# richarddurbin/modimizer

Hardware: AMD Instinct MI355X
Metric: Gbp/s hashed+sketched (k=21,d=64) (higher is better)
Workload: dtype u64; 1 GPU; BASELINE config 2: 10 Gbp synthetic ONT-like reads (log-normal N50 20 kb, 5% subs, 30x of a 333 Mbp genome), k=21 d=64 seed=17, seqhash scan + modset build (table bits 30); reads_per_gpu=598835, bases_per_gpu=10000000000, modimizers_per_gpu=156043826, modset_entries=102967436, k=21, d=64, table_bits=30, parallelism=reads sharded x1, modset per GPU

## Files before the change

include/modgpu.h:

```cpp
#ifndef MODGPU_H
#define MODGPU_H

#include <stdio.h>
#include <stdint.h>
#include <stdbool.h>
#include <stddef.h>

#if defined (MODGPU_WITH_REFERENCE_HEADERS) || defined (MS_MINOR)
#ifdef __cplusplus
extern "C" {
#endif
void mgSeqhashDestroy (Seqhash *sh) ;
void mgSeqhashRCiteratorDestroy (SeqhashRCiterator *si) ;
#ifdef __cplusplus
}
#endif
#else
#include "modgpu_compat.h"
#endif

#ifdef __cplusplus
extern "C" {
#endif


typedef enum {
  MG_OK = 0,
  MG_ERR_NO_DEVICE = 1,
  MG_ERR_HIP = 2,
  MG_ERR_ARG = 3,
  MG_ERR_CAPACITY = 4,
  MG_ERR_NOMEM = 5
} MgStatus ;

const char *mgLastError (void) ;
int  mgDeviceCount (void) ;
MgStatus mgSetDevice (int device) ;
const char *mgVersion (void) ;
const char *mgSourceHash (void) ;

U64 *mgIterScanHost (const Seqhash *sh, const char *s, int len) ;
void mgReloadKnobs (void) ;
int  mgIterHostBelow (int below) ;

MgStatus mgDeviceAlloc (void **dptr, size_t bytes) ;
MgStatus mgDeviceFree (void *dptr) ;
MgStatus mgMemcpyH2D (void *dst, const void *src, size_t bytes, void *stream) ;
MgStatus mgMemcpyD2H (void *dst, const void *src, size_t bytes, void *stream) ;
MgStatus mgMemsetD (void *dst, int byte, size_t bytes, void *stream) ;
MgStatus mgStreamSynchronize (void *stream) ;
MgStatus mgCopyD2HBig (void *hostDst, const void *devSrc, size_t bytes) ;
MgStatus mgCopyH2DBig (void *devDst, const void *hostSrc, size_t bytes) ;

#define MG_PACK_PAD 8
size_t   mgPackedWords (U64 nBases) ;
void     mgPackHost (const char *bases, U64 nBases, U32 *words) ;
MgStatus mgPackDevice (const U8 *dBases, U64 nBases, U32 *dWords, void *stream) ;
MgStatus mgUnpackDevice (const U32 *dWords, U64 nBases, U8 *dBases, void *stream) ;
MgStatus mgUploadPack (const char *bases, U64 nBases, U32 *dPacked, void *stream) ;

#define MG_POS_MASK 0x7fffffffu
#define MG_FWD_BIT  0x80000000u
size_t   mgScanWorkBytes (U64 totalBases, U32 nReads, U64 capacity) ;
MgStatus seqhashScanBatchDevice (const Seqhash *sh, const U32 *dPacked, U64 totalBases,
                                 const U64 *dReadOffsets, U32 nReads,
                                 U64 *dKmer, U32 *dPosF, U32 *dReadId, U64 capacity,
                                 U64 *dCount, void *dWork, void *stream) ;

int64_t seqhashScanBatch (const Seqhash *sh, const char *bases, const int64_t *readOffsets, int nReads,
                          U64 **kmer, int **pos, bool **isF, int64_t **survStart) ;

MgStatus seqhashMinimizerBatchDevice (const Seqhash *sh, const U32 *dPacked, U64 totalBases,
                                      const U64 *dReadOffsets, U32 nReads,
                                      U64 *dHash, U32 *dPosF, U64 *dReadStart, U64 capacity, U64 *n, void *stream) ;
int64_t seqhashMinimizerBatch (const Seqhash *sh, const char *bases, const int64_t *readOffsets, int nReads,
                               U64 **hash, int **pos, bool **isF, int64_t **start) ;

MgStatus modsetAddBatchDevice (Modset *ms, const U64 *dKmer, U64 n, U32 *dIndexOut, int withDepth, void *stream) ;
MgStatus modsetFindBatchDevice (Modset *ms, const U64 *dKmer, U64 n, U32 *dIndexOut, void *stream) ;

MgStatus modsetSyncToHost (Modset *ms, int wantIndex) ;
int      mgXferThreadCount (void) ;
void     mgXferDiag (U64 out8[8]) ;
MgStatus mgModsetDeviceRelease (Modset *ms) ;
void     mgModsetHostChanged (Modset *ms) ;
MgStatus mgModsetClear (Modset *ms, void *stream) ;

U64 mgModsetDeviceSlots (Modset *ms) ;

MgStatus mgTableCheckLayout (Modset *ms, U64 *out6) ;
MgStatus mgTableDiag (Modset *ms, U64 *out9) ;
MgStatus mgScanDiag (U64 *out18) ;

MgStatus modsetDepthHistogramDevice (Modset *ms, U64 *dHist65536, void *stream) ;

MgStatus mgAddReadsDevice (Modset *ms, const U32 *dPacked, U64 totalBases,
                           const U64 *dReadOffsets, U32 nReads, U64 *nHash, void *stream) ;
MgStatus mgQueryReadsDevice (Modset *ms, const U32 *dPacked, U64 totalBases,
                             const U64 *dReadOffsets, U32 nReads,
                             U32 *dSeedIndex, U32 *dSeedPosF, U32 *dSeedRead, U64 capacity,
                             U64 *nSeeds, void *stream) ;

MgStatus mgQueryReadsDeviceAsync (Modset *ms, const U32 *dPacked, U64 totalBases, const U64 *dReadOffsets, U32 nReads,
                                  U32 *dSeedIndex, U32 *dSeedPosF, U32 *dSeedRead, U64 capacity, void **ticket, void *stream) ;
MgStatus mgQueryReadsDeviceWait (void *ticket, U64 *nSeeds, void *stream) ;

MgStatus mgInsertReadsDevice (Modset *ms, const U32 *dPacked, U64 totalBases,
                              const U64 *dReadOffsets, U32 nReads,
                              U32 *dSeedIndex, U32 *dSeedPosF, U32 *dSeedRead, U64 capacity,
                              U64 *nSeeds, void *stream) ;

bool mgModsetMergeArrays (Modset *ms1, U64 *value2, U16 *depth2, U8 *info2, U32 n2) ;
bool mgModsetMergeDeviceArrays (Modset *ms1, const U64 *dValue2, const U16 *dDepth2, const U8 *dInfo2, U32 n2) ;

typedef struct MgComm MgComm ;
MgStatus mgCommInitAll (MgComm **comms , int nDev, const int *devices ) ;
MgStatus mgCommGetUniqueId (void *id128) ;
MgStatus mgCommInitRank (MgComm **comm, int nRanks, int rank, const void *id128, int device) ;
int      mgCommRank (const MgComm *c) ;
int      mgCommSize (const MgComm *c) ;
void     mgCommDestroy (MgComm *c) ;
MgStatus mgHistogramAllReduce (Modset *ms, U64 *hist65536, MgComm *c) ;
MgStatus mgDepthAllReduce (Modset *ms, MgComm *c) ;
MgStatus mgModsetMergeRankOrder (Modset *ms, MgComm *c, int root) ;

int64_t mgAddSequenceBatch (Modset *ms, const char *bases, const int64_t *readOffsets, int nReads) ;
void    mgDepthHistogram (Modset *ms, FILE *f) ;
int     mgAddSequences (Modset *ms, const char *bases, const int64_t *readOffsets, int nReads, FILE *out) ;
void    mgModsetWriteText (Modset *ms, FILE *f) ;

typedef struct {
  Modset *ms ;
  U32 size ;
  U32 max ;
  U32 *index, *offset, *id ;
  U32 *depth ;
  U32 *rev, *loc ;
  int nSeq ;
  char **names ;
  U32 *len ;
} MgReference ;
MgReference *mgReferenceCreate (Modset *ms, U32 size) ;
void mgReferenceDestroy (MgReference *ref) ;
int  mgReferenceRead (MgReference *ref, const char *bases, const int64_t *offsets, int nSeq,
                      const char **names, bool isAdd, FILE *out) ;
void mgReferenceWrite (MgReference *ref, const char *root) ;
FILE *mgGzipOpenWrite (const char *name) ;
FILE *mgGzipOpenRead (const char *name) ;
FILE *mgFzOpen (const char *name, const char *mode) ;
MgReference *mgReferenceLoad (const char *root) ;
int  mgQueryProcess (MgReference *ref, const char *bases, const int64_t *offsets, int nReads,
                     const char **names, FILE *out) ;
void mgSetVerbose (int on) ;

typedef struct {
  Modset *ms ;
  int nReads, capReads ;
  int *len, *nHit, *nMiss ;
  int (*nCopy)[4] ;
  U64 *hitStart ;
  U32 *hit ; U16 *dx ;
  U64 totHit, capHit ;
  U64 *invStart ;
  U32 *invSpace ;
  U8 *bad ; int *contained ;
} MgReadset ;
MgReadset *mgReadsetCreate (Modset *ms) ;
void mgReadsetDestroy (MgReadset *rs) ;
int  mgReadsetRead (MgReadset *rs, const char *bases, const int64_t *offsets, int nReads) ;
int  mgReadsetFileRead (MgReadset *rs, const char *filename) ;
void mgReadsetStats (MgReadset *rs, FILE *out) ;
void mgReadsetWrite (MgReadset *rs, const char *root) ;
MgReadset *mgReadsetLoad (const char *root) ;
int  mgReadsetCleanMods (MgReadset *rs, FILE *out) ;
int  mgReadsetCleanModsPath (void) ;
int  mgReadsetProperties (MgReadset *rs, FILE *out) ;
int  mgReadsetPropertiesPath (void) ;
typedef struct { U32 n ; U64 *start ;
                 U32 *iy ; U16 *nHit, *nBadOrder, *nBadFlip ; U8 *flags ; } MgOverlaps ;
int  mgReadsetFindOverlaps (MgReadset *rs, const U32 *reads, U32 n, int level, FILE *out, MgOverlaps *res ) ;
void mgOverlapsFree (MgOverlaps *res) ;
int  mgReadsetOverlapStats (MgReadset *rs, U32 d, FILE *out) ;
int  mgReadsetMarkBadReads (MgReadset *rs, FILE *out) ;
int  mgReadsetMarkContained (MgReadset *rs, FILE *out) ;
int  mgReadsetOverlapsPath (void) ;
void mgReadsetOverlapsDiag (U64 out4[4]) ;
typedef struct { U8 flags ;
                 int rDNApos, nGood, nMod2, nBadLD, nSplit, nSplitLD ; } MgModInfo ;
int  mgReadsetRefFlagFile (MgReadset *rs, const char *refFile, FILE *out) ;
int  mgReadsetRefFlagHits (MgReadset *rs, const U32 *index, const int *pos, U64 n, FILE *out) ;
int  mgReadsetResetBits (MgReadset *rs, int op, FILE *out) ;
int  mgReadsetTestMods (MgReadset *rs, int minDepth, int maxDepth, FILE *yFile, FILE *zFile, FILE *out) ;
const MgModInfo *mgReadsetModInfo (const MgReadset *rs) ;
const U8 *mgReadsetReadFlags (const MgReadset *rs) ;
int  mgReadsetTestModsRun (const MgReadset *rs) ;
int  mgReadsetRdnaPath (void) ;
void mgReadsetRdnaDiag (U64 out4[4]) ;
void mgReadsetRdnaGrid (U32 out4[4]) ;

typedef struct {
  Modset *ms ;
  int len ;
  int *pos ;
  bool *isF ;
  int ownsMs ;
} MgRepRef ;
MgRepRef *mgRepRefCreate (const char *seqFile, const char *modFile, FILE *err) ;
MgRepRef *mgRepRefFromArrays (Modset *ms, const char *bases, int64_t len, FILE *err) ;
void mgRepRefDestroy (MgRepRef *ref) ;

typedef struct MgRepRun MgRepRun ;
typedef struct {
  int nRead, nBad, nGood ;
  int *n, *seqF, *seqR ;
  bool *bad, *isF ;
  U32 max ;
  int *modN, *modNPre ;
  int *goodI, *goodLen ;
  U64 *hitStart ;
  int *hitK, *hitX ;
  int nMod, nDup, tDup, minMax ;
} MgRepResult ;
void mgRepResultFree (MgRepResult *res) ;
MgRepRun *mgRepRunBegin (MgRepRef *ref, Modset *ms) ;
int  mgRepRunAdd (MgRepRun *run, const char *bases, const int64_t *offsets, int nReads, FILE *out) ;
int  mgRepRunFinish (MgRepRun *run, FILE *err, MgRepResult *res) ;
int  mgRepAnalyze3File (MgRepRef *ref, const char *seqFile, const char *modFile, FILE *out, FILE *err, MgRepResult *res) ;
int  mgRepPath (void) ;

typedef struct {
  int nRead, nBad, nGood ;
  U32 max ;
  int nmod[5][4] ;
  int readsBefore, readsAfter ;
  int *modN, *modNPre, *modNPost ;
  U64 *preStart, *postStart ;
  int *preK, *preN, *preX, *postK, *postN, *postX ;
  int *readI ;
  U64 *hitStart ;
  int *hitK ;
} MgRep1Result ;
void mgRep1ResultFree (MgRep1Result *res) ;
int  mgRepRunFinish1 (MgRepRun *run, FILE *out, FILE *err, MgRep1Result *res) ;
int  mgRepAnalyze1File (MgRepRef *ref, const char *seqFile, const char *modFile, FILE *out, FILE *err, MgRep1Result *res) ;
int  mgRepAnalyze1Hits (U32 max, int K, int nReads, const int *readI, const U64 *hitStart, const int *hitK, const int *hitX,
// ... 98 lines not shown
```

modimizer_amd/__init__.py:

```python
import contextlib
import ctypes as C
import os
import subprocess

import numpy as np

_HERE = os.path.dirname(os.path.abspath(__file__))
LIB_PATH = os.environ.get("MODGPU_LIB") or os.path.join(_HERE, "libmodgpu.so")
CSRC = os.path.join(_HERE, "csrc")

U64P = C.POINTER(C.c_uint64)
U32P = C.POINTER(C.c_uint32)

MG_POS_MASK = 0x7FFFFFFF
MG_FWD_BIT = 0x80000000


class Seqhash(C.Structure):
    _fields_ = [("seed", C.c_int), ("k", C.c_int), ("w", C.c_int), ("mask", C.c_uint64),
                ("shift1", C.c_int), ("shift2", C.c_int), ("factor1", C.c_uint64),
                ("factor2", C.c_uint64), ("patternRC", C.c_uint64 * 4)]


class SeqhashRCiterator(C.Structure):
    _fields_ = [("sh", C.POINTER(Seqhash)), ("s", C.c_void_p), ("sEnd", C.c_void_p),
                ("h", C.c_uint64), ("hRC", C.c_uint64), ("hashBuf", C.c_void_p), ("fBuf", C.c_void_p),
                ("base", C.c_int), ("iStart", C.c_int), ("iMin", C.c_int), ("isDone", C.c_bool)]


class Modset(C.Structure):
    _fields_ = [("hasher", C.POINTER(Seqhash)), ("tableBits", C.c_int), ("size", C.c_uint32),
                ("tableSize", C.c_uint64), ("tableMask", C.c_uint64), ("index", U32P),
                ("value", U64P), ("depth", C.POINTER(C.c_uint16)), ("info", C.POINTER(C.c_uint8)),
                ("max", C.c_uint32)]


class MgReference(C.Structure):
    _fields_ = [("ms", C.POINTER(Modset)), ("size", C.c_uint32), ("max", C.c_uint32),
                ("index", U32P), ("offset", U32P), ("id", U32P), ("depth", U32P), ("rev", U32P), ("loc", U32P),
                ("nSeq", C.c_int), ("names", C.POINTER(C.c_char_p)), ("len", U32P)]


class MgReadset(C.Structure):
    _fields_ = [("ms", C.POINTER(Modset)), ("nReads", C.c_int), ("capReads", C.c_int),
                ("len", C.POINTER(C.c_int)), ("nHit", C.POINTER(C.c_int)), ("nMiss", C.POINTER(C.c_int)),
                ("nCopy", C.POINTER(C.c_int * 4)), ("hitStart", U64P), ("hit", U32P), ("dx", C.POINTER(C.c_uint16)),
                ("totHit", C.c_uint64), ("capHit", C.c_uint64), ("invStart", U64P), ("invSpace", U32P),
                ("bad", C.POINTER(C.c_uint8)), ("contained", C.POINTER(C.c_int))]


class MgOverlaps(C.Structure):
    _fields_ = [("n", C.c_uint32), ("start", U64P), ("iy", U32P), ("nHit", C.POINTER(C.c_uint16)), ("nBadOrder", C.POINTER(C.c_uint16)),
                ("nBadFlip", C.POINTER(C.c_uint16)), ("flags", C.POINTER(C.c_uint8))]


class MgModInfo(C.Structure):
    _fields_ = [("flags", C.c_uint8), ("rDNApos", C.c_int), ("nGood", C.c_int), ("nMod2", C.c_int), ("nBadLD", C.c_int), ("nSplit", C.c_int), ("nSplitLD", C.c_int)]


class MgRepRef(C.Structure):
    _fields_ = [("ms", C.POINTER(Modset)), ("len", C.c_int), ("pos", C.POINTER(C.c_int)), ("isF", C.POINTER(C.c_bool)), ("ownsMs", C.c_int)]


class MgRepResult(C.Structure):
    _fields_ = [("nRead", C.c_int), ("nBad", C.c_int), ("nGood", C.c_int),
                ("n", C.POINTER(C.c_int)), ("seqF", C.POINTER(C.c_int)), ("seqR", C.POINTER(C.c_int)),
                ("bad", C.POINTER(C.c_bool)), ("isF", C.POINTER(C.c_bool)), ("max", C.c_uint32),
                ("modN", C.POINTER(C.c_int)), ("modNPre", C.POINTER(C.c_int)),
                ("goodI", C.POINTER(C.c_int)), ("goodLen", C.POINTER(C.c_int)), ("hitStart", U64P),
                ("hitK", C.POINTER(C.c_int)), ("hitX", C.POINTER(C.c_int)),
                ("nMod", C.c_int), ("nDup", C.c_int), ("tDup", C.c_int), ("minMax", C.c_int)]


class MgRep1Result(C.Structure):
    _fields_ = [("nRead", C.c_int), ("nBad", C.c_int), ("nGood", C.c_int), ("max", C.c_uint32), ("nmod", (C.c_int * 4) * 5),
                ("readsBefore", C.c_int), ("readsAfter", C.c_int),
                ("modN", C.POINTER(C.c_int)), ("modNPre", C.POINTER(C.c_int)), ("modNPost", C.POINTER(C.c_int)),
                ("preStart", U64P), ("postStart", U64P),
                ("preK", C.POINTER(C.c_int)), ("preN", C.POINTER(C.c_int)), ("preX", C.POINTER(C.c_int)),
                ("postK", C.POINTER(C.c_int)), ("postN", C.POINTER(C.c_int)), ("postX", C.POINTER(C.c_int)),
                ("readI", C.POINTER(C.c_int)), ("hitStart", U64P), ("hitK", C.POINTER(C.c_int))]


class MgComposition(C.Structure):
    _fields_ = [("type", C.c_int), ("nSeq", C.c_uint64), ("totLen", C.c_uint64), ("lenMin", C.c_uint64), ("lenMax", C.c_uint64),
                ("base", C.c_uint64 * 256), ("qual", C.c_uint64 * 256), ("nBins", C.c_uint32), ("binCount", C.POINTER(C.c_int)), ("binSum", U64P)]


class MgSeqConvert(C.Structure):
    _fields_ = [("inType", C.c_int), ("outType", C.c_int)] + [(n, C.c_uint64) for n in (
        "nSeq", "totSeqLen", "maxSeqLen", "totIdLen", "totDescLen", "maxIdLen", "maxDescLen", "nSeqIn", "totSeqLenIn")]


class MgGzMember(C.Structure):
    _fields_ = [("cOff", C.c_uint64), ("uOff", C.c_uint64), ("cLen", C.c_uint32), ("uLen", C.c_uint32), ("crc", C.c_uint32), ("pad", C.c_uint32)]


class MgGzBlock(C.Structure):
    _fields_ = [("uOff", C.c_uint64), ("uLen", C.c_uint32), ("pad", C.c_uint32)]


class MgSeqBatch(C.Structure):
    _fields_ = [("bases", C.POINTER(C.c_int8)), ("offsets", C.POINTER(C.c_int64)), ("names", C.POINTER(C.c_char_p)),
                ("nSeq", C.c_int), ("total", C.c_int64), ("isFastq", C.c_int), ("basesCap", C.c_int64)]


EXPORTS = [
    "seqhashCreate", "seqhashWrite", "seqhashRead", "seqhashReport", "modRCiterator", "modRCnext",
    "minimizerRCiterator", "minimizerRCnext", "seqString", "mgSeqhashDestroy", "mgSeqhashRCiteratorDestroy",
    "modsetCreate", "modsetDestroy", "modsetWrite", "modsetRead", "modsetIndexFind", "modsetSummary",
    "modsetPack", "modsetDepthPrune", "modsetMerge",
    "mgLastError", "mgDeviceCount", "mgSetDevice", "mgVersion", "mgSourceHash", "mgDeviceAlloc", "mgDeviceFree",
    "mgMemcpyH2D", "mgMemcpyD2H", "mgMemsetD", "mgStreamSynchronize",
    "mgPackedWords", "mgPackHost", "mgPackDevice", "mgUnpackDevice", "mgUploadPack",
    "mgScanWorkBytes", "seqhashScanBatchDevice", "seqhashScanBatch", "seqhashMinimizerBatchDevice", "seqhashMinimizerBatch",
    "modsetAddBatchDevice", "modsetFindBatchDevice", "modsetSyncToHost", "mgXferThreadCount", "mgXferDiag", "mgCopyD2HBig", "mgCopyH2DBig", "mgModsetDeviceRelease",
    "mgModsetHostChanged", "modsetDepthHistogramDevice", "mgTableCheckLayout", "mgTableDiag", "mgScanDiag", "mgAddReadsDevice", "mgQueryReadsDevice", "mgQueryReadsDeviceAsync", "mgQueryReadsDeviceWait",
    "mgAddSequenceBatch", "mgDepthHistogram", "mgSynthGenome", "mgSynthReads",
    "mgInsertReadsDevice", "mgAddSequences", "mgModsetWriteText", "mgReferenceCreate", "mgReferenceDestroy",
    "mgReferenceRead", "mgQueryProcess", "mgReferenceWrite", "mgGzipOpenWrite", "mgFzOpen", "mgGzipOpenRead", "mgReferenceLoad",
    "mgCommInitAll", "mgCommGetUniqueId", "mgCommInitRank", "mgCommRank", "mgCommSize", "mgCommDestroy", "mgHistogramAllReduce", "mgDepthAllReduce", "mgModsetMergeRankOrder",
    "mgReadsetCreate", "mgReadsetDestroy", "mgReadsetRead", "mgReadsetFileRead", "mgReadsetStats", "mgReadsetWrite", "mgReadsetLoad",
    "mgReadsetCleanMods", "mgReadsetCleanModsPath", "mgReadsetProperties", "mgReadsetPropertiesPath",
    "mgReadsetFindOverlaps", "mgOverlapsFree", "mgReadsetOverlapStats", "mgReadsetMarkBadReads", "mgReadsetMarkContained", "mgReadsetOverlapsPath", "mgReadsetOverlapsDiag",
    "mgReadsetRefFlagFile", "mgReadsetRefFlagHits", "mgReadsetResetBits", "mgReadsetTestMods", "mgReadsetModInfo", "mgReadsetReadFlags", "mgReadsetTestModsRun", "mgReadsetRdnaPath", "mgReadsetRdnaDiag", "mgReadsetRdnaGrid",
    "mgRepRefCreate", "mgRepRefFromArrays", "mgRepRefDestroy", "mgRepRunBegin", "mgRepRunAdd", "mgRepRunFinish", "mgRepResultFree", "mgRepAnalyze3File", "mgRepPath",
    "mgRep1ResultFree", "mgRepRunFinish1", "mgRepAnalyze1File", "mgRepAnalyze1Hits", "mgRepCount2", "mgRepAnalyze2File", "mgRep1Diag",
    "mgCompositionFile", "mgCompositionText", "mgCompositionFree", "mgCompositionDiag",
    "mgSeqConvertFile", "mgSeqConvertText", "mgSeqConvertDiag",
    "mgInflateMembersDevice", "mgInflateDiag", "mgInflateMemberHost", "mgBgzfInflateFile", "mgGzipInflateFile", "mgGunzipHost", "mgGunzipDiag",
    "mgDeflateBlocksDevice", "mgDeflateBlockHost", "mgDeflateDiag", "mgBgzfDeflateFile", "mgSeqConvertFileBgzf",
    "mgSeqOpen", "mgSeqNextBatch", "mgSeqBatchFree", "mgSeqClose", "mgSeqReleaseBuffers", "mgReleaseBuffers", "mgTextParseFileDevice", "mgSeqOpenAt", "mgTextFileDiag", "mgAddSequenceFile", "mgReferenceFastaRead", "mgQueryFile",
    "mgReportDepths", "mgRefPaint", "mgRefPaintFile", "mgModsetWriteTextDevice", "mgModsetReadText", "mgModsetReadTextPath",
    "mgAddSequenceFile10x", "mgAddSequenceBatch10x", "mgTrim10xDevice", "mgAdd10xDiag",
    "mgModsetSetCopy", "mgModsetSetCopyM", "mgModsetSetCopyPath", "mgModsetSummaryDevice",
    "mgIterScanHost", "mgIterHostBelow", "mgReloadKnobs", "mgFormatF2", "mgModsetMergeArrays", "mgModsetMergeDeviceArrays", "mgModsetClear", "mgModsetDeviceSlots", "mgSetVerbose", "mgProfileEnable", "mgProfileOnly", "mgProfileReset", "mgProfileKernels", "mgProfileGet",
]


@contextlib.contextmanager
def knobs(**kv):
    old = {}
    for k, v in kv.items():
        name = "MODGPU_" + k
        old[name] = os.environ.get(name)
        if v is None:
            os.environ.pop(name, None)
        else:
            os.environ[name] = str(v)
    lib().mgReloadKnobs()
    try:
        yield
    finally:
        for name, v in old.items():
            if v is None:
                os.environ.pop(name, None)
            else:
                os.environ[name] = v
        lib().mgReloadKnobs()


def source_hash():
    import hashlib
    names = sorted(f for f in os.listdir(CSRC) if f.endswith((".hip", ".c", ".h"))) + ["Makefile", "../../include/modgpu.h", "../../include/modgpu_compat.h"]
    inc = os.path.join(_HERE, "..", "include")
    path = lambda n: os.path.join(inc, os.path.basename(n)) if n.startswith("../") else os.path.join(CSRC, n)
    listing = "".join("%s  %s\n" % (hashlib.sha256(open(path(n), "rb").read()).hexdigest(), n) for n in names)
    return hashlib.sha256(listing.encode()).hexdigest()[:16]


def binary_hash(path=None):
    import re
    try:
        m = re.search(rb"MODGPU_SRC_HASH=([0-9a-f]{16})", open(path or LIB_PATH, "rb").read())
    except OSError:
        return None
    return m.group(1).decode() if m else None


def build(force=False):
    import fcntl
    if os.environ.get("MODGPU_LIB"):
        return LIB_PATH
    def make_if_stale():
        if force or binary_hash() != source_hash():
            subprocess.check_call(["make", "-C", CSRC, "-j8", "-s"] + (["-B"] if force else []))
            if binary_hash() != source_hash():
                raise RuntimeError("libmodgpu.so does not carry the hash of its sources after make: %s != %s" % (binary_hash(), source_hash()))
    try:
        lk = open(os.path.join(CSRC, ".build.lock"), "w")
    except OSError:
        make_if_stale()
        return LIB_PATH
    with lk:
        fcntl.flock(lk, fcntl.LOCK_EX)
        make_if_stale()
    return LIB_PATH


_lib = None


def lib():
    global _lib
    if _lib is not None:
        return _lib
    if os.environ.get("MODGPU_NO_TORCH", "0") != "1":
        try:
            import torch
        except Exception:
            pass
    build()
    L = C.CDLL(LIB_PATH, mode=C.RTLD_GLOBAL)
    if not os.environ.get("MODGPU_LIB"):
        L.mgSourceHash.restype = C.c_char_p
        if L.mgSourceHash().decode() != source_hash():
            raise RuntimeError("the loaded libmodgpu.so was not built from the sources in this tree")
    vp, u64, u32, i32, i64 = C.c_void_p, C.c_uint64, C.c_uint32, C.c_int, C.c_int64
    SH, MS, IT = C.POINTER(Seqhash), C.POINTER(Modset), C.POINTER(SeqhashRCiterator)

    def sig(name, res, *args):
        if os.environ.get("MODGPU_LIB") and not hasattr(L, name):
            return
        f = getattr(L, name); f.restype = res; f.argtypes = list(args)
    sig("seqhashCreate", SH, i32, i32, i32)
    sig("seqhashWrite", None, SH, vp); sig("seqhashRead", SH, vp); sig("seqhashReport", None, SH, vp)
    sig("modRCiterator", IT, SH, vp, i32)
    sig("modRCnext", C.c_bool, IT, U64P, C.POINTER(i32), C.POINTER(C.c_bool))
    sig("minimizerRCiterator", IT, SH, vp, i32)
    sig("mgIterScanHost", vp, SH, vp, i32); sig("mgIterHostBelow", i32, i32); sig("mgReloadKnobs", None)
    sig("mgFormatF2", i32, C.c_char_p, C.c_double)
    sig("minimizerRCnext", C.c_bool, IT, U64P, C.POINTER(i32), C.POINTER(C.c_bool))
    sig("seqString", C.c_char_p, u64, i32)
    sig("mgSeqhashDestroy", None, SH); sig("mgSeqhashRCiteratorDestroy", None, IT)
    sig("modsetCreate", MS, SH, i32, u32); sig("modsetDestroy", None, MS)
    sig("modsetWrite", None, MS, vp); sig("modsetRead", MS, vp)
    sig("modsetIndexFind", u32, MS, u64, i32); sig("modsetSummary", None, MS, vp)
    sig("modsetPack", C.c_bool, MS); sig("modsetDepthPrune", None, MS, i32, i32)
    sig("modsetMerge", C.c_bool, MS, MS)
    sig("mgLastError", C.c_char_p); sig("mgDeviceCount", i32); sig("mgSetDevice", i32, i32)
    sig("mgVersion", C.c_char_p)
    sig("mgSourceHash", C.c_char_p)
    sig("mgDeviceAlloc", i32, C.POINTER(vp), C.c_size_t); sig("mgDeviceFree", i32, vp)
    sig("mgMemcpyH2D", i32, vp, vp, C.c_size_t, vp); sig("mgMemcpyD2H", i32, vp, vp, C.c_size_t, vp)
    sig("mgMemsetD", i32, vp, i32, C.c_size_t, vp); sig("mgStreamSynchronize", i32, vp)
    sig("mgPackedWords", C.c_size_t, u64); sig("mgPackHost", None, vp, u64, vp)
    sig("mgUploadPack", i32, vp, u64, vp, vp); sig("mgPackDevice", i32, vp, u64, vp, vp); sig("mgUnpackDevice", i32, vp, u64, vp, vp)
    sig("mgScanWorkBytes", C.c_size_t, u64, u32, u64)
    sig("seqhashScanBatchDevice", i32, SH, vp, u64, vp, u32, vp, vp, vp, u64, vp, vp, vp)
    sig("seqhashScanBatch", i64, SH, vp, vp, i32, C.POINTER(vp), C.POINTER(vp), C.POINTER(vp), C.POINTER(vp))
    sig("seqhashMinimizerBatchDevice", i32, SH, vp, u64, vp, u32, vp, vp, vp, u64, U64P, vp)
    sig("seqhashMinimizerBatch", i64, SH, vp, vp, i32, C.POINTER(vp), C.POINTER(vp), C.POINTER(vp), C.POINTER(vp))
    sig("modsetAddBatchDevice", i32, MS, vp, u64, vp, i32, vp)
    sig("modsetFindBatchDevice", i32, MS, vp, u64, vp, vp)
    sig("modsetSyncToHost", i32, MS, i32); sig("mgXferThreadCount", i32); sig("mgXferDiag", None, U64P); sig("mgCopyD2HBig", i32, vp, vp, C.c_size_t); sig("mgCopyH2DBig", i32, vp, vp, C.c_size_t); sig("mgModsetDeviceRelease", i32, MS)
    sig("mgModsetHostChanged", None, MS)
    sig("modsetDepthHistogramDevice", i32, MS, vp, vp); sig("mgTableCheckLayout", i32, MS, U64P); sig("mgTableDiag", i32, MS, U64P); sig("mgScanDiag", i32, U64P)
    sig("mgAddReadsDevice", i32, MS, vp, u64, vp, u32, U64P, vp)
    sig("mgQueryReadsDevice", i32, MS, vp, u64, vp, u32, vp, vp, vp, u64, U64P, vp)
    sig("mgQueryReadsDeviceAsync", i32, MS, vp, u64, vp, u32, vp, vp, vp, u64, C.POINTER(vp), vp); sig("mgQueryReadsDeviceWait", i32, vp, U64P, vp)
    sig("mgAddSequenceBatch", i64, MS, vp, vp, i32); sig("mgDepthHistogram", None, MS, vp)
    sig("mgSynthGenome", i32, vp, u64, u64, vp)
    sig("mgSynthReads", i32, vp, u64, vp, vp, vp, u32, u64, C.c_double, u64, vp, vp)
    sig("mgInsertReadsDevice", i32, MS, vp, u64, vp, u32, vp, vp, vp, u64, U64P, vp)
    sig("mgAddSequences", i32, MS, vp, vp, i32, vp); sig("mgModsetWriteText", None, MS, vp)
    sig("mgReferenceCreate", vp, MS, u32); sig("mgReferenceDestroy", None, vp)
    sig("mgReferenceRead", i32, vp, vp, vp, i32, C.POINTER(C.c_char_p), C.c_bool, vp)
    sig("mgQueryProcess", i32, vp, vp, vp, i32, C.POINTER(C.c_char_p), vp)
    RS = C.POINTER(MgReadset)
    sig("mgReadsetCreate", RS, MS); sig("mgReadsetDestroy", None, RS)
    sig("mgReadsetRead", i32, RS, vp, vp, i32); sig("mgReadsetFileRead", i32, RS, C.c_char_p)
    sig("mgReadsetStats", None, RS, vp); sig("mgReadsetWrite", None, RS, C.c_char_p); sig("mgReadsetLoad", RS, C.c_char_p)
    sig("mgReadsetCleanMods", i32, RS, vp); sig("mgReadsetCleanModsPath", i32); sig("mgReadsetProperties", i32, RS, vp); sig("mgReadsetPropertiesPath", i32)
    sig("mgReadsetFindOverlaps", i32, RS, vp, C.c_uint32, i32, vp, C.POINTER(MgOverlaps)); sig("mgOverlapsFree", None, C.POINTER(MgOverlaps))
    sig("mgReadsetOverlapStats", i32, RS, C.c_uint32, vp); sig("mgReadsetMarkBadReads", i32, RS, vp); sig("mgReadsetMarkContained", i32, RS, vp)
    sig("mgReadsetOverlapsPath", i32); sig("mgReadsetOverlapsDiag", None, vp)
    sig("mgReadsetRefFlagFile", i32, RS, C.c_char_p, vp); sig("mgReadsetRefFlagHits", i32, RS, vp, vp, u64, vp); sig("mgReadsetResetBits", i32, RS, i32, vp)
    sig("mgReadsetTestMods", i32, RS, i32, i32, vp, vp, vp); sig("mgReadsetModInfo", C.POINTER(MgModInfo), RS); sig("mgReadsetReadFlags", C.POINTER(C.c_uint8), RS)
    sig("mgReadsetTestModsRun", i32, RS); sig("mgReadsetRdnaPath", i32); sig("mgReadsetRdnaDiag", None, vp); sig("mgReadsetRdnaGrid", None, vp)
    RR, RES = C.POINTER(MgRepRef), C.POINTER(MgRepResult)
    sig("mgRepRefCreate", RR, C.c_char_p, C.c_char_p, vp); sig("mgRepRefFromArrays", RR, MS, vp, i64, vp); sig("mgRepRefDestroy", None, RR)
    sig("mgRepRunBegin", vp, RR, MS); sig("mgRepRunAdd", i32, vp, vp, vp, i32, vp); sig("mgRepRunFinish", i32, vp, vp, RES); sig("mgRepResultFree", None, RES)
    sig("mgRepAnalyze3File", i32, RR, C.c_char_p, C.c_char_p, vp, vp, RES); sig("mgRepPath", i32)
    RES1 = C.POINTER(MgRep1Result)
    sig("mgRep1ResultFree", None, RES1); sig("mgRepRunFinish1", i32, vp, vp, vp, RES1); sig("mgRepAnalyze1File", i32, RR, C.c_char_p, C.c_char_p, vp, vp, RES1)
    sig("mgRepAnalyze1Hits", i32, C.c_uint32, i32, i32, vp, vp, vp, vp, vp, vp, RES1); sig("mgRepCount2", i32, RR, vp, vp, i32, vp)
    sig("mgRepAnalyze2File", i32, RR, C.c_char_p, C.c_char_p, vp, vp); sig("mgRep1Diag", None, vp)
    COMP = C.POINTER(MgComposition)
    sig("mgCompositionFile", i32, C.c_char_p, i32, vp, vp, COMP); sig("mgCompositionText", i32, vp, u64, i32, vp, vp, COMP)
    sig("mgCompositionFree", None, COMP); sig("mgCompositionDiag", None, vp)
    CONV = C.POINTER(MgSeqConvert)
    sig("mgSeqConvertFile", i32, C.c_char_p, C.c_char_p, i32, vp, CONV); sig("mgSeqConvertText", i32, vp, u64, i32, vp, vp, CONV); sig("mgSeqConvertDiag", None, vp)
    sig("mgInflateMembersDevice", i32, vp, u64, C.POINTER(MgGzMember), u32, vp, u64, vp, C.POINTER(u32), vp); sig("mgInflateDiag", None, vp)
    sig("mgInflateMemberHost", i32, vp, u32, vp, u32, u32, C.POINTER(u32), vp); sig("mgBgzfInflateFile", i32, C.c_char_p, C.c_char_p, vp)
    sig("mgGzipInflateFile", i32, C.c_char_p, C.c_char_p, vp); sig("mgGunzipDiag", None, vp)
    sig("mgGunzipHost", i32, vp, u64, u32, u32, u32, vp, u64, C.POINTER(u64), C.POINTER(u32), vp)
    sig("mgDeflateBlocksDevice", i32, vp, u64, C.POINTER(MgGzBlock), u32, vp, u64, C.POINTER(u64), vp); sig("mgDeflateDiag", None, vp)
    sig("mgDeflateBlockHost", i32, vp, u32, vp, C.POINTER(u32), vp); sig("mgBgzfDeflateFile", i32, C.c_char_p, C.c_char_p, vp)
    sig("mgSeqConvertFileBgzf", i32, C.c_char_p, C.c_char_p, i32, vp, CONV)
    sig("mgSeqOpen", vp, C.c_char_p); sig("mgSeqNextBatch", i32, vp, C.c_int64, C.POINTER(MgSeqBatch))
    sig("mgSeqBatchFree", None, C.POINTER(MgSeqBatch)); sig("mgSeqClose", None, vp); sig("mgSeqReleaseBuffers", None); sig("mgReleaseBuffers", None)
    sig("mgTextParseFileDevice", i32, C.c_char_p, C.POINTER(vp), C.POINTER(vp), C.POINTER(i64))
    sig("mgSeqOpenAt", vp, C.c_char_p, u64, u64, u64); sig("mgTextFileDiag", None, vp)
    sig("mgAddSequenceFile", i32, MS, C.c_char_p, vp); sig("mgReferenceFastaRead", i32, vp, C.c_char_p, C.c_bool, vp)
    sig("mgQueryFile", i32, vp, C.c_char_p, vp)
    sig("mgReportDepths", i32, MS, C.POINTER(MS), i32, vp)
    sig("mgRefPaint", i32, MS, vp, vp, i32, C.POINTER(C.c_char_p), vp); sig("mgRefPaintFile", i32, MS, C.c_char_p, vp)
    sig("mgModsetWriteTextDevice", i32, MS, vp); sig("mgModsetReadText", MS, C.c_char_p); sig("mgModsetReadTextPath", i32)
    sig("mgAddSequenceFile10x", i32, MS, C.c_char_p, vp); sig("mgAddSequenceBatch10x", i64, MS, vp, vp, i32, u64)
    sig("mgTrim10xDevice", i32, vp, u64, vp, u32, u64, vp, vp, U64P, vp); sig("mgAdd10xDiag", None, U64P)
    sig("mgModsetSetCopy", i32, MS, i32, i32, i32); sig("mgModsetSetCopyM", i32, MS, i32); sig("mgModsetSetCopyPath", i32)
    sig("mgModsetSummaryDevice", i32, MS, vp)
    sig("mgReferenceWrite", None, vp, C.c_char_p); sig("mgGzipOpenWrite", vp, C.c_char_p); sig("mgGzipOpenRead", vp, C.c_char_p); sig("mgFzOpen", vp, C.c_char_p, C.c_char_p);
    sig("mgCommInitAll", i32, C.POINTER(vp), i32, C.POINTER(i32)); sig("mgCommGetUniqueId", i32, vp); sig("mgCommInitRank", i32, C.POINTER(vp), i32, i32, vp, i32)
    sig("mgCommRank", i32, vp); sig("mgCommSize", i32, vp); sig("mgCommDestroy", None, vp)
    sig("mgHistogramAllReduce", i32, MS, vp, vp); sig("mgDepthAllReduce", i32, MS, vp); sig("mgModsetMergeRankOrder", i32, MS, vp, i32)
    sig("mgReferenceLoad", C.POINTER(MgReference), C.c_char_p)
    sig("mgModsetMergeArrays", C.c_bool, MS, vp, vp, vp, u32)
    sig("mgModsetMergeDeviceArrays", C.c_bool, MS, vp, vp, vp, u32)
    sig("mgModsetClear", i32, MS, vp); sig("mgModsetDeviceSlots", u64, MS); sig("mgSetVerbose", None, i32)
    sig("mgProfileEnable", None, i32); sig("mgProfileOnly", None, i32); sig("mgProfileReset", None); sig("mgProfileKernels", i32)
    sig("mgProfileGet", i32, i32, C.POINTER(C.c_char_p), C.POINTER(C.c_double), U64P)
    _lib = L
    return L


class ModgpuError(RuntimeError):
    pass


def check(status):
    if status != 0:
        raise ModgpuError("libmodgpu status %d: %s" % (status, lib().mgLastError().decode()))


_libc = C.CDLL(None)
_libc.free.argtypes = [C.c_void_p]
_libc.fopen.restype = C.c_void_p
_libc.fopen.argtypes = [C.c_char_p, C.c_char_p]
_libc.fclose.argtypes = [C.c_void_p]


class CFile:

    def __init__(self, path, mode="w"):
        self.f = _libc.fopen(path.encode(), mode.encode())
        if not self.f:
            raise OSError("cannot open " + path)

    def __enter__(self):
        return C.c_void_p(self.f)

    def __exit__(self, *a):
        _libc.fclose(self.f)



def seqhashCreate(k, w, seed=17):
    if k < 1 or k >= 32:
        raise ValueError("seqhash k %d must be between 1 and 32" % k)
    if w < 1:
        raise ValueError("seqhash w %d must be positive" % w)
    return lib().seqhashCreate(k, w, seed)


def modsetCreate(sh, bits, size=0):
    if bits < 20 or bits > 34:
        raise ValueError("table bits %d must be between 20 and 34" % bits)
    if size >= (1 << bits) >> 2:
        raise ValueError("Modset size %u is too big for %d bits" % (size, bits))
    return lib().modsetCreate(sh, bits, size)


def iterate(sh, bases, minimizer=False):
    L = lib()
    bases = np.ascontiguousarray(bases, dtype=np.uint8)
    mk, nx = (L.minimizerRCiterator, L.minimizerRCnext) if minimizer else (L.modRCiterator, L.modRCnext)
    it = mk(sh, bases.ctypes.data, len(bases))
    u = C.c_uint64(); p = C.c_int(); f = C.c_bool()
    ks, ps, fs = [], [], []
    while nx(it, C.byref(u), C.byref(p), C.byref(f)):
        ks.append(u.value); ps.append(p.value); fs.append(int(f.value))
    L.mgSeqhashRCiteratorDestroy(it)
    return np.array(ks, np.uint64), np.array(ps, np.int32), np.array(fs, np.uint8)


def scan_batch(sh, bases, offsets):
    L = lib()
    bases = np.ascontiguousarray(bases, dtype=np.uint8)
    offsets = np.ascontiguousarray(offsets, dtype=np.int64)
    n_reads = len(offsets) - 1
    pk, pp, pf, ps = C.c_void_p(), C.c_void_p(), C.c_void_p(), C.c_void_p()
    n = L.seqhashScanBatch(sh, bases.ctypes.data, offsets.ctypes.data, n_reads,
                           C.byref(pk), C.byref(pp), C.byref(pf), C.byref(ps))
    if n < 0:
        raise ModgpuError("seqhashScanBatch failed: " + L.mgLastError().decode())

    def take(ptr, ctype, count, dtype):
        a = np.ctypeslib.as_array(C.cast(ptr, C.POINTER(ctype)), (max(count, 1),))[:count].astype(dtype, copy=True)
        _libc.free(ptr)
        return a
    kmer = take(pk, C.c_uint64, n, np.uint64)
    pos = take(pp, C.c_int, n, np.int32)
    isf = take(pf, C.c_bool, n, np.uint8)
    st = take(ps, C.c_int64, n_reads + 1, np.int64)
    return kmer, pos, isf, st


def minimizer_batch(sh, bases, offsets):
    L = lib()
# ... 691 lines not shown
```

modimizer_amd/csrc/mg_api_int.h:

```cpp
#ifndef MG_API_INT_H
#define MG_API_INT_H
#include <stdlib.h>
#include <string.h>
#include <mutex>
#include "mg_common.h"
#include "mg_internal.h"

#define MG_LOOKUP_LOAD_PCT 40

struct MgArena {
  char *base = 0; size_t bytes = 0; size_t used = 0;
  MgStatus reserve (size_t need)
  { if (need <= bytes) return MG_OK;
    if (base) MG_HIP (hipFree (base));
    base = 0; bytes = 0;
    size_t want = need + need / 8 + (1 << 20);
    MG_HIP (hipMalloc ((void **) &base, want));
    bytes = want;
    return MG_OK;
  }
  void reset () { used = 0; }
  void *take (size_t n) { size_t a = mgAl256 (used); used = a + n; return base + a; }
  void release () { if (base) (void) hipFree (base); base = 0; bytes = used = 0; }
};

struct MgDev {
  MgTable t;
  MgArena arena;
  MgArena arena2;
  hipStream_t side = 0;
  hipEvent_t scanned[2] = { 0, 0 }, inputReady = 0;
  int ticketsOut = 0, nextSlot = 0; bool slotBusy[2] = { false, false };
  U64 *hPin;
  U32 hostIndexMax;
  bool built;
  int device = -1;
};

static inline U64 mgScanRetryCap (const volatile U64 *c, U64 cap, U64 *n)
{ *n = c[0]; return (c[1] || c[0] > cap) ? c[3] : 0; }

MG_HIDDEN MgStatus mgCheckHasher (const Seqhash *sh);
MG_HIDDEN U64      mgSurvivorGuess (const Seqhash *sh, U64 totalBases);
MG_HIDDEN void     mgUploadRelease (void);
MG_HIDDEN MgDev   *mgDevLookup (const Modset *ms);
MG_HIDDEN MgStatus mgDevGet (Modset *ms, MgDev **out, hipStream_t st);
MG_HIDDEN MgStatus mgDevRefuseInFlight (const MgDev *d);
MG_HIDDEN U64      mgAddChunkSize (void);
#define MG_ADD_CHUNK (mgAddChunkSize ())
MG_HIDDEN MgStatus mgAddBatch (Modset *ms, MgDev *d, const U64 *dKmer, U64 n, U32 *dIndexOut, int withDepth,
                               bool arenaLive, hipStream_t st, const MgHistReq *counted = 0, const MgSegSrc *segSrc = 0);
extern "C" void mgHostBatchRelease (void);
#endif
```

modimizer_amd/csrc/mg_common.h:

```cpp
#ifndef MG_COMMON_H
#define MG_COMMON_H
#include "mg_knobs.h"

#include <hip/hip_runtime.h>
#include <stdint.h>
#include <time.h>
#include <algorithm>
#include <vector>
#include "modgpu.h"

#define MG_WAVE 64

#define MG_SCAN_THREADS   256
#define MG_POS_PER_THREAD 64
#define MG_TILE_BASES     (64 * MG_POS_PER_THREAD)
#define MG_TILE_WORDS     (MG_TILE_BASES / 16)

struct MgHashParams {
  U64 factor1;
  U64 mask;
  int k;
  int shift1;
  U32 d;
  int dShift;
  U64 dOddInv;
  U64 dOddLim;
  U32 c24;
  U32 inv32;
  U32 lim32;
  U32 small32;
};

void mgSetError (const char *fmt, ...);
MgStatus mgHipFail (hipError_t e, const char *what);
MgStatus mgEnsureDevice (void);
MgHashParams mgMakeParams (const Seqhash *sh);

enum MgKernelId {
  MG_K_PACK = 0, MG_K_UNPACK, MG_K_TILE_FIRST_READ, MG_K_SCAN, MG_K_TABLE_INSERT, MG_K_TABLE_ASSIGN,
  MG_K_TABLE_FLAG, MG_K_TABLE_FIND, MG_K_TABLE_LOAD, MG_K_TABLE_EXPORT, MG_K_TABLE_HIST,
  MG_K_INDEX_REPLAY, MG_K_INDEX_FINISH, MG_K_SYNTH_GENOME, MG_K_SYNTH_READS, MG_K_MEMSET,
  MG_K_SEG_SCAN, MG_K_SEG_COMPACT, MG_K_PART, MG_K_PART_HIST, MG_K_PART_SCATTER, MG_K_RANK_COUNT, MG_K_RANK_SCAN, MG_K_BUCKET_DEDUP,
  MG_K_BUCKET_MERGE, MG_K_RANK_LOOKUP, MG_K_TABLE_FIND_SEG, MG_K_HOT_REDUCE, MG_K_BUCKET_FIND, MG_K_UNPART, MG_K_CHAIN, MG_K_CHAIN_RESOLVE,
  MG_K_PAINT_ITEMS, MG_K_DEPTH_GUARD, MG_K_DEPTH_GATHER, MG_K_TEXT_LEN, MG_K_TEXT_SCAN, MG_K_TEXT_WRITE,
  MG_K_SETTEXT_LINES, MG_K_SETTEXT_SCAN, MG_K_SETTEXT_PARSE, MG_K_SETTEXT_LAST,
  MG_K_OVL_ACTIVE, MG_K_OVL_EMIT, MG_K_OVL_SORT, MG_K_OVL_RUNS, MG_K_OVL_PAIR,
  MG_K_TRIM_OFFSETS, MG_K_TRIM_GATHER, MG_K_SETCOPY, MG_K_COPY_TALLY, MG_K_COUNT
};
void mgProfBegin (int id, hipStream_t st);
void mgProfEnd (int id, hipStream_t st);
#define MG_LAUNCH(id, st, ...) do { mgProfBegin (id, st); hipLaunchKernelGGL (__VA_ARGS__); mgProfEnd (id, st); } while (0)

#define MG_HIP(call) do { hipError_t e_ = (call); if (e_ != hipSuccess) return mgHipFail (e_, #call); } while (0)

struct MgDevScratch {
  const char *what; std::vector<void *> held;
  explicit MgDevScratch (const char *what_) : what (what_) {}
  MgDevScratch (const MgDevScratch &) = delete;
  MgDevScratch &operator= (const MgDevScratch &) = delete;
  ~MgDevScratch () { for (void *p : held) (void) hipFree (p); }
  MgStatus fail () const { return mgHipFail (hipGetLastError (), what); }
  void adopt (void *p) { if (p) held.push_back (p); }
  template <class T> MgStatus get (T **p, size_t count)
  { *p = 0; const hipError_t e = hipMalloc ((void **) p, count * sizeof (T)); if (e != hipSuccess) return mgHipFail (e, what); adopt (*p); return MG_OK; }
  template <class T> T *take (T *p) { held.erase (std::remove (held.begin (), held.end (), (void *) p), held.end ()); return p; }
};
static inline bool mgDevFreeBytes (size_t *freeB)
{ size_t total = 0; if (hipMemGetInfo (freeB, &total) != hipSuccess) { (void) hipGetLastError (); return false; } return true; }
static inline int mgFailedWith (const char *sentence) { if (!mgLastError ()[0]) mgSetError ("%s", sentence); return -1; }

template <class T> struct MgDevBuf {
  T *p = 0; size_t cap = 0;
  MgStatus reserve (size_t want, size_t alloc, const char *what)
  { if (cap >= want) return MG_OK;
    drop ();
    const hipError_t e = hipMalloc ((void **) &p, alloc * sizeof (T)); if (e != hipSuccess) { p = 0; return mgHipFail (e, what); }
    cap = alloc; return MG_OK;
  }
  void drop () { if (p) (void) hipFree (p); p = 0; cap = 0; }
};

#ifdef __HIPCC__
__device__ __forceinline__ bool mgDivisible (U64 x, const MgHashParams &p)
{
  if (x & (((U64) 1 << p.dShift) - 1)) return false;
  return ((x >> p.dShift) * p.dOddInv) <= p.dOddLim;
}

__device__ __forceinline__ bool mgDivisibleOdd (U64 h, const MgHashParams &p) { return h * p.dOddInv <= p.dOddLim; }

__device__ __forceinline__ bool mgDivisibleOdd32 (U64 h, const MgHashParams &p)
{
  const U32 lo = (U32) h, hi = (U32) (h >> 32);
  const U32 a = __builtin_amdgcn_alignbit (hi, lo, 24);
  const U32 t = __umul24 (a, p.c24) + (lo & 0xffffffu);
  return t * p.inv32 <= p.lim32;
}

__device__ __forceinline__ bool mgDivisibleAny32 (U64 h, const MgHashParams &p)
{
  return !((U32) h & (((U32) 1 << p.dShift) - 1u)) && mgDivisibleOdd32 (h >> p.dShift, p);
}

__device__ __forceinline__ U32 mgRevComp16 (U32 w)
{
  const U32 x = __brev (w);
  return __builtin_amdgcn_bitop3_b32 (x << 1, x >> 1, 0x55555555u, 0x27);
}

__device__ __forceinline__ U64 mgRevComp (U64 f, int shift1)
{
  const U64 x = ((U64) mgRevComp16 ((U32) f) << 32) | mgRevComp16 ((U32) (f >> 32));
  return x >> shift1;
}
struct MgGeom { U32 R; int log2NB; int kbits; };
__device__ __forceinline__ U64 mgMixBits (U64 x, int b)
{
  if (b <= 32)
    { U32 y = (U32) x;
      const U32 m32 = b >= 32 ? ~0u : (((U32) 1 << b) - 1);
      const int h32 = (b + 1) >> 1;
      y ^= y >> h32; y = (y * 0xed558ccdu) & m32;
      y ^= y >> h32; y = (y * 0x1a85ec53u) & m32;
      y ^= y >> h32;
      return y;
    }
  const U64 mask = b >= 64 ? ~0ull : (((U64) 1 << b) - 1);
  const int h = (b + 1) >> 1;
  x ^= x >> h; x = (x * 0xff51afd7ed558ccdull) & mask;
  x ^= x >> h; x = (x * 0xc4ceb9fe1a85ec53ull) & mask;
  x ^= x >> h;
  return x;
}
#define MG_MIX_TOP 10
#define MG_MIX_MUL 0x9E3779B1u
__device__ __forceinline__ U64 mgMixK (U64 x, int b)
{
  if (b < 24) return mgMixBits (x, b);
  const int lb = b - MG_MIX_TOP;
  const U64 L = x & (((U64) 1 << lb) - 1), A = x >> lb;
  const U32 low = lb >= 32 ? (U32) L : ((U32) L & (((U32) 1 << lb) - 1));
  const U32 g = (low * MG_MIX_MUL) >> (32 - MG_MIX_TOP);
  return ((A ^ (U64) g) << lb) | mgMixBits (L, lb);
}
__device__ __forceinline__ U32 mgMixTopOfKmer (U64 x, int b, int hiB)
{
  const int lb = b - MG_MIX_TOP;
  const U32 low = lb >= 32 ? (U32) x : ((U32) x & (((U32) 1 << lb) - 1));
  return (U32) (x >> (b - hiB)) ^ ((low * MG_MIX_MUL) >> (32 - hiB));
}
__device__ __forceinline__ U32 mgBucketOfM (U64 m, const MgGeom &g)
{
  if (!g.log2NB) return 0u;
  const int s = g.kbits - g.log2NB;
  return s >= 0 ? (U32) (m >> s) : ((U32) m << (-s));
}
__device__ __forceinline__ U32 mgHomeOfM (U64 m, const MgGeom &g)
{
  U32 x = (U32) m;
  if (g.kbits >= 24) x ^= (U32) (m >> (g.kbits - MG_MIX_TOP)) * 0x9E5u;
  return __umulhi (x * 0x85EBCA6Bu, g.R);
}
__device__ __forceinline__ U32 mgNextSlot (U32 at, U32 R) { return at + 1 == R ? 0u : at + 1; }
#endif

static inline unsigned mgGrid (U64 n, unsigned per = 256, unsigned cap = 4096)
{ U64 b = (n + per - 1) / per; if (b > cap) b = cap; if (b < 1) b = 1; return (unsigned) b; }
static inline size_t mgAl256 (size_t n) { return (n + 255) & ~(size_t) 255; }
static inline double mgNowS (void) { struct timespec ts; clock_gettime (CLOCK_MONOTONIC, &ts); return ts.tv_sec + 1e-9 * ts.tv_nsec; }

static inline void mgPartSplit (int log2NB, int *hiB, int *loB)
{ if (log2NB <= 9) { *hiB = log2NB; *loB = 0; } else { *loB = log2NB / 2; *hiB = log2NB - *loB; } }

#define MG_HIST_STRIDE 16
struct MgHistReq { int log2NB; int kbits; U32 *binCount; int hiB; };

struct MgSegSrc { const U64 *segKmer; const U64 *segCount; const U64 *segStart; U64 segCap; U32 nSegs; };


MgStatus mgLaunchPack (const U8 *dBases, U64 nBases, U32 *dWords, hipStream_t st);
MgStatus mgLaunchUnpack (const U32 *dWords, U64 nBases, U8 *dBases, hipStream_t st);
MgStatus mgLaunchScan (const MgHashParams &p, const U32 *dPacked, U64 totalBases,
                       const U64 *dReadOffsets, U32 nReads,
                       U64 *dKmer, U32 *dPosF, U32 *dReadId, U64 capacity,
                       U64 *dCount, void *dWork, hipStream_t st, const MgHistReq *hist = 0, MgSegSrc *lazy = 0);

U64      mgScanTiles (U64 totalBases);
size_t   mgScanInfoBytes (U64 totalBases);
MgStatus mgScanPrepare (const U64 *dReadOffsets, U32 nReads, U64 totalBases, void *dInfo, hipStream_t st);
size_t   mgScanRangeWorkBytes (U64 nTilesRange, U64 capacity);
MgStatus mgLaunchSegCompact (const MgSegSrc &src, U64 *dKmer, U64 capacity, const U64 *dCount, hipStream_t st);
MgStatus mgLaunchScanRange (const MgHashParams &p, const U32 *dPacked, U64 totalBases,
                            const U64 *dReadOffsets, U32 nReads, const void *dInfo, U64 tile0, U64 tile1,
                            U64 *dKmer, U32 *dPosF, U32 *dReadId, U64 capacity,
                            U64 *dCount, void *dWork, hipStream_t st, const MgHistReq *hist = 0, MgSegSrc *lazy = 0);

U64      mgIterMaxBases (void);
U64      mgIterSegEntries (void);
MgStatus mgLaunchIterScan (const MgHashParams &p, const U32 *dPacked, U64 totalBases, const U64 *dReadOff,
                           U64 *dSegKmer, U32 *dSegPosF, U64 *out, U64 capEntries, U64 *flag, U64 seq, hipStream_t st);

MgStatus mgLaunchMinimizers (const MgHashParams &p, U32 w, const U32 *dPacked, const U64 *dReadOffsets, U32 nReads,
                             U64 *dHash, U32 *dPosF, U64 *dReadStart, U64 capacity, U64 *totalOut, hipStream_t st);

struct MgSlot { U64 key; U32 ord; U32 cnt; };
struct MgTable {
  MgSlot *slots; U64 nSlots;
  U64 capSlots;
  U32 capNB;
  U32 R; int log2NB;
  int kbits;
  U32 *occ;
  U64 *value;
  U16 *baseDepth;
  bool baseZero;
  U64 *liveHist;
  bool liveHistValid;
  U32 size;
  U32 max;
  U32 syncedMax;
  U64 *counters;
  bool pendingDepth;
  bool dirty;
  U64 *find8;
  U64 find8Cap;
  U64 find8Version, version;
  bool empty;
  U64 *pin;
  int newPct;
  int loadPct;
  int  maxLog2Slots;
  U32  wantR;
  U64  diag[7];
  int  tightPct;
};
MgStatus mgTableAlloc (MgTable *t, U64 slotsWanted, hipStream_t st);
MgStatus mgTableEnsure (MgTable *t, U64 nIncoming, hipStream_t st);
MgStatus mgTableRollback (MgTable *t, hipStream_t st);
MgStatus mgTableClean (MgTable *t, hipStream_t st);
void     mgTableForget (MgTable *t, hipStream_t st);
size_t   mgTableAddScratchBytes (const MgTable *t, U64 n);
bool     mgTableUseBuckets (const MgTable *t, U64 n);
MgStatus mgTableAdd (MgTable *t, const U64 *dKmer, U64 n, int withDepth, void *scratch, hipStream_t st,
                     const MgHistReq *counted = 0,
                     const MgSegSrc *segSrc = 0);
bool     mgTableAddTakesSegments (const MgTable *t, U64 n, const MgHistReq *counted);
MgStatus mgTableMarkOccupied (MgTable *t, const U64 *dKmer, U64 n, hipStream_t st);
MgStatus mgTableFind (MgTable *t, const U64 *dKmer, U64 n, U32 *dIndexOut, hipStream_t st);
MgStatus mgTableLayoutCheck (MgTable *t, U64 *dOut4, hipStream_t st);
enum { MG_DIAG_FIND_DIRECT = 0, MG_DIAG_FIND_PART1, MG_DIAG_FIND_PART2_16, MG_DIAG_FIND_PART2_8, MG_DIAG_PACK8, MG_DIAG_REHASH_BUCKET, MG_DIAG_REHASH_ATOMIC };
size_t   mgTableFindPartScratchBytes (U64 n);
int      mgTableFindDigitBits (const MgTable *t);
bool     mgTableFindTakesPartition (const MgTable *t, U64 n, const MgHistReq *counted);
size_t   mgTableFindPart2ScratchBytes (U64 n);
MgStatus mgTableFindPartitioned (MgTable *t, const MgSegSrc &segSrc, U64 n, const MgHistReq *counted, U32 *dIndexOut, U64 *el, void *scratch, hipStream_t st,
                                 void *scratch2 = 0);
MgStatus mgTableFindSegments (MgTable *t, const MgSegSrc &src, U64 n, U32 *dIndexOut, hipStream_t st);
MgStatus mgTableLoadHost (MgTable *t, const U64 *dValue, U32 first, U32 last, hipStream_t st);
MgStatus mgTableExportDepth (MgTable *t, U16 *dDelta, hipStream_t st);
MgStatus mgTableHistogram (MgTable *t, U64 *dHist, hipStream_t st);
MgStatus mgModsetTableForPass (Modset *ms, MgTable **t);
MgStatus mgTableReplayIndex (MgTable *t, const MgHashParams &p, int tableBits, U32 *dIndex, hipStream_t st);
MgStatus mgTableMergeApply (const U32 *dIdx, const U16 *dDepth2, const U8 *dInfo2, U32 n2, U16 *dBaseDepth, U8 *dInfo1, hipStream_t st);
size_t   mgTablePruneScratchBytes (U32 n);
MgStatus mgTablePrune (MgTable *t, const U8 *dInfo, int lo, int hi, U64 *dNewValue, U16 *dNewDepth, U8 *dNewInfo,
                       void *scratch, hipStream_t st);
#define MG_COUNT_WORDS 4

MgStatus mgLaunchSynthGenome (U32 *dPacked, U64 nBases, U64 seed, hipStream_t st);
MgStatus mgLaunchSynthReads (const U32 *dGenome, U64 genomeBases, const U64 *dReadStart,
                             const U64 *dReadOffsets, const U8 *dStrand, U32 nReads, U64 totalBases,
                             double errRate, U64 seed, U32 *dOut, hipStream_t st);

#endif
```

modimizer_amd/csrc/mg_knobs.c:

```c
#define _GNU_SOURCE
#include <pthread.h>
#include <sched.h>
#include <stdio.h>
#include <stdlib.h>
#include <string.h>
#include <unistd.h>
#include <sys/mman.h>
#include "mg_knobs.h"

static MgKnobs gKnobs;
static pthread_once_t gOnce = PTHREAD_ONCE_INIT;

static long num (const char *name)
{ const char *e = getenv (name); return e && *e ? atol (e) : MG_KNOB_UNSET; }

static void readAll (void)
{
  MgKnobs k;
  const char *e = getenv ("MODGPU_TABLE_PATH");
  k.tablePath = e && *e ? (long) e[0] : MG_KNOB_UNSET;
  e = getenv ("MODGPU_FIND_PATH");
  k.findPath = e && *e ? (long) e[0] : MG_KNOB_UNSET;
  k.partPacked = num ("MODGPU_PART_PACKED");       k.partBig = num ("MODGPU_PART_BIG");
  k.addChunk = num ("MODGPU_ADD_CHUNK");           k.scanGrid = num ("MODGPU_SCAN_GRID");
  k.scanGeneric = num ("MODGPU_SCAN_GENERIC");     k.scanHist = num ("MODGPU_SCAN_HIST");
  k.scanDiv64 = num ("MODGPU_SCAN_DIV64");        k.minTiled = num ("MODGPU_MIN_TILED");
  k.minTile = num ("MODGPU_MIN_TILE");
  k.noSegmentInput = num ("MODGPU_NO_SEGMENT_INPUT");
  k.rankSliceShift = num ("MODGPU_RANK_SLICE_SHIFT");
  k.flagPolarity = num ("MODGPU_FLAG_POLARITY");   k.mergeSlots = num ("MODGPU_MERGE_SLOTS");
  k.mergePlace = num ("MODGPU_MERGE_PLACE");
  k.bucketR = num ("MODGPU_BUCKET_R");             k.bucketT = num ("MODGPU_BUCKET_T");
  e = getenv ("MODGPU_HOT_SPLIT");
  k.hotSplit = e && *e ? atol (e) : MG_KNOB_UNSET;
  { const char *c = e ? strchr (e, ',') : 0; k.hotChunk = c ? atol (c + 1) : MG_KNOB_UNSET; }
  k.noAvx2 = num ("MODGPU_NO_AVX2");               k.textHost = num ("MODGPU_TEXT_HOST");
  k.textWindowKb = num ("MODGPU_TEXT_WINDOW_KB");   k.bgzfHost = num ("MODGPU_BGZF_HOST");
  k.inflateNoCrc = num ("MODGPU_INFLATE_NOCRC");   k.bgzfBlock = num ("MODGPU_BGZF_BLOCK");
  k.gzipHost = num ("MODGPU_GZIP_HOST");           k.gzipChunkKb = num ("MODGPU_GZIP_CHUNK_KB");
  k.gzipBatch = num ("MODGPU_GZIP_BATCH");         k.gzipRatio = num ("MODGPU_GZIP_RATIO");
  k.gzipMinKb = num ("MODGPU_GZIP_MIN_KB");
  k.fileBatchMbp = num ("MODGPU_FILE_BATCH_MBP");  k.fileBatchBases = num ("MODGPU_FILE_BATCH_BASES");
  k.textIdsDevice = num ("MODGPU_TEXT_IDS_DEVICE");
  k.queryHostChain = num ("MODGPU_QUERY_HOST_CHAIN");
  k.iterHostBelow = num ("MODGPU_ITER_HOST_BELOW");
  k.readsetHost = num ("MODGPU_READSET_HOST");
  k.overlapCands = num ("MODGPU_OVERLAP_CANDS");
  k.overlapLds = num ("MODGPU_OVERLAP_LDS");
  k.testModsBatch = num ("MODGPU_TESTMODS_BATCH");
  k.segSlack = num ("MODGPU_SEG_SLACK");
  k.partDigits = num ("MODGPU_PART_DIGITS");
  k.findBits = num ("MODGPU_FIND_BITS");
  k.scatterGrid = num ("MODGPU_SCATTER_GRID");     k.tableLoad = num ("MODGPU_TABLE_LOAD");
  k.tightLoad = num ("MODGPU_TIGHT_LOAD");         k.find8 = num ("MODGPU_FIND8");
  k.packThreads = num ("MODGPU_PACK_THREADS");     k.parseThreads = num ("MODGPU_PARSE_THREADS");
  k.xferThreads = num ("MODGPU_XFER_THREADS");       k.gzipThreads = num ("MODGPU_GZIP_THREADS");
  k.xferPieceKb = num ("MODGPU_XFER_PIECE_KB");      k.xferStreams = num ("MODGPU_XFER_STREAMS");
  k.seedTiming = num ("MODGPU_SEED_TIMING");       k.uploadTiming = num ("MODGPU_UPLOAD_TIMING");
  k.textTiming = num ("MODGPU_TEXT_TIMING");       k.parseTiming = getenv ("MODGPU_PARSE_TIMING") ? 1 : MG_KNOB_UNSET;
  k.scanDebug = num ("MODGPU_SCAN_DEBUG");         k.bucketDebug = num ("MODGPU_BUCKET_DEBUG");
  gKnobs = k;
}

const MgKnobs *mgKnobs (void) { pthread_once (&gOnce, readAll); return &gKnobs; }
void mgIterKnobsReloaded (void) __attribute__ ((weak));
void mgReloadKnobs (void) { pthread_once (&gOnce, readAll); readAll (); if (mgIterKnobsReloaded) mgIterKnobsReloaded (); }

static int gCpuBudget;
static pthread_once_t gCpuOnce = PTHREAD_ONCE_INIT;
static void cpuBudgetOnce (void)
{
  long v = sysconf (_SC_NPROCESSORS_ONLN);
  cpu_set_t set;
  if (sched_getaffinity (0, sizeof (set), &set) == 0 && CPU_COUNT (&set) < v) v = CPU_COUNT (&set);
  FILE *q = fopen ("/sys/fs/cgroup/cpu.max", "r");
  if (q)
    { char a[64]; long per = 0;
      if (fscanf (q, "%63s %ld", a, &per) == 2 && strcmp (a, "max") && per > 0) { const long c = (atol (a) + per - 1) / per; if (c < v) v = c; }
      fclose (q);
    }
  gCpuBudget = v < 1 ? 1 : (int) v;
}
int mgCpuBudget (void) { pthread_once (&gCpuOnce, cpuBudgetOnce); return gCpuBudget; }

void mgHugeHint (void *p, size_t n)
{
#ifdef MADV_HUGEPAGE
  if (p && n >= ((size_t) 8 << 20))
    { const size_t pg = 4096;
      char *a = (char *) (((size_t) p + pg - 1) & ~(pg - 1)), *e = (char *) (((size_t) p + n) & ~(pg - 1));
      if (e > a) (void) madvise (a, (size_t) (e - a), MADV_HUGEPAGE);
    }
#else
  (void) p; (void) n;
#endif
}
void *mgAllocBig (size_t n) { void *p = malloc (n ? n : 1); mgHugeHint (p, n); return p; }
```

modimizer_amd/csrc/mg_knobs.h:

```cpp
#ifndef MG_KNOBS_H
#define MG_KNOBS_H
#include <limits.h>
#ifdef __cplusplus
extern "C" {
#endif
#define MG_KNOB_UNSET LONG_MIN
typedef struct {
  long findPath;
  long tablePath;
  long partPacked;
  long partBig;
  long addChunk;
  long scanGrid;
  long scanGeneric;
  long minTile;
  long minTiled;
  long scanDiv64;
  long scanHist;
  long noSegmentInput;
  long rankSliceShift;
  long flagPolarity;
  long mergeSlots;
  long mergePlace;
  long bucketR, bucketT;
  long hotSplit, hotChunk;
  long noAvx2;
  long textHost;
  long textWindowKb;
  long fileBatchMbp;
  long fileBatchBases;
  long readsetHost;
  long overlapCands;
  long testModsBatch;
  long overlapLds;
  long bgzfHost;
  long textIdsDevice;
  long gzipHost;
  long gzipChunkKb;
  long gzipBatch;
  long gzipRatio;
  long gzipMinKb;
  long bgzfBlock;
  long queryHostChain;
  long iterHostBelow;
  long scatterGrid;
  long segSlack;
  long partDigits;
  long findBits;
  long tableLoad;
  long find8;
  long tightLoad;
  long packThreads;
  long parseThreads;
  long gzipThreads;
  long xferPieceKb;
  long xferStreams;
  long xferThreads;
  long inflateNoCrc;
  long seedTiming, uploadTiming, textTiming, parseTiming;
  long scanDebug, bucketDebug;
} MgKnobs;
const MgKnobs *mgKnobs (void);
void mgReloadKnobs (void);
int mgCpuBudget (void);
#include <stddef.h>
void mgHugeHint (void *p, size_t n);
void *mgAllocBig (size_t n);
#ifdef __cplusplus
}
#endif
#endif
```

modimizer_amd/csrc/mg_modsetdev.hip:

```cpp
#include <unordered_map>
#include "mg_api_int.h"
#include "mg_xfer.h"

struct MgOnDevice
{ int before = -1; bool moved = false;
  explicit MgOnDevice (int dev) { if (dev >= 0 && hipGetDevice (&before) == hipSuccess && before != dev) moved = hipSetDevice (dev) == hipSuccess; }
  ~MgOnDevice () { if (moved) (void) hipSetDevice (before); }
};

static std::mutex gRegLock;
static std::unordered_map<const Modset *, MgDev *> gReg;
extern "C" { volatile int mgLiveDeviceModsets = 0; }

MgDev *mgDevLookup (const Modset *ms)
{ std::lock_guard<std::mutex> g (gRegLock); auto it = gReg.find (ms); return it == gReg.end () ? 0 : it->second; }

static void mgDevFree (MgDev *d)
{
  if (!d) return;
  MgOnDevice here (d->device);
  if (d->hPin) (void) hipHostFree (d->hPin);
  if (d->built)
    { (void) hipFree (d->t.slots); (void) hipFree (d->t.value); (void) hipFree (d->t.occ); (void) hipFree (d->t.find8);
      (void) hipFree (d->t.baseDepth); (void) hipFree (d->t.counters); (void) hipFree (d->t.liveHist);
    }
  if (d->side) { (void) hipStreamSynchronize (d->side); (void) hipStreamDestroy (d->side); }
  d->arena.release (); d->arena2.release ();
  for (int i = 0 ; i < 2 ; ++i) if (d->scanned[i]) (void) hipEventDestroy (d->scanned[i]);
  if (d->inputReady) (void) hipEventDestroy (d->inputReady);
  delete d;
}

static void mgDevDrop (Modset *ms, MgDev *d)
{
  { std::lock_guard<std::mutex> g (gRegLock); gReg.erase (ms); mgLiveDeviceModsets = (int) gReg.size (); }
  mgDevFree (d);
}

static MgStatus mgDevOnCallersGpu (const MgDev *d, bool quiet = false)
{
  int cur = -1;
  if (hipGetDevice (&cur) == hipSuccess && cur == d->device) return MG_OK;
  if (!quiet) mgSetError ("this Modset's table lives on GPU %d, the calling thread is on GPU %d (mgSetDevice)", d->device, cur);
  return MG_ERR_ARG;
}

MgStatus mgDevRefuseInFlight (const MgDev *d)
{
  if (!d->ticketsOut) return MG_OK;
  mgSetError ("a query batch of this modset is in flight (mgQueryReadsDeviceAsync without its mgQueryReadsDeviceWait)");
  return MG_ERR_ARG;
}

static MgStatus mgDevBuild (Modset *ms, MgDev *d, hipStream_t st)
{
  MgTable &t = d->t;
  if (ms->tableBits < 20 || ms->tableBits > 32)
    { mgSetError ("device modset supports table bits 20..32 (got %d)", ms->tableBits); return MG_ERR_ARG; }
  memset (&t, 0, sizeof (t));
  t.maxLog2Slots = ms->tableBits - 1;
  t.kbits = 2 * ms->hasher->k;
  t.wantR = 4096;
  { const long r = mgKnobs ()->bucketR; if (r != MG_KNOB_UNSET && r >= 256) t.wantR = (U32) r; }
  t.size = ms->size;
  t.pin = d->hPin + 24;
  U64 cap = (ms->tableSize >> 2);
  MG_HIP (hipMalloc ((void **) &t.value, cap * sizeof (U64)));
  MG_HIP (hipMalloc ((void **) &t.baseDepth, cap * sizeof (U16)));
  MG_HIP (hipMalloc ((void **) &t.counters, 64));
  d->built = true;
  MG_HIP (hipMemsetAsync (t.baseDepth, 0, cap * sizeof (U16), st));
  MG_HIP (hipMemsetAsync (t.counters, 0, 64, st));
  { MgStatus s0 = mgTableEnsure (&t, ms->max, st); if (s0) return s0; }
  t.max = 0; t.syncedMax = 0;
  t.baseZero = !ms->max;
  if (ms->max)
    { MG_HIP (hipStreamSynchronize (st));
      MgStatus s;
      if ((s = mgXferH2D (t.value, ms->value, ((size_t) ms->max + 1) * sizeof (U64)))) return s;
      if ((s = mgXferH2D (t.baseDepth, ms->depth, ((size_t) ms->max + 1) * sizeof (U16)))) return s;
      if ((s = mgTableLoadHost (&t, t.value, 1, ms->max, st))) return s;
      MG_HIP (hipStreamSynchronize (st));
      t.max = t.syncedMax = ms->max;
    }
  d->hostIndexMax = ms->max;
  return MG_OK;
}

MgStatus mgDevGet (Modset *ms, MgDev **out, hipStream_t st)
{
  MgStatus s = mgEnsureDevice (); if (s) return s;
  if (!ms || !ms->hasher) { mgSetError ("null Modset"); return MG_ERR_ARG; }
  if ((s = mgCheckHasher (ms->hasher))) return s;
  MgDev *d = mgDevLookup (ms);
  if (!d)
    { d = new MgDev (); d->built = false; d->hostIndexMax = 0; d->hPin = 0;
      if (hipGetDevice (&d->device) != hipSuccess) { delete d; return mgHipFail (hipGetLastError (), "hipGetDevice"); }
      if (hipHostMalloc ((void **) &d->hPin, 256, hipHostMallocDefault) != hipSuccess) { delete d; return mgHipFail (hipGetLastError (), "hipHostMalloc"); }
      if ((s = mgDevBuild (ms, d, st))) { mgDevFree (d); return s; }
      mgXferWarm ();
      std::lock_guard<std::mutex> g (gRegLock); gReg[ms] = d; mgLiveDeviceModsets = (int) gReg.size ();
    }
  else if ((s = mgDevOnCallersGpu (d))) return s;
  if (d->built && ms->max > d->t.max)
    {
      U32 first = d->t.max + 1, last = ms->max;
      if (last >= (ms->tableSize >> 2)) { mgSetError ("modset max %u beyond table capacity", last); return MG_ERR_CAPACITY; }
      MG_HIP (hipMemcpyAsync (d->t.value + first, ms->value + first, (size_t) (last - first + 1) * sizeof (U64), hipMemcpyHostToDevice, st));
      MG_HIP (hipMemcpyAsync (d->t.baseDepth + first, ms->depth + first, (size_t) (last - first + 1) * sizeof (U16), hipMemcpyHostToDevice, st));
      d->t.baseZero = false;
      if (!d->ticketsOut && (s = mgTableEnsure (&d->t, last - first + 1, st))) return s;
      if ((s = mgTableLoadHost (&d->t, d->t.value, first, last, st))) return s;
      MG_HIP (hipStreamSynchronize (st));
      d->t.max = d->t.syncedMax = last;
      if (d->hostIndexMax == first - 1) d->hostIndexMax = last;
    }
  d->t.size = ms->size;
  *out = d;
  return MG_OK;
}

extern "C" MgStatus mgModsetDeviceRelease (Modset *ms)
{
  MgDev *d = mgDevLookup (ms);
  if (!d) return MG_OK;
  MgStatus s = modsetSyncToHost (ms, 1);
  mgDevDrop (ms, d);
  return s;
}

extern "C" void mgModsetHostChanged (Modset *ms)
{
  MgDev *d = mgDevLookup (ms);
  if (d) mgDevDrop (ms, d);
}

extern "C" MgStatus mgModsetClear (Modset *ms, void *stream)
{
  hipStream_t st = (hipStream_t) stream;
  MgDev *d = mgDevLookup (ms);
  if (d) { MgStatus s = mgDevOnCallersGpu (d); if (s) return s; }
  U32 hostIndexed = d ? d->hostIndexMax : ms->max;
  U32 hostUsed = d ? d->t.syncedMax : ms->max;
  if (d)
    { MgTable &t = d->t;
      mgTableForget (&t, st);
      if (!t.baseZero) MG_HIP (hipMemsetAsync (t.baseDepth, 0, ((size_t) (t.max > t.syncedMax ? t.max : t.syncedMax) + 1) * sizeof (U16), st));
      t.baseZero = true;
      t.max = t.syncedMax = 0;
      t.pendingDepth = false;
      d->hostIndexMax = 0;
    }
  if (hostIndexed) memset (ms->index, 0, ms->tableSize * sizeof (U32));
  if (hostUsed)
    { memset (ms->depth, 0, ((size_t) hostUsed + 1) * sizeof (U16));
      memset (ms->info, 0, (size_t) hostUsed + 1);
    }
  ms->max = 0;
  return MG_OK;
}


static MgStatus mgFoldCounts (MgDev *d, hipStream_t st, Modset *host = 0)
{
  MgTable &t = d->t;
  if (!t.max) return MG_OK;
  if (!t.pendingDepth) return MG_OK;
  MgStatus s = d->arena.reserve (mgAl256 ((size_t) t.max * sizeof (U16)) + 4096); if (s) return s;
  d->arena.reset ();
  U16 *dDelta = (U16 *) d->arena.take ((size_t) t.max * sizeof (U16));
  s = mgTableExportDepth (&t, dDelta, st);
  MG_HIP (hipStreamSynchronize (st));
  if (!s && host) s = mgXferD2H (host->depth + 1, dDelta, (size_t) t.max * sizeof (U16), MG_XFER_SATADD16);
  return s;
}

static int mgMergeDeviceCore (Modset *ms1, MgDev *d, const U64 *dV2, const U16 *dD2, const U8 *dI2, U32 n2, hipStream_t st)
{
  MgTable &t = d->t;
  const U32 max1 = t.max;
  const char *const sorry = "device merge failed";
  MgDevScratch scratch ("device merge");
  U8 *dI1; U32 *dIdx;
  const size_t cap1 = (size_t) max1 + n2 + 2;
  if (scratch.get (&dI1, cap1) || scratch.get (&dIdx, n2)) return -1;
  if (hipMemset (dI1, 0, cap1) || hipDeviceSynchronize ()) return mgFailedWith (sorry);
  if (mgXferH2D (dI1, ms1->info, (size_t) max1 + 1)) return mgFailedWith (sorry);
  MgStatus as = mgAddBatch (ms1, d, dV2, n2, dIdx, 0, false, st);
  if (as == MG_ERR_CAPACITY) { fprintf (stderr, "FATAL ERROR: %s\n", mgLastError ()); exit (-1); }
  if (as) return mgFailedWith (sorry);
  t.baseZero = false; t.liveHistValid = false;
  if (mgTableMergeApply (dIdx, dD2, dI2, n2, t.baseDepth, dI1, st)) return mgFailedWith (sorry);
  if (hipStreamSynchronize (st)) return mgFailedWith (sorry);
  if (t.max > t.syncedMax)
    { if (mgXferD2H (ms1->value + t.syncedMax + 1, t.value + t.syncedMax + 1, (size_t) (t.max - t.syncedMax) * 8, MG_XFER_COPY)) return mgFailedWith (sorry);
      t.syncedMax = t.max;
    }
  if (mgXferD2H (ms1->depth, t.baseDepth, ((size_t) t.max + 1) * 2, MG_XFER_COPY)) return mgFailedWith (sorry);
  if (mgXferD2H (ms1->info, dI1, (size_t) t.max + 1, MG_XFER_COPY)) return mgFailedWith (sorry);
  ms1->depth[0] = 0;
  ms1->max = t.max;
  return 0;
}

extern "C" int mgHookMergeDevice (Modset *ms1, Modset *ms2)
{
  hipStream_t st = 0;
  MgDev *d; if (mgDevGet (ms1, &d, st)) return -1;
  const U32 n2 = ms2->max;
  if (mgFoldCounts (d, st)) return -1;
  if (!n2) return 0;
  MgDevScratch scratch ("device merge: the second set");
  U64 *dV2; U16 *dD2; U8 *dI2;
  if (scratch.get (&dV2, n2) || scratch.get (&dD2, n2) || scratch.get (&dI2, n2)) return -1;
  if (mgXferH2D (dV2, ms2->value + 1, (size_t) n2 * 8) || mgXferH2D (dD2, ms2->depth + 1, (size_t) n2 * 2) || mgXferH2D (dI2, ms2->info + 1, n2)) return mgFailedWith ("device merge failed");
  return mgMergeDeviceCore (ms1, d, dV2, dD2, dI2, n2, st);
}

extern "C" int mgHookMergeDeviceArrays (Modset *ms1, const U64 *dValue2, const U16 *dDepth2, const U8 *dInfo2, U32 n2)
{
  hipStream_t st = 0;
  MgDev *d; if (mgDevGet (ms1, &d, st)) return -1;
  if (mgFoldCounts (d, st)) return -1;
  if (!n2) return 0;
  return mgMergeDeviceCore (ms1, d, dValue2, dDepth2, dInfo2, n2, st);
}

extern "C" int mgHookPruneDevice (Modset *ms, int lo, int hi)
{
  hipStream_t st = 0;
  MgDev *d; if (mgDevGet (ms, &d, st)) return -1;
  MgTable &t = d->t;
  const U32 n = t.max;
  if (mgFoldCounts (d, st)) return -1;
  const char *const sorry = "device prune failed";
  MgDevScratch scratch ("device prune");
  U8 *dInfo, *dNewInfo; U64 *dNewValue; U16 *dNewDepth; char *dWork;
  if (scratch.get (&dInfo, (size_t) n + 1) || scratch.get (&dNewInfo, (size_t) n + 2) || scratch.get (&dNewValue, (size_t) n + 2)
      || scratch.get (&dNewDepth, (size_t) n + 2) || scratch.get (&dWork, mgTablePruneScratchBytes (n ? n : 1))) return -1;
  if (mgXferH2D (dInfo, ms->info, (size_t) n + 1)) return mgFailedWith (sorry);
  if (mgTablePrune (&t, dInfo, lo, hi, dNewValue, dNewDepth, dNewInfo, dWork, st)) return mgFailedWith (sorry);
  U64 c[2];
  if (hipMemcpyAsync (c, t.counters, 16, hipMemcpyDeviceToHost, st) || hipStreamSynchronize (st)) return mgFailedWith (sorry);
  const U32 m = (U32) c[0];
  if (m)
    { t.baseZero = false; t.liveHistValid = false;
      if (hipMemcpy (t.value + 1, dNewValue + 1, (size_t) m * 8, hipMemcpyDeviceToDevice) || hipMemcpy (t.baseDepth + 1, dNewDepth + 1, (size_t) m * 2, hipMemcpyDeviceToDevice)
          || mgXferD2H (ms->value + 1, dNewValue + 1, (size_t) m * 8, MG_XFER_COPY) || mgXferD2H (ms->depth + 1, dNewDepth + 1, (size_t) m * 2, MG_XFER_COPY)
          || mgXferD2H (ms->info + 1, dNewInfo + 1, m, MG_XFER_COPY)) return mgFailedWith (sorry);
    }
  if (n > m && hipMemset (t.baseDepth + m + 1, 0, (size_t) (n - m) * 2)) return mgFailedWith (sorry);
  mgTableForget (&t, st);
  t.max = 0;
  if (mgTableEnsure (&t, m, st)) return mgFailedWith (sorry);
  if (m && mgTableLoadHost (&t, t.value, 1, m, st)) return mgFailedWith (sorry);
  if (hipStreamSynchronize (st)) return mgFailedWith (sorry);
  t.max = t.syncedMax = m;
  ms->max = m;
  d->hostIndexMax = 0;
  return 0;
}

extern "C" void mgHookDestroy (Modset *ms) { mgModsetHostChanged (ms); }
extern "C" void mgHookHostRewrote (Modset *ms) { mgModsetHostChanged (ms); }
extern "C" void mgHookNeedHostAll (Modset *ms, int wantIndex)
{
  MgDev *d = mgDevLookup (ms);
  if (!d) return;
  if (modsetSyncToHost (ms, wantIndex) != MG_OK)
    { fprintf (stderr, "FATAL ERROR: %s\n", mgLastError ()); exit (-1); }
}
extern "C" void mgHookNeedHost (Modset *ms, int wantIndex)
{
  MgDev *d = mgDevLookup (ms);
  if (!d) return;
  if (!d->t.pendingDepth && d->t.syncedMax == d->t.max && (!wantIndex || d->hostIndexMax >= d->t.max)) return;
  mgHookNeedHostAll (ms, wantIndex);
}
extern "C" int mgHookHasDevice (Modset *ms) { return mgDevLookup (ms) != 0; }


U64 mgAddChunkSize (void)
{
  const long c = mgKnobs ()->addChunk;
  U64 v = c != MG_KNOB_UNSET && c > 0 ? (U64) c : ((U64) 1 << 30);
  if (v > ((U64) 1 << 30)) v = (U64) 1 << 30;
  return v;
}

static MgStatus mgAddChunk (Modset *ms, MgDev *d, const U64 *dKmer, U64 n, U32 *dIndexOut, int withDepth,
                            void *scratch, hipStream_t st, const MgHistReq *counted = 0, const MgSegSrc *segSrc = 0)
{
  MgTable &t = d->t;
  MgStatus s;
  MG_HIP (hipMemsetAsync (t.counters, 0, 16, st));
  if ((s = mgTableAdd (&t, dKmer, n, withDepth, scratch, st, counted, segSrc))) return s;
  volatile U64 *c = d->hPin;
  MG_HIP (hipMemcpyAsync (d->hPin, t.counters, 16, hipMemcpyDeviceToHost, st));
  MG_HIP (hipStreamSynchronize (st));
  U64 newMax = (U64) t.max + c[0];
  if (c[1] || newMax >= t.size)
    {
      if ((s = mgTableRollback (&t, st))) return s;
      mgSetError ("hashTableSize %u is too small for %llu", t.size, (unsigned long long) newMax);
      return MG_ERR_CAPACITY;
    }
  t.max = (U32) newMax;
  ms->max = t.max;
  if (n >= 4096) t.newPct = (int) (c[0] * 100 / n);
  if (dIndexOut && (s = mgTableFind (&t, dKmer, n, dIndexOut, st))) return s;
  return MG_OK;
}

MgStatus mgAddBatch (Modset *ms, MgDev *d, const U64 *dKmer, U64 n, U32 *dIndexOut, int withDepth,
                     bool arenaLive, hipStream_t st, const MgHistReq *counted, const MgSegSrc *segSrc)
{
  if (!n) return MG_OK;
  MgStatus s = mgDevRefuseInFlight (d); if (s) return s;
  U64 chunk = n < MG_ADD_CHUNK ? n : MG_ADD_CHUNK;
  if ((s = mgTableEnsure (&d->t, chunk, st))) return s;
  size_t need = mgTableAddScratchBytes (&d->t, chunk) + 4096;
  if (!arenaLive)
    { if ((s = d->arena.reserve (need))) return s;
      d->arena.reset ();
    }
  else if (d->arena.bytes - d->arena.used < need)
    { mgSetError ("internal: arena too small for insert temporaries"); return MG_ERR_NOMEM; }
  void *scratch = d->arena.take (mgTableAddScratchBytes (&d->t, chunk));
  for (U64 off = 0 ; off < n && !s ; off += chunk)
    { U64 m = n - off < chunk ? n - off : chunk;
      if (off) s = mgTableEnsure (&d->t, m, st);
      if (!s) s = mgAddChunk (ms, d, dKmer + off, m, dIndexOut ? dIndexOut + off : 0, withDepth, scratch, st,
                              (counted && n <= chunk) ? counted : 0,
                              n <= chunk ? segSrc : 0);
    }
  return s;
}

extern "C" MgStatus modsetAddBatchDevice (Modset *ms, const U64 *dKmer, U64 n, U32 *dIndexOut, int withDepth, void *stream)
{
  hipStream_t st = (hipStream_t) stream;
  MgDev *d; MgStatus s = mgDevGet (ms, &d, st); if (s) return s;
  return mgAddBatch (ms, d, dKmer, n, dIndexOut, withDepth, false, st);
}

extern "C" MgStatus modsetFindBatchDevice (Modset *ms, const U64 *dKmer, U64 n, U32 *dIndexOut, void *stream)
{
  hipStream_t st = (hipStream_t) stream;
  MgDev *d; MgStatus s = mgDevGet (ms, &d, st); if (s) return s;
  d->t.loadPct = MG_LOOKUP_LOAD_PCT;
  if (d->t.slots && (s = mgTableEnsure (&d->t, 0, st))) return s;
  return mgTableFind (&d->t, dKmer, n, dIndexOut, st);
}

extern "C" MgStatus modsetSyncToHost (Modset *ms, int wantIndex)
{
  MgDev *d = mgDevLookup (ms);
  if (!d) return MG_OK;
  MgOnDevice here (d->device);
  MgTable &t = d->t;
  hipStream_t st = 0;
  MgStatus s;
  MG_HIP (hipDeviceSynchronize ());
  if (d->ticketsOut && (t.pendingDepth || (wantIndex && d->hostIndexMax < t.max)))
    { mgSetError ("a query batch of this modset is in flight (its scratch is what a sync would use)"); return MG_ERR_ARG; }
  if (t.max > t.syncedMax)
    { const U32 first = t.syncedMax + 1;
      if ((s = mgXferD2H (ms->value + first, t.value + first, (size_t) (t.max - first + 1) * sizeof (U64), MG_XFER_COPY))) return s;
      t.syncedMax = t.max;
    }
  ms->max = t.max;
  if ((s = mgFoldCounts (d, st, ms))) return s;
  if (wantIndex && d->hostIndexMax < t.max)
    { if ((s = d->arena.reserve (mgAl256 (ms->tableSize * sizeof (U32)) + 4096))) return s;
      d->arena.reset ();
      U32 *dIndex = (U32 *) d->arena.take (ms->tableSize * sizeof (U32));
      if ((s = mgTableReplayIndex (&t, mgMakeParams (ms->hasher), ms->tableBits, dIndex, st))) return s;
      MG_HIP (hipStreamSynchronize (st));
      if ((s = mgXferD2H (ms->index, dIndex, ms->tableSize * sizeof (U32), MG_XFER_COPY))) return s;
      d->hostIndexMax = t.max;
    }
  return MG_OK;
}

extern "C" MgStatus mgModsetAdoptDepthDevice (Modset *ms, const U16 *dDepth16)
{
  MgDev *d = mgDevLookup (ms);
  if (!d || !d->built) return MG_OK;
  MgTable &t = d->t;
  if (t.pendingDepth || t.max != ms->max) { mgModsetHostChanged (ms); return MG_OK; }
  MG_HIP (hipMemcpy (t.baseDepth, dDepth16, ((size_t) t.max + 1) * sizeof (U16), hipMemcpyDeviceToDevice));
  t.baseZero = false; t.liveHistValid = false;
  return MG_OK;
}

extern "C" int mgHookDeviceView (Modset *ms, const U64 **dValue1, const U16 **dDepth1, U32 *max)
{
  MgDev *d = mgDevLookup (ms);
  if (!d || !d->built || d->ticketsOut) return -1;
  if (mgDevOnCallersGpu (d, true)) return -1;
  if (hipDeviceSynchronize () != hipSuccess || mgFoldCounts (d, 0, ms)) return -1;
  *dValue1 = d->t.value + 1; *dDepth1 = d->t.baseDepth + 1; *max = d->t.max;
  return 0;
}

extern "C" int mgHookDeviceViewMake (Modset *ms, const U64 **dValue1, const U16 **dDepth1, U32 *max)
{
  MgDev *d; if (mgDevGet (ms, &d, 0)) return -1;
  return mgHookDeviceView (ms, dValue1, dDepth1, max);
}

extern "C" U64 mgModsetDeviceSlots (Modset *ms) { MgDev *d = mgDevLookup (ms); return d && d->built ? d->t.nSlots : 0; }

extern "C" MgStatus mgTableCheckLayout (Modset *ms, U64 *out6)
{
  MgDev *d; MgStatus s = mgDevGet (ms, &d, 0); if (s) return s;
  MgDevScratch scratch ("mgTableCheckLayout");
  U64 *dOut;
  if (scratch.get (&dOut, 4)) return MG_ERR_HIP;
  s = mgTableLayoutCheck (&d->t, dOut, 0);
  if (!s && (hipMemcpy (out6, dOut, 32, hipMemcpyDeviceToHost) || hipMemcpy (out6 + 4, d->t.counters + 4, 16, hipMemcpyDeviceToHost))) s = MG_ERR_HIP;
  return s;
}

extern "C" MgStatus mgTableDiag (Modset *ms, U64 *out9)
{
  memset (out9, 0, 9 * sizeof (U64));
  MgDev *d = mgDevLookup (ms);
  if (!d || !d->built) return MG_OK;
  out9[0] = (U64) d->t.log2NB; out9[1] = d->t.R;
  for (int i = 0 ; i < 7 ; ++i) out9[2 + i] = d->t.diag[i];
  return MG_OK;
}

extern "C" MgStatus modsetDepthHistogramDevice (Modset *ms, U64 *dHist, void *stream)
{
  hipStream_t st = (hipStream_t) stream;
  MgDev *d; MgStatus s = mgDevGet (ms, &d, st); if (s) return s;
  return mgTableHistogram (&d->t, dHist, st);
}

MgStatus mgModsetTableForPass (Modset *ms, MgTable **t)
{
  *t = 0;
  if (!ms) { mgSetError ("null Modset"); return MG_ERR_ARG; }
  if (!mgDevLookup (ms)) return MG_OK;
  MgDev *d; MgStatus s = mgDevGet (ms, &d, 0); if (s) return s;
  if (!d->built) return MG_OK;
  if ((s = mgDevRefuseInFlight (d))) return s;
  MG_HIP (hipDeviceSynchronize ());
  ms->max = d->t.max;
  *t = &d->t;
  return MG_OK;
}
```

modimizer_amd/csrc/mg_reads.hip:

```cpp
#include "mg_api_int.h"

struct MgScanBufs { U64 *kmer; U32 *posF; U32 *rid; void *work; U64 *count; U64 cap; MgHistReq counted;
                    MgSegSrc seg; bool lazy; void *findScratch, *findScratch2; };

struct MgScanReq { const Seqhash *sh; const U32 *dPacked; U64 totalBases; const U64 *dReadOffsets; U32 nReads; bool wantPos; size_t extraPerSurvivor;
                   U32 *outPosF, *outRid; U64 outCap; bool lazy; };
static inline MgArena &mgArenaOf (MgDev *d, int slot) { return slot ? d->arena2 : d->arena; }
static inline U64 *mgCountPin (MgDev *d, int slot) { return d->hPin + 8 + 8 * slot; }

static MgStatus mgScanStart (MgDev *d, int slot, const MgScanReq &q, U64 cap, MgScanBufs *b, hipStream_t st)
{
  b->lazy = false; b->seg.nSegs = 0; b->seg.segKmer = 0; b->findScratch = 0; b->findScratch2 = 0;
  MgArena &ar = mgArenaOf (d, slot);
  const long fp = mgKnobs ()->findPath;
  const bool lookupHist = q.lazy && q.wantPos && !q.extraPerSurvivor && d->t.slots && fp != 'd'
                          && (fp == 'p' || fp == '2' || (cap >= ((U64) 1 << 24) && d->t.nSlots >= ((U64) 1 << 24) && d->t.log2NB > 9));
  const bool lookup2 = lookupHist && fp != 'p';
  MgHashParams p = mgMakeParams (q.sh);
  const size_t perS = 8 + (q.wantPos ? 8 : 0) + q.extraPerSurvivor;
  const size_t need = mgAl256 (cap * perS) + 4 * 4096 + 512 * MG_HIST_STRIDE * 4 + mgAl256 (mgScanWorkBytes (q.totalBases, q.nReads, cap))
                      + (q.extraPerSurvivor ? mgTableAddScratchBytes (&d->t, cap < MG_ADD_CHUNK ? cap : MG_ADD_CHUNK) + 8192 : 0) + 8 * 256
                      + (lookupHist ? mgTableFindPartScratchBytes (cap) + 8192 : 0) + (lookup2 ? mgTableFindPart2ScratchBytes (cap) + 8192 : 0);
  MgStatus s = ar.reserve (need); if (s) return s;
  ar.reset ();
  b->cap = cap;
  b->kmer = (U64 *) ar.take (cap * 8);
  const bool direct = q.wantPos && q.outPosF && q.outRid && q.outCap >= cap;
  b->posF = !q.wantPos ? 0 : (direct ? q.outPosF : (U32 *) ar.take (cap * 4));
  b->rid = !q.wantPos ? 0 : (direct ? q.outRid : (U32 *) ar.take (cap * 4));
  b->work = ar.take (mgScanWorkBytes (q.totalBases, q.nReads, cap));
  b->count = (U64 *) ar.take (8 * MG_COUNT_WORDS);
  b->counted.log2NB = 0; b->counted.kbits = 64; b->counted.binCount = 0; b->counted.hiB = 0;
  if (q.extraPerSurvivor || lookupHist)
    { b->counted.binCount = (U32 *) ar.take (512 * MG_HIST_STRIDE * sizeof (U32));
      b->counted.log2NB = d->t.log2NB; b->counted.kbits = d->t.kbits;
      if (lookupHist) b->counted.hiB = mgTableFindDigitBits (&d->t);
    }
  b->findScratch = lookupHist ? ar.take (mgTableFindPartScratchBytes (cap)) : 0;
  b->findScratch2 = lookup2 ? ar.take (mgTableFindPart2ScratchBytes (cap)) : 0;
  const bool lz = q.lazy && (q.wantPos ? q.extraPerSurvivor == 0 : b->counted.binCount != 0);
  if ((s = mgLaunchScan (p, q.dPacked, q.totalBases, q.dReadOffsets, q.nReads, b->kmer, b->posF, b->rid, cap, b->count, b->work, st,
                         b->counted.binCount ? &b->counted : 0, lz ? &b->seg : 0))) return s;
  b->lazy = lz;
  MG_HIP (hipMemcpyAsync (mgCountPin (d, slot), b->count, MG_COUNT_WORDS * sizeof (U64), hipMemcpyDeviceToHost, st));
  return MG_OK;
}
static MgStatus mgScanFinish (MgDev *d, int slot, const MgScanBufs *b, U64 *nOut, U64 *retryCap, hipStream_t st, hipEvent_t done = 0)
{
  if (done) MG_HIP (hipEventSynchronize (done));
  else MG_HIP (hipStreamSynchronize (st));
  *retryCap = mgScanRetryCap (mgCountPin (d, slot), b->cap, nOut);
  return MG_OK;
}

static MgStatus mgScanRounds (MgDev *d, int slot, const MgScanReq &q, U64 cap, MgScanBufs *b, U64 *nOut, hipStream_t st, hipEvent_t started = 0)
{
  for (int round = 0 ; round < 3 ; ++round)
    { MgStatus s;
      const bool running = started && !round;
      if (!running && (s = mgScanStart (d, slot, q, cap, b, st))) return s;
      if ((s = mgScanFinish (d, slot, b, nOut, &cap, st, running ? started : 0))) return s;
      if (!cap) return MG_OK;
    }
  mgSetError ("scan capacity could not be established");
  return MG_ERR_CAPACITY;
}

static MgStatus mgScanIntoArena (MgDev *d, const Seqhash *sh, const U32 *dPacked, U64 totalBases,
                                 const U64 *dReadOffsets, U32 nReads, bool wantPos, size_t extraPerSurvivor,
                                 MgScanBufs *b, U64 *nOut, hipStream_t st,
                                 U32 *outPosF = 0, U32 *outRid = 0, U64 outCap = 0, bool lazy = false)
{
  MgStatus s = mgDevRefuseInFlight (d); if (s) return s;
  MgScanReq q = { sh, dPacked, totalBases, dReadOffsets, nReads, wantPos, extraPerSurvivor, outPosF, outRid, outCap, lazy };
  if (extraPerSurvivor)
    {
      U64 expect = totalBases / (U64) (sh->w > 0 ? sh->w : 1) + 1;
      if (expect > MG_ADD_CHUNK) expect = MG_ADD_CHUNK;
      if ((s = mgTableEnsure (&d->t, expect, st))) return s;
    }
  return mgScanRounds (d, 0, q, mgSurvivorGuess (sh, totalBases), b, nOut, st);
}

extern "C" MgStatus mgAddReadsDevice (Modset *ms, const U32 *dPacked, U64 totalBases,
                                      const U64 *dReadOffsets, U32 nReads, U64 *nHash, void *stream)
{
  hipStream_t st = (hipStream_t) stream;
  MgDev *d; MgStatus s = mgDevGet (ms, &d, st); if (s) return s;
  if (nHash) *nHash = 0;
  if (!totalBases || !nReads) return MG_OK;
  MgScanBufs b; U64 n = 0;
  d->t.loadPct = 75;
  if ((s = mgScanIntoArena (d, ms->hasher, dPacked, totalBases, dReadOffsets, nReads, false, 4, &b, &n, st, 0, 0, 0, true))) return s;
  if (nHash) *nHash = n;
  if (!n) return MG_OK;
  if (b.lazy)
    { const U64 chunk = n < MG_ADD_CHUNK ? n : MG_ADD_CHUNK;
      if ((s = mgTableEnsure (&d->t, chunk, st))) return s;
      if (n <= MG_ADD_CHUNK && mgTableAddTakesSegments (&d->t, n, &b.counted))
        return mgAddBatch (ms, d, 0, n, 0, 1, true, st, &b.counted, &b.seg);
      if ((s = mgLaunchSegCompact (b.seg, b.kmer, b.cap, b.count, st))) return s;
    }
  return mgAddBatch (ms, d, b.kmer, n, 0, 1, true, st, &b.counted);
}

static MgStatus mgSeedsOfScanned (Modset *ms, MgDev *d, MgScanBufs &b, U64 n, U32 *dSeedIndex, U32 *dSeedPosF, U32 *dSeedRead, U64 capacity, hipStream_t st)
{
  if (n > capacity)
    { mgSetError ("%llu seeds exceed the caller's capacity %llu", (unsigned long long) n, (unsigned long long) capacity); return MG_ERR_CAPACITY; }
  MgStatus s;
  if (ms) s = mgAddBatch (ms, d, b.kmer, n, dSeedIndex, 0, true, st, &b.counted);
  else if (b.lazy && b.findScratch && mgTableFindTakesPartition (&d->t, n, &b.counted))
    s = mgTableFindPartitioned (&d->t, b.seg, n, &b.counted, dSeedIndex, b.kmer, b.findScratch, st, b.findScratch2);
  else s = b.lazy ? mgTableFindSegments (&d->t, b.seg, n, dSeedIndex, st) : mgTableFind (&d->t, b.kmer, n, dSeedIndex, st);
  if (s) return s;
  if (dSeedPosF && b.posF != dSeedPosF) MG_HIP (hipMemcpyAsync (dSeedPosF, b.posF, n * 4, hipMemcpyDeviceToDevice, st));
  if (dSeedRead && b.rid != dSeedRead) MG_HIP (hipMemcpyAsync (dSeedRead, b.rid, n * 4, hipMemcpyDeviceToDevice, st));
  MG_HIP (hipStreamSynchronize (st));
  return MG_OK;
}

static MgStatus mgSeedReads (Modset *ms, const Seqhash *scanWith, int mode, const U32 *dPacked, U64 totalBases,
                             const U64 *dReadOffsets, U32 nReads,
                             U32 *dSeedIndex, U32 *dSeedPosF, U32 *dSeedRead, U64 capacity,
                             U64 *nSeeds, hipStream_t st)
{
  MgDev *d; MgStatus s = mgDevGet (ms, &d, st); if (s) return s;
  if (nSeeds) *nSeeds = 0;
  if (!scanWith) scanWith = ms->hasher;
  if ((s = mgCheckHasher (scanWith))) return s;
  if (scanWith->k != ms->hasher->k) { mgSetError ("a batch scanned with k %d cannot be looked up in a set of k %d", scanWith->k, ms->hasher->k); return MG_ERR_ARG; }
  if (!totalBases || !nReads) return MG_OK;
  MgScanBufs b; U64 n = 0;
  d->t.loadPct = MG_LOOKUP_LOAD_PCT;
  if (mode == 0 && d->t.slots && (s = mgTableEnsure (&d->t, 0, st))) return s;
  const int timing = mgKnobs ()->seedTiming == 1;
  struct timespec q0, q1, q2; if (timing) clock_gettime (CLOCK_MONOTONIC, &q0);
  if ((s = mgScanIntoArena (d, scanWith, dPacked, totalBases, dReadOffsets, nReads, true, mode ? 4 : 0, &b, &n, st,
                            dSeedPosF, dSeedRead, capacity, mode == 0))) return s;
  if (timing) clock_gettime (CLOCK_MONOTONIC, &q1);
  if (nSeeds) *nSeeds = n;
  if ((s = mgSeedsOfScanned (mode ? ms : 0, d, b, n, dSeedIndex, dSeedPosF, dSeedRead, capacity, st))) return s;
  if (timing)
    { clock_gettime (CLOCK_MONOTONIC, &q2);
      fprintf (stderr, "mgSeedReads: scan+count %.2f ms, lookup+sync %.2f ms\n", (q1.tv_sec - q0.tv_sec) * 1e3 + (q1.tv_nsec - q0.tv_nsec) * 1e-6,
               (q2.tv_sec - q1.tv_sec) * 1e3 + (q2.tv_nsec - q1.tv_nsec) * 1e-6);
    }
  return MG_OK;
}

extern "C" MgStatus mgQueryReadsDevice (Modset *ms, const U32 *dPacked, U64 totalBases,
                                        const U64 *dReadOffsets, U32 nReads,
                                        U32 *dSeedIndex, U32 *dSeedPosF, U32 *dSeedRead, U64 capacity,
                                        U64 *nSeeds, void *stream)
{ return mgSeedReads (ms, 0, 0, dPacked, totalBases, dReadOffsets, nReads, dSeedIndex, dSeedPosF, dSeedRead, capacity, nSeeds, (hipStream_t) stream); }

extern "C" MgStatus mgInsertReadsDevice (Modset *ms, const U32 *dPacked, U64 totalBases,
                                         const U64 *dReadOffsets, U32 nReads,
                                         U32 *dSeedIndex, U32 *dSeedPosF, U32 *dSeedRead, U64 capacity,
                                         U64 *nSeeds, void *stream)
{ return mgSeedReads (ms, 0, 1, dPacked, totalBases, dReadOffsets, nReads, dSeedIndex, dSeedPosF, dSeedRead, capacity, nSeeds, (hipStream_t) stream); }

extern "C" void mgSeedBufsFree (MgSeedBufs *bufs)
{
  (void) hipFree (bufs->ix); (void) hipFree (bufs->posF); (void) hipFree (bufs->rid);
  bufs->ix = bufs->posF = bufs->rid = 0; bufs->cap = 0;
}
static MgStatus mgSeedBufsReserve (MgSeedBufs *bufs, U64 need)
{
  if (bufs->cap >= need) return MG_OK;
  mgSeedBufsFree (bufs);
  const U64 room = need + need * (U64) bufs->sparePct / 100 + 1;
  U32 **arr[3] = { &bufs->ix, &bufs->posF, &bufs->rid };
  for (int j = 0 ; j < 3 ; ++j)
    { const hipError_t e = hipMalloc ((void **) arr[j], room * sizeof (U32));
      if (e != hipSuccess) { *arr[j] = 0; mgSeedBufsFree (bufs); return mgHipFail (e, "a batch's seed arrays"); }
    }
  bufs->cap = room; return MG_OK;
}
extern "C" MgStatus mgSeedsOfBatch (Modset *ms, const Seqhash *scanWith, int insert, const U32 *dPacked, U64 totalBases, const U64 *dReadOffsets, U32 nReads,
                                    U64 guess, MgSeedBufs *bufs, U64 *nSeeds, void *stream)
{
  const bool empty = !totalBases || !nReads;
  U64 offer = empty ? 0 : (guess < totalBases + 1 ? guess : totalBases + 1);
  *nSeeds = 0;
  for (int attempt = 0 ; ; ++attempt)
    { MgStatus s = mgSeedBufsReserve (bufs, offer); if (s) return s;
      s = mgSeedReads (ms, scanWith, insert ? 1 : 0, dPacked, totalBases, dReadOffsets, nReads, bufs->ix, bufs->posF, bufs->rid, offer, nSeeds, (hipStream_t) stream);
      if (s != MG_ERR_CAPACITY || attempt || *nSeeds <= offer) return s;
      offer = *nSeeds;
    }
}

struct MgQueryTicket { Modset *ms; MgDev *d; int slot; MgScanReq q; MgScanBufs b; U32 *dSeedIndex, *dSeedPosF, *dSeedRead; U64 capacity; };

extern "C" MgStatus mgQueryReadsDeviceAsync (Modset *ms, const U32 *dPacked, U64 totalBases, const U64 *dReadOffsets, U32 nReads,
                                             U32 *dSeedIndex, U32 *dSeedPosF, U32 *dSeedRead, U64 capacity, void **ticket, void *stream)
{
  hipStream_t st = (hipStream_t) stream;
  if (!ticket) { mgSetError ("mgQueryReadsDeviceAsync: null ticket"); return MG_ERR_ARG; }
  *ticket = 0;
  MgDev *d; MgStatus s = mgDevGet (ms, &d, st); if (s) return s;
  if (d->ticketsOut >= 2) { mgSetError ("two query batches are in flight already"); return MG_ERR_ARG; }
  d->t.loadPct = MG_LOOKUP_LOAD_PCT;
  if (d->t.slots && !d->ticketsOut && (s = mgTableEnsure (&d->t, 0, st))) return s;
  if (!d->side)
    {
      int lo = 0, hi = 0; (void) hipDeviceGetStreamPriorityRange (&lo, &hi);
      MG_HIP (hipStreamCreateWithPriority (&d->side, hipStreamNonBlocking, lo));
      for (int i = 0 ; i < 2 ; ++i) MG_HIP (hipEventCreateWithFlags (&d->scanned[i], hipEventDisableTiming));
      MG_HIP (hipEventCreateWithFlags (&d->inputReady, hipEventDisableTiming));
    }
  const int slot = d->slotBusy[d->nextSlot] ? d->nextSlot ^ 1 : d->nextSlot;
  MgQueryTicket *t = new MgQueryTicket ();
  t->ms = ms; t->d = d; t->slot = slot; t->dSeedIndex = dSeedIndex; t->dSeedPosF = dSeedPosF; t->dSeedRead = dSeedRead; t->capacity = capacity;
  t->q = MgScanReq { ms->hasher, dPacked, totalBases, dReadOffsets, nReads, true, 0, dSeedPosF, dSeedRead, capacity, true };
  t->b = MgScanBufs (); t->b.cap = 0;
  if (totalBases && nReads)
    {
      hipError_t e = hipEventRecord (d->inputReady, st);
      if (e == hipSuccess) e = hipStreamWaitEvent (d->side, d->inputReady, 0);
      if (e != hipSuccess) { delete t; return mgHipFail (e, "mgQueryReadsDeviceAsync"); }
      if ((s = mgScanStart (d, slot, t->q, mgSurvivorGuess (ms->hasher, totalBases), &t->b, d->side))) { delete t; return s; }
      if ((e = hipEventRecord (d->scanned[slot], d->side)) != hipSuccess) { delete t; return mgHipFail (e, "mgQueryReadsDeviceAsync"); }
    }
  d->slotBusy[slot] = true; d->nextSlot = slot ^ 1; ++d->ticketsOut;
  *ticket = t;
  return MG_OK;
}

extern "C" MgStatus mgQueryReadsDeviceWait (void *ticket, U64 *nSeeds, void *stream)
{
  MgQueryTicket *t = (MgQueryTicket *) ticket;
  if (!t) { mgSetError ("mgQueryReadsDeviceWait: null ticket"); return MG_ERR_ARG; }
  MgDev *d = t->d;
  if (nSeeds) *nSeeds = 0;
  MgStatus s = MG_OK;
  U64 n = 0;
  if (t->q.totalBases && t->q.nReads && !(s = mgScanRounds (d, t->slot, t->q, t->b.cap, &t->b, &n, d->side, d->scanned[t->slot])))
    { if (nSeeds) *nSeeds = n;
      s = mgSeedsOfScanned (0, d, t->b, n, t->dSeedIndex, t->dSeedPosF, t->dSeedRead, t->capacity, (hipStream_t) stream);
    }
  d->slotBusy[t->slot] = false; --d->ticketsOut;
  delete t;
  return s;
}
```

modimizer_amd/csrc/mg_runtime.hip:

```cpp
#include <stdarg.h>
#include "mg_api_int.h"
#include "mg_xfer.h"


static thread_local char gErr[512] = "";

void mgSetError (const char *fmt, ...)
{ va_list ap; va_start (ap, fmt); vsnprintf (gErr, sizeof (gErr), fmt, ap); va_end (ap); }

extern "C" const char *mgLastError (void) { return gErr; }

MgStatus mgHipFail (hipError_t e, const char *what)
{ mgSetError ("HIP error %d (%s) in %s", (int) e, hipGetErrorString (e), what); return MG_ERR_HIP; }

extern "C" int mgDeviceCount (void)
{ int n = 0; if (hipGetDeviceCount (&n) != hipSuccess) { (void) hipGetLastError (); return 0; } return n; }

MgStatus mgEnsureDevice (void)
{
  static int known = -1;
  if (known < 0) known = mgDeviceCount ();
  if (known <= 0)
    { mgSetError ("no HIP device available: libmodgpu has no CPU fallback for the batch path");
      return MG_ERR_NO_DEVICE;
    }
  return MG_OK;
}

extern "C" MgStatus mgSetDevice (int device)
{ MgStatus s = mgEnsureDevice (); if (s) return s; MG_HIP (hipSetDevice (device)); return MG_OK; }

extern "C" MgStatus mgDeviceAlloc (void **dptr, size_t bytes)
{ MgStatus s = mgEnsureDevice (); if (s) return s; MG_HIP (hipMalloc (dptr, bytes ? bytes : 16)); return MG_OK; }
extern "C" MgStatus mgDeviceFree (void *dptr) { if (dptr) MG_HIP (hipFree (dptr)); return MG_OK; }
extern "C" MgStatus mgMemcpyH2D (void *dst, const void *src, size_t bytes, void *stream)
{ if (bytes) MG_HIP (hipMemcpyAsync (dst, src, bytes, hipMemcpyHostToDevice, (hipStream_t) stream)); return MG_OK; }
extern "C" MgStatus mgMemcpyD2H (void *dst, const void *src, size_t bytes, void *stream)
{ if (bytes) MG_HIP (hipMemcpyAsync (dst, src, bytes, hipMemcpyDeviceToHost, (hipStream_t) stream));
  MG_HIP (hipStreamSynchronize ((hipStream_t) stream)); return MG_OK; }
extern "C" void *mgPinnedAlloc (size_t bytes)
{ void *p = 0; if (mgEnsureDevice () || hipHostMalloc (&p, bytes ? bytes : 16, hipHostMallocPortable | hipHostMallocMapped) != hipSuccess) { (void) hipGetLastError (); return 0; } return p; }
extern "C" void mgPinnedFree (void *p) { if (p) (void) hipHostFree (p); }
__global__ void mgCopyOutKernel (const U64 *__restrict__ src, U64 *__restrict__ dstHost, U64 nWords)
{ for (U64 i = (U64) blockIdx.x * blockDim.x + threadIdx.x ; i < nWords ; i += (U64) gridDim.x * blockDim.x) dstHost[i] = src[i]; }
extern "C" MgStatus mgCopyOutPinned (void *dstPinned, const void *srcDev, size_t bytes, void *stream)
{
  if (!bytes) return MG_OK;
  void *dDst = 0;
  if ((bytes & 7) || ((uintptr_t) dstPinned & 7) || ((uintptr_t) srcDev & 7) || hipHostGetDevicePointer (&dDst, dstPinned, 0) != hipSuccess)
    { (void) hipGetLastError (); return mgMemcpyD2H (dstPinned, srcDev, bytes, stream); }
  const U64 nWords = bytes >> 3;
  unsigned grid = (unsigned) ((nWords + 255) / 256); if (grid > 2048) grid = 2048;
  hipLaunchKernelGGL (mgCopyOutKernel, dim3 (grid), dim3 (256), 0, (hipStream_t) stream, (const U64 *) srcDev, (U64 *) dDst, nWords);
  MG_HIP (hipGetLastError ());
  MG_HIP (hipStreamSynchronize ((hipStream_t) stream));
  return MG_OK;
}
extern "C" MgStatus mgMemsetD (void *dst, int byte, size_t bytes, void *stream)
{ if (bytes) MG_HIP (hipMemsetAsync (dst, byte, bytes, (hipStream_t) stream)); return MG_OK; }
extern "C" MgStatus mgStreamSynchronize (void *stream)
{ MG_HIP (hipStreamSynchronize ((hipStream_t) stream)); return MG_OK; }


static const char *gKernelNames[MG_K_COUNT] = {
  "mgPackKernel", "mgUnpackKernel", "mgTileInfoKernel", "mgScanKernel", "mgTableInsertKernel",
  "mgRankAssignKernel", "mgDirectFlagKernel", "mgTableFindKernel", "mgTableLoadKernel",
  "mgTableExportDepthKernel", "mgTableHistKernel", "mgReplayIndexKernel", "mgIndexFinishKernel",
  "mgSynthGenomeKernel", "mgSynthReadsKernel", "memset", "mgSegScanKernel", "mgSegCompactKernel",
  "mgPartChunks+ScanKernel", "mgPartHistKernel", "mgPartScatterKernel", "mgRankCountKernel", "mgRankScanKernel", "mgBucketDedupKernel",
  "mgBucketMergeKernel", "mgRankLookupKernel", "mgTableFindSegKernel", "mgHotPlan+ReduceKernel", "mgBucketFindKernel", "mgUnpartKernel", "mgChainKernel", "mgChainResolveKernel",
  "mgPaintItemsKernel", "mgDepthGuardKernel", "mgDepthGatherKernel", "mgTextLenKernel", "mgTextScanKernel", "mgTextWriteKernel",
  "mgSetTextLinesKernel", "mgSetTextScanKernel", "mgSetTextParseKernel", "mgSetTextLastKernel",
  "mgOvElem..TableKernels", "mgOvEmitKernel", "overlap sorts", "mgOvHead..PairInitKernels", "mgOvPairKernel",
  "mgTrimSkip+OffsetsKernel", "mgTrimGatherKernel", "mgSetCopyKernel", "mgCopyTallyKernel" };
#define MG_PROF_POOL 8192
struct MgProfRec { int id; hipEvent_t a, b; };
static struct {
  bool on = false;
  int only = -1;
  MgProfRec rec[MG_PROF_POOL]; int used = 0, made = 0;
  double ms[MG_K_COUNT] = { 0 }; U64 n[MG_K_COUNT] = { 0 };
  int open = -1;
} gProf;

static void mgProfDrain (void)
{
  if (!gProf.used) return;
  (void) hipDeviceSynchronize ();
  for (int i = 0 ; i < gProf.used ; ++i)
    { float t = 0;
      if (hipEventElapsedTime (&t, gProf.rec[i].a, gProf.rec[i].b) == hipSuccess)
        { gProf.ms[gProf.rec[i].id] += t; ++gProf.n[gProf.rec[i].id]; }
    }
  gProf.used = 0;
}

void mgProfBegin (int id, hipStream_t st)
{
  if (!gProf.on || (gProf.only >= 0 && id != gProf.only)) return;
  if (gProf.used == MG_PROF_POOL) mgProfDrain ();
  MgProfRec &r = gProf.rec[gProf.used];
  if (gProf.used >= gProf.made)
    { if (hipEventCreate (&r.a) != hipSuccess || hipEventCreate (&r.b) != hipSuccess) { gProf.on = false; return; }
      gProf.made = gProf.used + 1;
    }
  r.id = id;
  (void) hipEventRecord (r.a, st);
  gProf.open = gProf.used;
}

void mgProfEnd (int id, hipStream_t st)
{
  if (!gProf.on || gProf.open < 0) return;
  (void) id;
  (void) hipEventRecord (gProf.rec[gProf.open].b, st);
  gProf.used = gProf.open + 1;
  gProf.open = -1;
}

extern "C" void mgProfileEnable (int on) { if (!on) mgProfDrain (); gProf.on = on != 0; }
extern "C" void mgProfileOnly (int kernelId) { mgProfDrain (); gProf.only = (kernelId >= 0 && kernelId < MG_K_COUNT) ? kernelId : -1; }
extern "C" void mgProfileReset (void)
{ mgProfDrain (); for (int i = 0 ; i < MG_K_COUNT ; ++i) { gProf.ms[i] = 0; gProf.n[i] = 0; } }
extern "C" int mgProfileKernels (void) { return MG_K_COUNT; }
extern "C" MgStatus mgProfileGet (int id, const char **name, double *totalMs, U64 *launches)
{
  if (id < 0 || id >= MG_K_COUNT) { mgSetError ("bad kernel id"); return MG_ERR_ARG; }
  mgProfDrain ();
  if (name) *name = gKernelNames[id];
  if (totalMs) *totalMs = gProf.ms[id];
  if (launches) *launches = gProf.n[id];
  return MG_OK;
}


MgHashParams mgMakeParams (const Seqhash *sh)
{
  MgHashParams p;
  p.factor1 = sh->factor1; p.mask = sh->mask; p.k = sh->k; p.shift1 = sh->shift1;
  p.d = (U32) sh->w;
  p.dShift = __builtin_ctz (p.d);
  U64 odd = (U64) (p.d >> p.dShift);
  U64 x = odd;
  for (int i = 0 ; i < 6 ; ++i) x *= 2 - odd * x;
  p.dOddInv = x;
  p.dOddLim = ~(U64) 0 / odd;
  p.small32 = (2 * sh->k <= 40 && odd < ((U64) 1 << 15)) ? 1u : 0u;
  p.c24 = (U32) (((U64) 1 << 24) % odd); p.inv32 = (U32) x; p.lim32 = (U32) (0xffffffffull / odd);
  return p;
}

MgStatus mgCheckHasher (const Seqhash *sh)
{
  if (!sh || sh->k < 1 || sh->k >= 32 || sh->w < 1 || sh->shift1 != 64 - 2 * sh->k)
    { mgSetError ("invalid Seqhash (k %d w %d)", sh ? sh->k : -1, sh ? sh->w : -1); return MG_ERR_ARG; }
  return MG_OK;
}


extern "C" size_t mgPackedWords (U64 nBases) { return (size_t) ((nBases + 15) / 16) + MG_PACK_PAD; }

extern "C" MgStatus mgPackDevice (const U8 *dBases, U64 nBases, U32 *dWords, void *stream)
{ MgStatus s = mgEnsureDevice (); if (s) return s; return mgLaunchPack (dBases, nBases, dWords, (hipStream_t) stream); }
extern "C" MgStatus mgUnpackDevice (const U32 *dWords, U64 nBases, U8 *dBases, void *stream)
{ MgStatus s = mgEnsureDevice (); if (s) return s; return mgLaunchUnpack (dWords, nBases, dBases, (hipStream_t) stream); }

extern "C" MgStatus mgSynthGenome (U32 *dPacked, U64 nBases, U64 seed, void *stream)
{ MgStatus s = mgEnsureDevice (); if (s) return s; return mgLaunchSynthGenome (dPacked, nBases, seed, (hipStream_t) stream); }

extern "C" MgStatus mgSynthReads (const U32 *dGenomePacked, U64 genomeBases,
                                  const U64 *dReadStart, const U64 *dReadOffsets, const U8 *dStrand, U32 nReads,
                                  U64 totalBases, double errRate, U64 seed, U32 *dPackedOut, void *stream)
{ MgStatus s = mgEnsureDevice (); if (s) return s;
  return mgLaunchSynthReads (dGenomePacked, genomeBases, dReadStart, dReadOffsets, dStrand, nReads, totalBases,
                             errRate, seed, dPackedOut, (hipStream_t) stream);
}

extern "C" void mgReleaseBuffers (void)
{
  mgSeqReleaseBuffers ();
  mgTextReleaseBuffers ();
  mgQueryReleaseBuffers ();
  mgHostBatchRelease ();
  mgIterReleaseBuffers ();
  mgXferReleaseBuffers ();
  mgUploadRelease ();
}
```

modimizer_amd/csrc/mg_table.hip:

```cpp
#include "mg_table.h"


__global__ void mgTableInsertKernel (MgSlot *__restrict__ slots, MgGeom g, const U64 *__restrict__ kmer, U64 n,
                                     U32 *__restrict__ slotId, int withDepth, U64 *counters)
{
  U64 o = (U64) blockIdx.x * blockDim.x + threadIdx.x;
  const U64 stride = (U64) gridDim.x * blockDim.x;
  for ( ; o < n ; o += stride)
    { const U64 m = mgMixK (kmer[o], g.kbits), key = m + 1;
      const U64 base = (U64) mgBucketOfM (m, g) * g.R;
      U32 at = mgHomeOfM (m, g);
      bool ok = false;
      for (U32 probes = 0 ; probes < g.R ; ++probes)
        { U64 cur = slots[base + at].key;
          if (cur == 0)
            { cur = atomicCAS ((unsigned long long *) &slots[base + at].key, 0ull, (unsigned long long) key);
              if (cur == 0) cur = key;
            }
          if (cur == key) { ok = true; break; }
          at = mgNextSlot (at, g.R);
        }
      if (!ok) { counters[1] = 1; slotId[o] = 0xffffffffu; continue; }
      const U64 s = base + at;
      U32 v = slots[s].ord;
      U32 tok = mgToken (o);
      if (v < tok) atomicMax (&slots[s].ord, tok);
      if (withDepth)
        {
          const U64 s0 = ((U64) (U32) __builtin_amdgcn_readfirstlane ((int) (U32) (s >> 32)) << 32) | (U32) __builtin_amdgcn_readfirstlane ((int) (U32) s);
          const bool mine = s == s0;
          const U64 grp = __ballot (mine);
          if (!mine) atomicAdd (&slots[s].cnt, 1u);
          else if ((threadIdx.x & 63) == (U32) __builtin_ctzll (grp)) atomicAdd (&slots[s].cnt, (U32) __popcll (grp));
        }
      slotId[o] = (U32) s;
    }
}


__global__ __launch_bounds__ (256)
void mgDirectFlagKernel (const MgSlot *__restrict__ slots, const U32 *__restrict__ slotId, U64 n,
                         unsigned char *__restrict__ flags)
{
  U64 o = (U64) blockIdx.x * blockDim.x + threadIdx.x;
  const U64 stride = (U64) gridDim.x * blockDim.x;
  for ( ; o < n ; o += stride)
    { U32 s = slotId[o];
      flags[o] = (s != 0xffffffffu && slots[s].ord == mgToken (o)) ? 1 : 0;
    }
}


__global__ __launch_bounds__ (256)
void mgRankCountKernel (const unsigned char *__restrict__ flags, U64 n, U64 rowsPerUnit, U64 *__restrict__ unitCount)
{
  MG_BUILD_PRIO ();
  const int lane = threadIdx.x & 63;
  const U64 unit = (U64) blockIdx.x * 4 + (threadIdx.x >> 6);
  const U64 nRows = (n + 63) / 64;
  U64 row = unit * rowsPerUnit, rEnd = row + rowsPerUnit;
  if (rEnd > nRows) rEnd = nRows;
  U32 c = 0;
  if ((reinterpret_cast<uintptr_t> (flags) & 15) == 0)
    for ( ; row + 64 <= rEnd && (row + 64) * 64 <= n ; row += 64)
      { uint4 q[4];
#pragma unroll
        for (int j = 0 ; j < 4 ; ++j) q[j] = *reinterpret_cast<const uint4 *> (flags + (row + 16 * j) * 64 + (U64) lane * 16);
#pragma unroll
        for (int j = 0 ; j < 4 ; ++j)
          c += (U32) __popc (q[j].x & 0x01010101u) + (U32) __popc (q[j].y & 0x01010101u) + (U32) __popc (q[j].z & 0x01010101u) + (U32) __popc (q[j].w & 0x01010101u);
      }
  for ( ; row + 4 <= rEnd ; row += 4)
    { U32 v[4];
#pragma unroll
      for (int j = 0 ; j < 4 ; ++j) { U64 o = (row + j) * 64 + lane; v[j] = (o < n) ? (flags[o] & 1) : 0; }
      c += v[0] + v[1] + v[2] + v[3];
    }
  for ( ; row < rEnd ; ++row) { U64 o = row * 64 + lane; c += (o < n) ? (flags[o] & 1) : 0; }
  c = mgWaveReduce<MgSum> (c);
  if (lane == 0) unitCount[unit] = c;
}

#define MG_RANK_ROWS 8
template <bool DIRECT, bool SEG>
__global__ __launch_bounds__ (256)
void mgRankAssignKernel (const unsigned char *__restrict__ flags, const U64 *__restrict__ kmer, const MgSegSrc src, const MgSubSeg *__restrict__ subSeg,
                         U64 n, U64 rowsPerUnit,
                         const U64 *__restrict__ unitBase, U32 baseMax, U32 size,
                         U64 *__restrict__ value, MgSlot *__restrict__ slots, const U32 *__restrict__ slotId,
                         MgRankGrp *__restrict__ grp)
{
  MG_BUILD_PRIO ();
  const int lane = threadIdx.x & 63;
  const U64 unit = (U64) blockIdx.x * 4 + (U32) __builtin_amdgcn_readfirstlane ((int) (threadIdx.x >> 6));
  const U64 nRows = (n + 63) / 64;
  U64 row = unit * rowsPerUnit, rEnd = row + rowsPerUnit;
  if (rEnd > nRows) rEnd = nRows;
  if (row >= rEnd) return;
  U64 run = unitBase[unit];
  const U64 below = ((U64) 1 << lane) - 1;
  MgSegCursor cur; cur.w = 0; cur.s0 = 0; cur.s1 = 0;
  if (SEG) { mgSegCursorFrom (subSeg, row * 64 / MG_PART_SUB, &cur); mgSegCursorSeek (src, &cur, row * 64); }
  for ( ; row < rEnd ; row += MG_RANK_ROWS)
    { bool f[MG_RANK_ROWS]; U64 km[MG_RANK_ROWS]; U32 fl[MG_RANK_ROWS];
#pragma unroll
      for (int j = 0 ; j < MG_RANK_ROWS ; ++j)
        { const U64 o = (row + j) * 64 + lane;
          const bool in = (row + j < rEnd) && (o < n);
          fl[j] = flags[in ? o : 0];
        }
#pragma unroll
      for (int j = 0 ; j < MG_RANK_ROWS ; ++j)
        { const U64 o = (row + j) * 64 + lane;
          const bool in = (row + j < rEnd) && (o < n);
          if (SEG)
            { km[j] = 0;
              if ((row + j) * 64 < n && row + j < rEnd)
                { const U64 o0 = (row + j) * 64, last = o0 + 63 < n ? o0 + 63 : n - 1;
                  mgSegCursorSeek (src, &cur, o0);
                  const U64 *at = mgSegAddr (src, cur, o, last);
                  if (in) km[j] = __builtin_nontemporal_load (at);
                }
            }
          else km[j] = in ? __builtin_nontemporal_load (&kmer[o]) : 0;
        }
#pragma unroll
      for (int j = 0 ; j < MG_RANK_ROWS ; ++j)
        { const U64 o = (row + j) * 64 + lane;
          f[j] = (row + j < rEnd) && (o < n) && (fl[j] & 1);
          asm volatile ("" : "+v" (km[j]));
        }
#pragma unroll
      for (int j = 0 ; j < MG_RANK_ROWS ; ++j)
        { if (row + j >= rEnd) break;
          const U64 o = (row + j) * 64 + lane;
          const U64 bits = __ballot (f[j]);
          if (!DIRECT && lane == 0) { MgRankGrp g; g.bits = bits; g.rank = (U32) run; g.pad = 0; grp[row + j] = g; }
          if (f[j])
            { U64 idx = (U64) baseMax + 1 + run + (U32) __popcll (bits & below);
              if (idx < size)
                { __builtin_nontemporal_store (km[j], &value[idx]);
                  if (DIRECT) slots[slotId[o]].ord = (U32) idx | MG_ASSIGNED;
                }
            }
          run += (U32) __popcll (bits);
        }
    }
}

__global__ void mgTableLoadKernel (MgSlot *__restrict__ slots, MgGeom g, const U64 *__restrict__ value,
                                   U32 first, U32 last, U32 *__restrict__ occ, U64 *counters)
{
  U64 i = (U64) first + (U64) blockIdx.x * blockDim.x + threadIdx.x;
  const U64 stride = (U64) gridDim.x * blockDim.x;
  for ( ; i <= last ; i += stride)
    { const U64 m = mgMixK (value[i], g.kbits), key = m + 1;
      const U32 b = mgBucketOfM (m, g);
      const U64 base = (U64) b * g.R;
      U32 at = mgHomeOfM (m, g);
      bool placed = false, dup = false;
      for (U32 probes = 0 ; probes < g.R ; ++probes)
        { U64 cur = slots[base + at].key;
          if (cur == 0)
            { cur = atomicCAS ((unsigned long long *) &slots[base + at].key, 0ull, (unsigned long long) key);
              if (cur == 0) { placed = true; break; }
            }
          if (cur == key) { dup = true; break; }
          at = mgNextSlot (at, g.R);
        }
      if (placed) { slots[base + at].ord = (U32) i | MG_ASSIGNED; atomicAdd (&occ[b], 1u); }
      else if (!dup) counters[1] = 1;
    }
}


__global__ void mgTableExportDepthKernel (MgSlot *__restrict__ slots, U32 nBuckets, const U32 *__restrict__ occ, U32 R,
                                          U16 *__restrict__ baseDepth, U16 *__restrict__ delta, U32 max)
{
  for (U32 bk = blockIdx.x ; bk < nBuckets ; bk += gridDim.x)
    { if (!occ[bk]) continue;
      MgSlot *base = slots + (U64) bk * R;
      for (U32 i = threadIdx.x ; i < R ; i += blockDim.x)
        { uint4 v = *reinterpret_cast<const uint4 *> (&base[i]);
          if (!(v.x | v.y) || !mgIsAssigned (v.z)) continue;
          U32 idx = v.z & ~MG_ASSIGNED, c = v.w;
          if (idx > max) continue;
          U32 cl = c > 0xffffu ? 0xffffu : c;
          delta[idx - 1] = (U16) cl;
          U32 b = (U32) baseDepth[idx] + cl;
          baseDepth[idx] = (U16) (b > 0xffffu ? 0xffffu : b);
          if (c) base[i].cnt = 0;
        }
    }
}

#define MG_HIST_LDS_BINS 8192
__global__ __launch_bounds__ (256)
void mgTableHistKernel (const MgSlot *__restrict__ slots, U32 nBuckets, const U32 *__restrict__ occ, U32 R,
                        const U16 *__restrict__ baseDepth, unsigned long long *__restrict__ hist)
{
  __shared__ U32 sBins[MG_HIST_LDS_BINS];
  for (int b = threadIdx.x ; b < MG_HIST_LDS_BINS ; b += blockDim.x) sBins[b] = 0;
  __syncthreads ();
  const int lane = threadIdx.x & 63;
  U32 n1 = 0, n2 = 0;
  for (U32 bk = blockIdx.x ; bk < nBuckets ; bk += gridDim.x)
    { if (!occ[bk]) continue;
      const MgSlot *base = slots + (U64) bk * R;
      for (U32 i0 = 0 ; i0 < R ; i0 += 4 * blockDim.x)
        { uint4 v[4];
#pragma unroll
          for (int j = 0 ; j < 4 ; ++j)
            { const U32 i = i0 + j * blockDim.x + threadIdx.x;
              v[j] = i < R ? *reinterpret_cast<const uint4 *> (&base[i]) : make_uint4 (0, 0, 0, 0);
            }
#pragma unroll
          for (int j = 0 ; j < 4 ; ++j)
            { U32 d = 0; bool have = false;
              if ((v[j].x | v[j].y) && mgIsAssigned (v[j].z))
                { U32 idx = v[j].z & ~MG_ASSIGNED;
                  d = (baseDepth ? (U32) baseDepth[idx] : 0u) + v[j].w;
                  if (d > 0xffffu || d < v[j].w) d = 0xffffu;
                  have = true;
                }
              n1 += (U32) __popcll (__ballot (have && d == 1));
              n2 += (U32) __popcll (__ballot (have && d == 2));
              if (have && d != 1 && d != 2)
                { if (d < MG_HIST_LDS_BINS) atomicAdd (&sBins[d], 1u);
                  else atomicAdd (&hist[d], 1ull);
                }
            }
        }
    }
  if (lane == 0) { if (n1) atomicAdd (&sBins[1], n1); if (n2) atomicAdd (&sBins[2], n2); }
  __syncthreads ();
  for (int b = threadIdx.x ; b < MG_HIST_LDS_BINS ; b += blockDim.x)
    if (sBins[b]) atomicAdd (&hist[b], (unsigned long long) sBins[b]);
}

__global__ void mgReplayIndexKernel (const U64 *__restrict__ value, U32 max, U64 factor1, int shift1,
                                     int tableBits, U32 *__restrict__ index)
{
  const U64 tmask = ((U64) 1 << tableBits) - 1;
  U64 i = 1 + (U64) blockIdx.x * blockDim.x + threadIdx.x;
  const U64 stride = (U64) gridDim.x * blockDim.x;
  for ( ; i <= max ; i += stride)
    { U32 cur = (U32) i;
      U64 hash = (value[cur] * factor1) >> shift1;
      U64 off = hash & tmask;
      U64 diff = ((hash >> tableBits) & tmask) | 1;
      for (;;)
        { U32 prev = atomicMin (&index[off], cur);
          if (prev == 0xffffffffu) break;
          if (prev > cur)
            { cur = prev;
              hash = (value[cur] * factor1) >> shift1;
              diff = ((hash >> tableBits) & tmask) | 1;
            }
          off = (off + diff) & tmask;
        }
    }
}

__global__ void mgIndexFinishKernel (U32 *__restrict__ index, U64 n)
{
  U64 i = (U64) blockIdx.x * blockDim.x + threadIdx.x;
  const U64 stride = (U64) gridDim.x * blockDim.x;
  for ( ; i < n ; i += stride) if (index[i] == 0xffffffffu) index[i] = 0;
}


static inline int mgLog2 (U64 x) { int l = 0; while (((U64) 1 << l) < x) ++l; return l; }

MgPartFmt mgPartFmtOf (const MgTable *t, U64 n, int hiB)
{ MgPartFmt f; f.ordBits = mgLog2 (n) > 1 ? mgLog2 (n) : 1; f.remBits = t->kbits - hiB; f.loB = t->log2NB - hiB; return f; }
bool mgPartFmtFits (const MgTable *t, const MgPartFmt &f) { return t->kbits >= t->log2NB + 4 && f.remBits + f.ordBits <= 64; }


static MgStatus mgReadOverflow (MgTable *t, hipStream_t st, U64 *over)
{
  if (t->pin)
    { MG_HIP (hipMemcpyAsync (t->pin + 3, t->counters + 1, 8, hipMemcpyDeviceToHost, st));
      MG_HIP (hipStreamSynchronize (st));
      *over = t->pin[3];
    }
  else
    { MG_HIP (hipStreamSynchronize (st));
      MG_HIP (hipMemcpy (over, t->counters + 1, 8, hipMemcpyDeviceToHost));
    }
  return MG_OK;
}

__global__ __launch_bounds__ (256)
void mgCleanEmptyBucketsKernel (MgSlot *__restrict__ slots, MgGeom g, const U32 *__restrict__ occ, U32 nBuckets)
{
  const uint4 z = make_uint4 (0, 0, 0, 0);
  for (U32 b = blockIdx.x ; b < nBuckets ; b += gridDim.x)
    { if (occ[b]) continue;
// ... 242 lines not shown
  MgOldTable o; mgTableTakeOld (t, &o);
  MgStatus s = MG_OK;
  for (int attempt = 0 ; attempt < 2 ; ++attempt)
    { if (attempt == 0 && exact) { t->log2NB = exactLg; t->R = exactR; t->nSlots = (U64) exactR << exactLg; }
      else if (attempt == 0) mgSetGeometry (t, want);
      else
        { int lg = 0; U32 R = 0;
          U32 *dFine = 0;
          if (hipMalloc ((void **) &dFine, sizeof (U32) << MG_FINE_LOG2) != hipSuccess) { s = mgHipFail (hipGetLastError (), "hipMalloc"); break; }
          if (hipMemsetAsync (dFine, 0, sizeof (U32) << MG_FINE_LOG2, st) != hipSuccess) { s = mgHipFail (hipGetLastError (), "hipMemsetAsync"); (void) hipFree (dFine); break; }
          const U32 oldNB = (U32) 1 << o.log2NB;
          MG_LAUNCH (MG_K_TABLE_HIST, st, mgFineCountSlotsKernel, dim3 (oldNB < 8192 ? oldNB : 8192), dim3 (256), 0, st, o.slots, oldNB, o.occ, o.R, t->kbits, keepMax, dFine);
          s = mgFitGeometry (t, dFine, want, &lg, &R, st);
          (void) hipFree (dFine);
          if (s) break;
          t->log2NB = lg; t->R = R; t->nSlots = (U64) R << lg;
        }
      if ((s = mgTableAllocGeom (t, st))) break;
      U64 over = 0;
      if ((s = mgRehashPass (t, o, keepMax, st, &over))) break;
      if (!over)
        { MG_HIP (hipFree (o.slots)); MG_HIP (hipFree (o.occ));
          t->empty = false; ++t->version;
          return MG_OK;
        }
      (void) hipFree (t->slots); (void) hipFree (t->occ);
      t->slots = 0; t->occ = 0; t->capSlots = 0; t->capNB = 0;
      if (attempt) { mgSetError ("internal: the device table's fitted geometry (2^%d x %u) does not hold its entries", t->log2NB, t->R); s = MG_ERR_CAPACITY; }
    }
  mgTablePutOld (t, o, st);
  return s;
}
static MgStatus mgTableRehashTo (MgTable *t, U64 want, hipStream_t st) { return mgTableRehash (t, want, false, 0, 0, 0x7fffffffu, st); }
static MgStatus mgTableRehashExact (MgTable *t, int log2NB, U32 R, hipStream_t st) { return mgTableRehash (t, (U64) R << log2NB, true, log2NB, R, 0x7fffffffu, st); }

MgStatus mgTableRollback (MgTable *t, hipStream_t st)
{
  t->liveHistValid = false;
  if (!t->slots) return MG_OK;
  return mgTableRehash (t, t->nSlots, true, t->log2NB, t->R, t->max, st);
}

MgStatus mgTableEnsure (MgTable *t, U64 nIncoming, hipStream_t st)
{
  U64 want = mgSlotsFor (t, (U64) t->max + nIncoming);
  if (t->slots && want <= t->nSlots) return MG_OK;
  if (!t->slots || !t->max) return mgTableAlloc (t, want, st);
  if (nIncoming && want < 2 * t->nSlots) want = 2 * t->nSlots;
  if (want > ((U64) 1 << t->maxLog2Slots)) want = (U64) 1 << t->maxLog2Slots;
  if (want <= t->nSlots) return MG_OK;
  return mgTableRehashTo (t, want, st);
}


#define MG_RANK_UNITS 8192
static inline U64 mgRankRowsPerUnit (U64 n, U32 *nBlocks)
{
  U64 nRows = (n + 63) / 64;
  U64 per = (nRows + MG_RANK_UNITS - 1) / MG_RANK_UNITS; if (!per) per = 1;
  U64 units = (nRows + per - 1) / per; if (!units) units = 1;
  *nBlocks = (U32) ((units + 3) / 4);
  return per;
}

static void mgHotKnobs (U32 *split, U32 *chunk)
{
  const MgKnobs *k = mgKnobs ();
  U32 a = MG_HOT_SPLIT_DEFAULT, b = MG_HOT_CHUNK_DEFAULT;
  if (k->hotSplit != MG_KNOB_UNSET && k->hotSplit > 0)
    { a = (U32) k->hotSplit; b = k->hotChunk != MG_KNOB_UNSET && k->hotChunk > 0 ? (U32) k->hotChunk : a / 4; }
  if (b < 64) b = 64;
  if (a < b) a = b;
  *split = a; *chunk = b;
}
static U64 mgHotItemsCap (U64 n) { U32 sp, ch; mgHotKnobs (&sp, &ch); return n / ch + n / sp + 16; }


static int mgPathOverride (void)
{
  const long c = mgKnobs ()->tablePath;
  return c == 'd' ? 1 : (c == 'b' ? 2 : 0);
}

bool mgTableUseBuckets (const MgTable *t, U64 n)
{
  int ov = mgPathOverride ();
  if (ov == 1) return false;
  if (ov == 2) return true;
  if (n < 1500000) return false;
  return n >= t->nSlots / 16;
}

bool mgTableAddTakesSegments (const MgTable *t, U64 n, const MgHistReq *counted)
{
  const int off = mgKnobs ()->noSegmentInput == 1;
  return !off && n && mgTableUseBuckets (t, n) && counted && counted->binCount && counted->log2NB == t->log2NB && counted->kbits == t->kbits && !counted->hiB;
}

#define MG_TIGHT_PCT_DEFAULT 70
#define MG_TIGHT_PCT_CLAIMS 50
#define MG_TIGHT_MIN_R 1024u

struct MgAddPlan {
  int hiB, loB;
  MgPartFmt f; bool packed;
  bool digitBytes;
  int markDup, slotShift, place;
  bool tighten; int tightPct;
  int sliceShift; U32 nSlices;
  U32 hotSplit, hotChunk;
};
static void mgAddPlan (const MgTable *t, U64 n, bool wasEmpty, MgAddPlan *p)
{
  const U64 NB = (U64) 1 << t->log2NB;
  mgPartSplit (t->log2NB, &p->hiB, &p->loB);
  p->f = mgPartFmtOf (t, n, p->hiB);
  { const int packEnv = mgKnobs ()->partPacked == MG_KNOB_UNSET ? 1 : (int) mgKnobs ()->partPacked;
    p->packed = packEnv && mgPartFmtFits (t, p->f);
  }
  p->digitBytes = p->loB && p->loB <= 8 && mgKnobs ()->partDigits != 0;
  mgHotKnobs (&p->hotSplit, &p->hotChunk);
  { const int polEnv = mgKnobs ()->flagPolarity == MG_KNOB_UNSET ? -1 : (int) mgKnobs ()->flagPolarity;
    p->markDup = polEnv >= 0 ? (polEnv ? 1 : 0) : (t->newPct > 50 ? 1 : 0);
  }
  const U64 expectNew = t->newPct > 0 ? n * (U64) t->newPct / 100 : n;
  { const int slotEnv = mgKnobs ()->mergeSlots == MG_KNOB_UNSET ? -1 : (int) mgKnobs ()->mergeSlots;
    const bool dense = ((U64) t->max + expectNew) * 2 > t->nSlots;
    p->slotShift = (t->kbits <= MG_SLOT_SHIFT && (slotEnv >= 0 ? slotEnv != 0 : dense)) ? MG_SLOT_SHIFT : 0;
  }
  int tightPct = t->tightPct ? t->tightPct : MG_TIGHT_PCT_CLAIMS;
  { const long tk = mgKnobs ()->tightLoad; if (tk != MG_KNOB_UNSET && tk >= 0 && tk <= 95) tightPct = (int) tk; }
  bool tighten = wasEmpty && tightPct > 0 && t->log2NB > 0 && t->pin;
  if (tighten && mgKnobs ()->tightLoad == MG_KNOB_UNSET)
    tighten = expectNew * 100 / (U64) tightPct < t->nSlots - t->nSlots / 4;
  { const long pk = mgKnobs ()->mergePlace;
    p->place = pk == MG_KNOB_UNSET ? 1 : (pk != 0);
    if (pk == MG_KNOB_UNSET && expectNew / NB * 115 / 100 > (U64) MG_MERGE_PREFETCH * mgBucketThreads (t->R, 0)) p->place = 0;
    if (p->place && wasEmpty) p->slotShift = 0;
    if (p->place && mgKnobs ()->tightLoad == MG_KNOB_UNSET)
      { if (!t->tightPct) tightPct = MG_TIGHT_PCT_DEFAULT;
        tighten = wasEmpty && tightPct > 0 && t->log2NB > 0 && t->pin;
      }
  }
  if (tighten) p->slotShift = 0;
  { p->sliceShift = 22;
    while (p->sliceShift > 16 && ((n - 1) >> p->sliceShift) + 1 < 32) --p->sliceShift;
    if (mgKnobs ()->rankSliceShift != MG_KNOB_UNSET) p->sliceShift = (int) mgKnobs ()->rankSliceShift;
    while (((n - 1) >> p->sliceShift) + 1 > (U64) (MG_RANK_GROUPS - 1)) ++p->sliceShift;
    p->nSlices = (U32) (((n - 1) >> p->sliceShift) + 1);
  }
  p->tighten = tighten; p->tightPct = tightPct;
}

static MgStatus mgAssignIndices (MgTable *t, const unsigned char *flags, const U64 *dKmer, const MgSegSrc *segSrc, const MgSubSeg *subSeg, U64 n,
                                 U64 *unitCount, U64 *unitBase, const U32 *slotId, MgRankGrp *grp, hipStream_t st)
{
  const MgSegSrc noSrc = {};
  U32 nBlocks; const U64 rows = mgRankRowsPerUnit (n, &nBlocks);
  MG_LAUNCH (MG_K_RANK_COUNT, st, mgRankCountKernel, dim3 (nBlocks), dim3 (256), 0, st, flags, n, rows, unitCount);
  MG_LAUNCH (MG_K_RANK_SCAN, st, (mgGroupSumKernel<U64, U64>), dim3 (1), dim3 (MG_GROUP_THREADS), 0, st, unitCount, unitBase, nBlocks * 4, t->counters);
#define MG_ASSIGN(DIRECT, SEG, KMER, SRC, SUB) MG_LAUNCH (MG_K_TABLE_ASSIGN, st, (mgRankAssignKernel<DIRECT, SEG>), dim3 (nBlocks), dim3 (256), 0, st, \
                                                          flags, KMER, SRC, SUB, n, rows, unitBase, t->max, t->size, t->value, t->slots, slotId, grp)
  if (slotId) MG_ASSIGN (true, false, dKmer, noSrc, (const MgSubSeg *) 0);
  else if (segSrc) MG_ASSIGN (false, true, (const U64 *) 0, *segSrc, subSeg);
  else MG_ASSIGN (false, false, dKmer, noSrc, (const MgSubSeg *) 0);
#undef MG_ASSIGN
  return MG_OK;
}

static MgStatus mgAddTighten (MgTable *t, int tightPct, const U32 *uniqCount, U64 *fullest, hipStream_t st)
{
  const U64 NB = (U64) 1 << t->log2NB;
  { MgStatus s = mgUniqStats (uniqCount, (U32) NB, (unsigned long long *) (t->counters + 2), st); if (s) return s; }
  MG_HIP (hipMemcpyAsync (t->pin, t->counters + 1, 24, hipMemcpyDeviceToHost, st));
  MG_HIP (hipStreamSynchronize (st));
  const U64 over = t->pin[0], U = t->pin[1], M = t->pin[2];
  if (over) return MG_OK;
  *fullest = M;
  U64 Rn = (U * 100 / ((U64) NB * (U64) tightPct) + 1 + MG_R_QUANTUM - 1) / MG_R_QUANTUM * MG_R_QUANTUM;
  const U64 Rfit = (M + M / 8 + 16 + MG_R_QUANTUM - 1) / MG_R_QUANTUM * MG_R_QUANTUM;
  if (Rn < Rfit) Rn = Rfit;
  if (Rn < MG_TIGHT_MIN_R) Rn = MG_TIGHT_MIN_R;
  if (Rn < t->R) { t->R = (U32) Rn; t->nSlots = (U64) NB * Rn; }
  return MG_OK;
}

size_t mgTableAddScratchBytes (const MgTable *t, U64 n)
{
  (void) t;
  U64 NB = (U64) 1 << 18;
  size_t rank = mgAl256 (n)  + 2 * mgAl256 ((MG_RANK_UNITS + 8) * 8) + mgAl256 ((n / 64 + 2) * sizeof (MgRankGrp));
  size_t direct = mgAl256 (n * 4);
  size_t part = 2 * (mgAl256 (n * 8) + mgAl256 (n * 4)) + mgAl256 (n * 4)
              + mgAl256 ((NB + 2) * 8) * 3 + mgAl256 ((NB + 2) * 4) * 2 + mgAl256 (((U64) MG_PART_MAXBINS + 2) * 8) * 3 + 2 * mgAl256 ((U64) MG_PART_MAXBINS * 16 * 8 + 4096)
              + mgAl256 ((MG_PART_MAXBINS + 2) * 4) + mgAl256 ((MG_PART_MAXBINS + 2 + n / MG_PART_CHUNK + MG_PART_MAXBINS + 2) * 4)
              + mgAl256 ((size_t) (MG_RANK_GROUPS + 2) * NB * sizeof (unsigned short)) + mgAl256 ((n / MG_PART_SUB + 2) * 24)
              + mgAl256 (mgHotItemsCap (n) * 8) + mgAl256 (mgHotItemsCap (n) * 4) + 256;
  return rank + (direct > part ? direct : part) + 4096;
}

MgStatus mgTableAdd (MgTable *t, const U64 *dKmer, U64 n, int withDepth, void *scratch, hipStream_t st,
                     const MgHistReq *counted, const MgSegSrc *segSrc)
{
  if (!n) return MG_OK;
  if (segSrc && !mgTableAddTakesSegments (t, n, counted)) { mgSetError ("internal: this insert needs the dense k-mers"); return MG_ERR_ARG; }
  t->liveHistValid = false;
  if (withDepth) t->pendingDepth = true;
  const bool wasEmpty = t->empty && t->max == 0;
  t->empty = false; ++t->version;
  MgGeom g = mgGeomOf (t);
  char *wb = (char *) scratch;
  unsigned char *flags = (unsigned char *) wb;       wb += mgAl256 (n);
  U64 *blockCount = (U64 *) wb;                      wb += mgAl256 ((MG_RANK_UNITS + 8) * 8);
  U64 *blockBase = (U64 *) wb;                       wb += mgAl256 ((MG_RANK_UNITS + 8) * 8);
  MgRankGrp *grp = (MgRankGrp *) wb;                 wb += mgAl256 ((n / 64 + 2) * sizeof (MgRankGrp));
  MG_HIP (hipMemsetAsync (blockCount, 0, (MG_RANK_UNITS + 8) * 8, st));

  if (!mgTableUseBuckets (t, n))
    { U32 *slotId = (U32 *) wb;
      { MgStatus cs = mgTableClean (t, st); if (cs) return cs; }
      MG_LAUNCH (MG_K_TABLE_INSERT, st, mgTableInsertKernel, dim3 (mgGridWide (n)), dim3 (256), 0, st, t->slots, g, dKmer, n, slotId, withDepth, t->counters);
      MG_LAUNCH (MG_K_TABLE_FLAG, st, mgDirectFlagKernel, dim3 (mgGridWide (n)), dim3 (256), 0, st, t->slots, slotId, n, flags);
      { MgStatus as = mgAssignIndices (t, flags, dKmer, (const MgSegSrc *) 0, (const MgSubSeg *) 0, n, blockCount, blockBase, slotId, grp, st); if (as) return as; }
      MG_HIP (hipGetLastError ());
      return mgTableMarkOccupied (t, dKmer, n, st);
    }

  const U64 NB = (U64) 1 << t->log2NB;
  U64 *kA = (U64 *) wb;  wb += mgAl256 (n * 8);
  U32 *tA = (U32 *) wb;  wb += mgAl256 (n * 4);
  U64 *kB = (U64 *) wb;  wb += mgAl256 (n * 8);
  U32 *tB = (U32 *) wb;  wb += mgAl256 (n * 4);
  U32 *cB = (U32 *) wb;  wb += mgAl256 (n * 4);
  U64 *fineStart = (U64 *) wb;                wb += mgAl256 ((NB + 2) * 8);
  unsigned long long *fineCursor = (unsigned long long *) wb; wb += mgAl256 ((NB + 2 + (U64) MG_PART_MAXBINS * 16) * 8);
                                 wb += mgAl256 ((NB + 2) * 8);
  U32 *fineCount = (U32 *) wb;                wb += mgAl256 ((NB + 2) * 4);
  U32 *uniqCount = (U32 *) wb;                wb += mgAl256 ((NB + 2) * 4);
  U64 *coarseStart = (U64 *) wb;              wb += mgAl256 (((U64) MG_PART_MAXBINS + 2) * 8);
  unsigned long long *coarseCursor = (unsigned long long *) wb; wb += mgAl256 (((U64) MG_PART_MAXBINS + 2) * 8 * 16);
  U64 *whole = (U64 *) wb;                    wb += mgAl256 (((U64) MG_PART_MAXBINS + 2) * 8);
  U32 *coarseCount = (U32 *) wb;              wb += mgAl256 ((MG_PART_MAXBINS + 2) * 4);
  U32 *chunkBase = (U32 *) wb;                wb += mgAl256 ((MG_PART_MAXBINS + 2 + n / MG_PART_CHUNK + MG_PART_MAXBINS + 2) * 4);
  unsigned short *sliceOff = (unsigned short *) wb;   wb += mgAl256 ((size_t) (MG_RANK_GROUPS + 2) * NB * sizeof (unsigned short));
  MgSubSeg *subSeg = (MgSubSeg *) wb;         wb += mgAl256 ((n / MG_PART_SUB + 2) * sizeof (MgSubSeg));
  U64 *hotItems = (U64 *) wb;                 wb += mgAl256 (mgHotItemsCap (n) * 8);
  U32 *hotBuckets = (U32 *) wb;               wb += mgAl256 (mgHotItemsCap (n) * 4);
  unsigned long long *hotCount = (unsigned long long *) wb; wb += 256;

  MgAddPlan plan;
  mgAddPlan (t, n, wasEmpty, &plan);
  const int hiB = plan.hiB, loB = plan.loB;
  const U32 *pre = (counted && counted->binCount && counted->log2NB == t->log2NB && counted->kbits == t->kbits && !counted->hiB) ? counted->binCount : 0;
  U64 segInit[2] = { 0, n };
  MG_HIP (hipMemcpyAsync (whole, segInit, 16, hipMemcpyHostToDevice, st));
  MgStatus s;
  MgPartPassArgs p1 = {};
  p1.inMode = segSrc ? MG_EL_SEG : MG_EL_DENSE; p1.packed = plan.packed; p1.f = plan.f; p1.kIn = dKmer; p1.n = n; p1.segStart = whole; p1.nSeg = 1;
  p1.nBins = (U32) 1 << hiB; p1.chunkBase = chunkBase; p1.counted = pre; p1.segSrc = segSrc; p1.subSeg = subSeg;
  if (!loB)
    { p1.kOut = kB; p1.tOut = tB; p1.binStart = fineStart; p1.cursor = fineCursor; p1.binCount = fineCount;
      if ((s = mgPartPass (t, p1, st))) return s;
    }
  else
    {
      unsigned char *digits = plan.digitBytes ? reinterpret_cast<unsigned char *> (cB) : 0;
      p1.shift = loB; p1.kOut = kA; p1.tOut = tA; p1.binStart = coarseStart; p1.cursor = coarseCursor; p1.binCount = coarseCount;
      p1.digitOut = digits; p1.nextBins = (U32) 1 << loB;
      if ((s = mgPartPass (t, p1, st))) return s;
      MgPartPassArgs p2 = {};
      p2.inMode = plan.packed ? MG_EL_PACKED : MG_EL_WIDE; p2.packed = plan.packed; p2.f = plan.f; p2.kIn = kA; p2.tIn = tA; p2.n = n; p2.segStart = coarseStart; p2.nSeg = (U32) 1 << hiB;
      p2.nBins = (U32) 1 << loB; p2.kOut = kB; p2.tOut = tB; p2.binStart = fineStart; p2.cursor = fineCursor; p2.binCount = fineCount; p2.chunkBase = chunkBase;
      p2.digitIn = digits;
      if ((s = mgPartPass (t, p2, st))) return s;
    }

  MG_HIP (hipMemsetAsync (flags, plan.markDup ? 1 : 0, n, st));
  MgBucketArgs a;
  a.slots = t->slots; a.g = g; a.nBuckets = (U32) NB; a.bucketStart = fineStart;
  a.pK = kB; a.pT = tB; a.pC = cB; a.uniqCount = uniqCount; a.occ = t->occ; a.flags = flags;
  a.grp = grp; a.baseMax = t->max; a.size = t->size; a.withDepth = withDepth;
  a.markDup = plan.markDup; a.slotShift = plan.slotShift; a.place = plan.place;
  a.sliceShift = plan.sliceShift; a.nSlices = plan.nSlices; a.sliceOff = sliceOff;
  a.hotSplit = plan.hotSplit; a.hotChunk = plan.hotChunk; a.hotItems = hotItems; a.hotCount = hotCount; a.hotBuckets = hotBuckets;
  a.counters = t->counters; a.f = plan.f;
#ifdef MG_ABLATE
  { const long dbg = mgKnobs ()->bucketDebug; a.debug = dbg != MG_KNOB_UNSET ? (int) dbg : 0; }
#endif
  const bool track = t->max == 0 && t->baseZero;
  a.liveHist = 0;
  if (track)
    { if (!t->liveHist) MG_HIP (hipMalloc ((void **) &t->liveHist, 65536 * sizeof (U64)));
      MG_HIP (hipMemsetAsync (t->liveHist, 0, 65536 * sizeof (U64), st));
      a.liveHist = (unsigned long long *) t->liveHist;
    }
  t->liveHistValid = track;
  size_t lds = mgMergeLdsBytes (t->R);
  { const size_t ldsDedup = (size_t) t->R * 16 + MG_RANK_GROUPS * 4; if (ldsDedup > lds) lds = ldsDedup; }
  const int bThreadsEnv = mgKnobs ()->bucketT == MG_KNOB_UNSET ? 0 : (int) mgKnobs ()->bucketT;
  const unsigned bThreads = mgBucketThreads (t->R, bThreadsEnv);
  U32 perBlock;
  const unsigned bGrid = mgBucketGrid (NB, &perBlock);

  if ((s = mgBucketDedup (a, plan.packed, bThreads, bGrid, perBlock, lds, st))) return s;
  U64 fullest = t->R;
  if (plan.tighten)
    { if ((s = mgAddTighten (t, plan.tightPct, uniqCount, &fullest, st))) return s;
      if (t->R != a.g.R) { a.g = mgGeomOf (t); lds = mgMergeLdsBytes (t->R); }
    }
  if ((s = mgAssignIndices (t, flags, dKmer, segSrc, subSeg, n, blockCount, blockBase, (const U32 *) 0, grp, st))) return s;
  if ((s = mgRankLookup (a, st))) return s;
  if ((s = mgBucketMerge (a, fullest, bThreads, bGrid, perBlock, lds, st))) return s;
  MG_HIP (hipGetLastError ());
  return MG_OK;
}

__global__ void mgMarkOccKernel (MgGeom g, const U64 *__restrict__ kmer, U64 n, U32 *__restrict__ occ)
{
  U64 o = (U64) blockIdx.x * blockDim.x + threadIdx.x;
  const U64 stride = (U64) gridDim.x * blockDim.x;
  for ( ; o < n ; o += stride)
    { U32 b = mgBucketOfM (mgMixK (kmer[o], g.kbits), g);
      if (!occ[b]) occ[b] = 1;
    }
}

MgStatus mgTableMarkOccupied (MgTable *t, const U64 *dKmer, U64 n, hipStream_t st)
{
  MG_LAUNCH (MG_K_TABLE_FLAG, st, mgMarkOccKernel, dim3 (mgGridWide (n)), dim3 (256), 0, st, mgGeomOf (t), dKmer, n, t->occ);
  MG_HIP (hipGetLastError ());
  return MG_OK;
}

__global__ __launch_bounds__ (256)
void mgTableCheckLayoutKernel (const MgSlot *__restrict__ slots, MgGeom g, U64 nSlots, unsigned long long *__restrict__ out)
{
  const U64 stride = (U64) gridDim.x * blockDim.x;
  U32 broken = 0, stray = 0, dup = 0, keys = 0;
  for (U64 o = (U64) blockIdx.x * blockDim.x + threadIdx.x ; o < nSlots ; o += stride)
    { const uint4 v = *reinterpret_cast<const uint4 *> (&slots[o]);
      const U64 key = mgKeyOf (v);
      if (!key) continue;
      ++keys;
      const U32 bkt = (U32) (o / g.R), me = (U32) (o - (U64) bkt * g.R);
      const U64 m = key - 1;
      if (mgBucketOfM (m, g) != bkt) { ++stray; continue; }
      const U64 base = (U64) bkt * g.R;
      for (U32 at = mgHomeOfM (m, g) ; at != me ; at = mgNextSlot (at, g.R))
        { const uint4 w = *reinterpret_cast<const uint4 *> (&slots[base + at]);
          const U64 k2 = mgKeyOf (w);
          if (!k2) { ++broken; break; }
          if (k2 == key) { ++dup; break; }
        }
    }
  if (broken) atomicAdd (&out[0], (unsigned long long) broken);
  if (stray) atomicAdd (&out[1], (unsigned long long) stray);
  if (dup) atomicAdd (&out[2], (unsigned long long) dup);
  if (keys) atomicAdd (&out[3], (unsigned long long) keys);
}

MgStatus mgTableLayoutCheck (MgTable *t, U64 *dOut, hipStream_t st)
{
  { MgStatus cs = mgTableClean (t, st); if (cs) return cs; }
  MG_HIP (hipMemsetAsync (dOut, 0, 32, st));
  MG_LAUNCH (MG_K_TABLE_FIND, st, mgTableCheckLayoutKernel, dim3 (mgGridWide (t->nSlots)), dim3 (256), 0, st, t->slots, mgGeomOf (t), t->nSlots, (unsigned long long *) dOut);
  MG_HIP (hipGetLastError ());
  return MG_OK;
}

static MgStatus mgLoadLaunch (MgTable *t, const U64 *dValue, U32 first, U32 last, hipStream_t st, U64 *over)
{
  MG_HIP (hipMemsetAsync (t->counters + 1, 0, 8, st));
  MG_LAUNCH (MG_K_TABLE_LOAD, st, mgTableLoadKernel, dim3 (mgGridWide ((U64) last - first + 1)), dim3 (256), 0, st,
             t->slots, mgGeomOf (t), dValue, first, last, t->occ, t->counters);
  MG_HIP (hipGetLastError ());
  return mgReadOverflow (t, st, over);
}

MgStatus mgTableLoadHost (MgTable *t, const U64 *dValue, U32 first, U32 last, hipStream_t st)
{
  if (last < first) return MG_OK;
  t->liveHistValid = false; t->empty = false; ++t->version;
  { MgStatus cs = mgTableClean (t, st); if (cs) return cs; }
  U64 over = 0;
  MgStatus s = mgLoadLaunch (t, dValue, first, last, st, &over);
  if (s || !over) return s;
  int lg = 0; U32 R = 0;
  U32 *dFine = 0;
  if (hipMalloc ((void **) &dFine, sizeof (U32) << MG_FINE_LOG2) != hipSuccess) return mgHipFail (hipGetLastError (), "hipMalloc");
  if (hipMemsetAsync (dFine, 0, sizeof (U32) << MG_FINE_LOG2, st) != hipSuccess) s = mgHipFail (hipGetLastError (), "hipMemsetAsync");
  else
    { MG_LAUNCH (MG_K_TABLE_HIST, st, mgFineCountValuesKernel, dim3 (mgGridWide (last)), dim3 (256), 0, st, dValue, 1u, last, t->kbits, dFine);
      s = mgFitGeometry (t, dFine, mgSlotsFor (t, last), &lg, &R, st);
    }
  (void) hipFree (dFine);
  if (!s) s = mgTableRehashExact (t, lg, R, st);
  if (s) return s;
  if ((s = mgLoadLaunch (t, dValue, first, last, st, &over))) return s;
  if (over) { mgSetError ("internal: the device table's fitted geometry (2^%d x %u) does not hold the host's entries", lg, R); return MG_ERR_CAPACITY; }
  return MG_OK;
}

MgStatus mgTableExportDepth (MgTable *t, U16 *dDelta, hipStream_t st)
{
  if (!t->max) return MG_OK;
  MG_HIP (hipMemsetAsync (dDelta, 0, (size_t) t->max * sizeof (U16), st));
  t->baseZero = false;
  t->pendingDepth = false;
  t->liveHistValid = false;
  { const U32 NB = (U32) 1 << t->log2NB;
    MG_LAUNCH (MG_K_TABLE_EXPORT, st, mgTableExportDepthKernel, dim3 (NB < 8192 ? NB : 8192), dim3 (256), 0, st,
               t->slots, NB, t->occ, t->R, t->baseDepth, dDelta, t->max);
  }
  MG_HIP (hipGetLastError ());
  return MG_OK;
}

__global__ void mgHistAddKernel (const U64 *__restrict__ live, unsigned long long *__restrict__ hist)
{ U32 i = blockIdx.x * blockDim.x + threadIdx.x; if (i < 65536 && live[i]) atomicAdd (&hist[i], (unsigned long long) live[i]); }

MgStatus mgTableHistogram (MgTable *t, U64 *dHist, hipStream_t st)
{
  if (!t->max) return MG_OK;
  if (t->liveHistValid && t->liveHist)
    { MG_LAUNCH (MG_K_TABLE_HIST, st, mgHistAddKernel, dim3 (256), dim3 (256), 0, st, t->liveHist, (unsigned long long *) dHist);
      MG_HIP (hipGetLastError ());
      return MG_OK;
    }
  { const U32 NB = (U32) 1 << t->log2NB;
    MG_LAUNCH (MG_K_TABLE_HIST, st, mgTableHistKernel, dim3 (NB < 2048 ? NB : 2048), dim3 (256), 0, st,
               t->slots, NB, t->occ, t->R, t->baseZero ? (const U16 *) 0 : t->baseDepth, (unsigned long long *) dHist);
  }
  MG_HIP (hipGetLastError ());
  return MG_OK;
}

MgStatus mgTableReplayIndex (MgTable *t, const MgHashParams &p, int tableBits, U32 *dIndex, hipStream_t st)
{
  U64 n = (U64) 1 << tableBits;
  MG_HIP (hipMemsetAsync (dIndex, 0xff, n * sizeof (U32), st));
  if (t->max)
    { MG_LAUNCH (MG_K_INDEX_REPLAY, st, mgReplayIndexKernel, dim3 (mgGridWide (t->max)), dim3 (256), 0, st,
                          t->value, t->max, p.factor1, p.shift1, tableBits, dIndex);
      MG_HIP (hipGetLastError ());
    }
  MG_LAUNCH (MG_K_INDEX_FINISH, st, mgIndexFinishKernel, dim3 (mgGrid (n, 256, 8192)), dim3 (256), 0, st, dIndex, n);
  MG_HIP (hipGetLastError ());
  return MG_OK;
}


__global__ void mgMergeApplyKernel (const U32 *__restrict__ idx, const U16 *__restrict__ depth2, const U8 *__restrict__ info2,
                                    U32 n2, U16 *__restrict__ baseDepth, U8 *__restrict__ info1)
{
  U64 i = (U64) blockIdx.x * blockDim.x + threadIdx.x;
  const U64 stride = (U64) gridDim.x * blockDim.x;
  for ( ; i < n2 ; i += stride)
    { U32 j = idx[i];
      if (!j) continue;
      U32 d = (U32) baseDepth[j] + depth2[i];
      baseDepth[j] = (U16) (d > 0xffffu ? 0xffffu : d);
      U32 a = info1[j] & 3, c = a + (info2[i] & 3);
      if (c > 3) c = 3;
      info1[j] = (U8) (a | c);
    }
}

__global__ void mgPruneFlagKernel (const U16 *__restrict__ depth, U32 n, int lo, int hi, unsigned char *__restrict__ keep)
{
  U64 i = (U64) blockIdx.x * blockDim.x + threadIdx.x;
  const U64 stride = (U64) gridDim.x * blockDim.x;
  for ( ; i < n ; i += stride)
    { int d = depth[i + 1];
      keep[i] = (d >= lo && (!hi || d < hi)) ? 1 : 0;
    }
}

__global__ void mgPruneMoveKernel (const unsigned char *__restrict__ keep, const MgRankGrp *__restrict__ grp, U32 n,
                                   const U16 *__restrict__ depth, const U8 *__restrict__ info,
                                   U16 *__restrict__ newDepth, U8 *__restrict__ newInfo)
{
  U64 i = (U64) blockIdx.x * blockDim.x + threadIdx.x;
  const U64 stride = (U64) gridDim.x * blockDim.x;
  for ( ; i < n ; i += stride)
    { if (!keep[i]) continue;
      MgRankGrp g = grp[i >> 6];
      U32 r = 1 + g.rank + (U32) __popcll (g.bits & (((U64) 1 << (i & 63)) - 1));
      newDepth[r] = depth[i + 1]; newInfo[r] = info[i + 1];
    }
}

MgStatus mgTableMergeApply (const U32 *dIdx, const U16 *dDepth2, const U8 *dInfo2, U32 n2, U16 *dBaseDepth, U8 *dInfo1, hipStream_t st)
{
  if (!n2) return MG_OK;
  MG_LAUNCH (MG_K_TABLE_EXPORT, st, mgMergeApplyKernel, dim3 (mgGridWide (n2)), dim3 (256), 0, st, dIdx, dDepth2, dInfo2, n2, dBaseDepth, dInfo1);
  MG_HIP (hipGetLastError ());
  return MG_OK;
}

size_t mgTablePruneScratchBytes (U32 n)
{ return mgAl256 (n) + 2 * mgAl256 ((MG_RANK_UNITS + 8) * 8) + mgAl256 (((U64) n / 64 + 2) * sizeof (MgRankGrp)) + 4096; }

MgStatus mgTablePrune (MgTable *t, const U8 *dInfo, int lo, int hi, U64 *dNewValue, U16 *dNewDepth, U8 *dNewInfo,
                       void *scratch, hipStream_t st)
{
  const U32 n = t->max;
  MG_HIP (hipMemsetAsync (t->counters, 0, 16, st));
  if (!n) return MG_OK;
  char *wb = (char *) scratch;
  unsigned char *keep = (unsigned char *) wb;        wb += mgAl256 (n);
  U64 *unitCount = (U64 *) wb;                       wb += mgAl256 ((MG_RANK_UNITS + 8) * 8);
  U64 *unitBase = (U64 *) wb;                        wb += mgAl256 ((MG_RANK_UNITS + 8) * 8);
  MgRankGrp *grp = (MgRankGrp *) wb;
  U32 nBlocks; U64 rows = mgRankRowsPerUnit (n, &nBlocks);
  MG_HIP (hipMemsetAsync (unitCount, 0, (MG_RANK_UNITS + 8) * 8, st));
  MG_LAUNCH (MG_K_TABLE_FLAG, st, mgPruneFlagKernel, dim3 (mgGridWide (n)), dim3 (256), 0, st, t->baseDepth, n, lo, hi, keep);
  MG_LAUNCH (MG_K_RANK_COUNT, st, mgRankCountKernel, dim3 (nBlocks), dim3 (256), 0, st, keep, (U64) n, rows, unitCount);
  MG_LAUNCH (MG_K_RANK_SCAN, st, (mgGroupSumKernel<U64, U64>), dim3 (1), dim3 (MG_GROUP_THREADS), 0, st, unitCount, unitBase, nBlocks * 4, t->counters);
  const MgSegSrc noSrc = {};
  MG_LAUNCH (MG_K_TABLE_ASSIGN, st, (mgRankAssignKernel<false, false>), dim3 (nBlocks), dim3 (256), 0, st,
             keep, t->value + 1, noSrc, (const MgSubSeg *) 0, (U64) n, rows, unitBase, 0u, 0xffffffffu, dNewValue, t->slots, (const U32 *) 0, grp);
  MG_LAUNCH (MG_K_TABLE_EXPORT, st, mgPruneMoveKernel, dim3 (mgGridWide (n)), dim3 (256), 0, st, keep, grp, n, t->baseDepth, dInfo, dNewDepth, dNewInfo);
  MG_HIP (hipGetLastError ());
  return MG_OK;
}
```

Measured before the change: 1238 Gbp/s.

## Split value writes from rank assignment and run them on a side stream

```diff
diff --git a/include/modgpu.h b/include/modgpu.h
--- a/include/modgpu.h
+++ b/include/modgpu.h
@@ -91,6 +91,7 @@
 MgStatus mgTableCheckLayout (Modset *ms, U64 *out6) ;
 MgStatus mgTableDiag (Modset *ms, U64 *out9) ;
 MgStatus mgScanDiag (U64 *out18) ;
+MgStatus mgValueWriterDiag (U64 *out2) ;
 
 MgStatus modsetDepthHistogramDevice (Modset *ms, U64 *dHist65536, void *stream) ;
 
diff --git a/modimizer_amd/__init__.py b/modimizer_amd/__init__.py
--- a/modimizer_amd/__init__.py
+++ b/modimizer_amd/__init__.py
@@ -115,7 +115,7 @@
     "mgPackedWords", "mgPackHost", "mgPackDevice", "mgUnpackDevice", "mgUploadPack",
     "mgScanWorkBytes", "seqhashScanBatchDevice", "seqhashScanBatch", "seqhashMinimizerBatchDevice", "seqhashMinimizerBatch",
     "modsetAddBatchDevice", "modsetFindBatchDevice", "modsetSyncToHost", "mgXferThreadCount", "mgXferDiag", "mgCopyD2HBig", "mgCopyH2DBig", "mgModsetDeviceRelease",
-    "mgModsetHostChanged", "modsetDepthHistogramDevice", "mgTableCheckLayout", "mgTableDiag", "mgScanDiag", "mgAddReadsDevice", "mgQueryReadsDevice", "mgQueryReadsDeviceAsync", "mgQueryReadsDeviceWait",
+    "mgModsetHostChanged", "modsetDepthHistogramDevice", "mgTableCheckLayout", "mgTableDiag", "mgScanDiag", "mgValueWriterDiag", "mgAddReadsDevice", "mgQueryReadsDevice", "mgQueryReadsDeviceAsync", "mgQueryReadsDeviceWait",
     "mgAddSequenceBatch", "mgDepthHistogram", "mgSynthGenome", "mgSynthReads",
     "mgInsertReadsDevice", "mgAddSequences", "mgModsetWriteText", "mgReferenceCreate", "mgReferenceDestroy",
     "mgReferenceRead", "mgQueryProcess", "mgReferenceWrite", "mgGzipOpenWrite", "mgFzOpen", "mgGzipOpenRead", "mgReferenceLoad",
@@ -255,7 +255,7 @@
     sig("modsetFindBatchDevice", i32, MS, vp, u64, vp, vp)
     sig("modsetSyncToHost", i32, MS, i32); sig("mgXferThreadCount", i32); sig("mgXferDiag", None, U64P); sig("mgCopyD2HBig", i32, vp, vp, C.c_size_t); sig("mgCopyH2DBig", i32, vp, vp, C.c_size_t); sig("mgModsetDeviceRelease", i32, MS)
     sig("mgModsetHostChanged", None, MS)
-    sig("modsetDepthHistogramDevice", i32, MS, vp, vp); sig("mgTableCheckLayout", i32, MS, U64P); sig("mgTableDiag", i32, MS, U64P); sig("mgScanDiag", i32, U64P)
+    sig("modsetDepthHistogramDevice", i32, MS, vp, vp); sig("mgTableCheckLayout", i32, MS, U64P); sig("mgTableDiag", i32, MS, U64P); sig("mgScanDiag", i32, U64P); sig("mgValueWriterDiag", i32, U64P)
     sig("mgAddReadsDevice", i32, MS, vp, u64, vp, u32, U64P, vp)
     sig("mgQueryReadsDevice", i32, MS, vp, u64, vp, u32, vp, vp, vp, u64, U64P, vp)
     sig("mgQueryReadsDeviceAsync", i32, MS, vp, u64, vp, u32, vp, vp, vp, u64, C.POINTER(vp), vp); sig("mgQueryReadsDeviceWait", i32, vp, U64P, vp)
diff --git a/modimizer_amd/csrc/mg_api_int.h b/modimizer_amd/csrc/mg_api_int.h
--- a/modimizer_amd/csrc/mg_api_int.h
+++ b/modimizer_amd/csrc/mg_api_int.h
@@ -19,6 +19,15 @@
     bytes = want;
     return MG_OK;
   }
+  bool tryReserve (size_t need)
+  { if (need <= bytes) return true;
+    if (base) (void) hipFree (base);
+    base = 0; bytes = 0;
+    const size_t want = need + need / 8 + (1 << 20);
+    if (hipMalloc ((void **) &base, want) != hipSuccess) { (void) hipGetLastError (); base = 0; return false; }
+    bytes = want;
+    return true;
+  }
   void reset () { used = 0; }
   void *take (size_t n) { size_t a = mgAl256 (used); used = a + n; return base + a; }
   void release () { if (base) (void) hipFree (base); base = 0; bytes = used = 0; }
@@ -31,6 +40,7 @@
   hipStream_t side = 0;
   hipEvent_t scanned[2] = { 0, 0 }, inputReady = 0;
   int ticketsOut = 0, nextSlot = 0; bool slotBusy[2] = { false, false };
+  hipStream_t valueStream = 0; hipEvent_t valueDone[2] = { 0, 0 }, merged = 0; bool valuePending[2] = { false, false }; int valueLast = 0;
   U64 *hPin;
   U32 hostIndexMax;
   bool built;
@@ -46,9 +56,14 @@
 MG_HIDDEN MgDev   *mgDevLookup (const Modset *ms);
 MG_HIDDEN MgStatus mgDevGet (Modset *ms, MgDev **out, hipStream_t st);
 MG_HIDDEN MgStatus mgDevRefuseInFlight (const MgDev *d);
+static inline MgArena &mgArenaOf (MgDev *d, int slot) { return slot ? d->arena2 : d->arena; }
+enum { MG_SETTLE_STREAM = 0, MG_SETTLE_HOST = 1 };
+MG_HIDDEN MgStatus mgValueSettle (MgDev *d, hipStream_t st, int how, int slot = -1);
+MG_HIDDEN MgStatus mgArenaOpen (MgDev *d, int slot, size_t need);
+MG_HIDDEN void     mgArenaTwin (MgDev *d, int slot);
 MG_HIDDEN U64      mgAddChunkSize (void);
 #define MG_ADD_CHUNK (mgAddChunkSize ())
 MG_HIDDEN MgStatus mgAddBatch (Modset *ms, MgDev *d, const U64 *dKmer, U64 n, U32 *dIndexOut, int withDepth,
-                               bool arenaLive, hipStream_t st, const MgHistReq *counted = 0, const MgSegSrc *segSrc = 0);
+                               int liveSlot, hipStream_t st, const MgHistReq *counted = 0, const MgSegSrc *segSrc = 0, bool asideByDefault = false);
 extern "C" void mgHostBatchRelease (void);
 #endif
diff --git a/modimizer_amd/csrc/mg_common.h b/modimizer_amd/csrc/mg_common.h
--- a/modimizer_amd/csrc/mg_common.h
+++ b/modimizer_amd/csrc/mg_common.h
@@ -45,7 +45,7 @@
   MG_K_PAINT_ITEMS, MG_K_DEPTH_GUARD, MG_K_DEPTH_GATHER, MG_K_TEXT_LEN, MG_K_TEXT_SCAN, MG_K_TEXT_WRITE,
   MG_K_SETTEXT_LINES, MG_K_SETTEXT_SCAN, MG_K_SETTEXT_PARSE, MG_K_SETTEXT_LAST,
   MG_K_OVL_ACTIVE, MG_K_OVL_EMIT, MG_K_OVL_SORT, MG_K_OVL_RUNS, MG_K_OVL_PAIR,
-  MG_K_TRIM_OFFSETS, MG_K_TRIM_GATHER, MG_K_SETCOPY, MG_K_COPY_TALLY, MG_K_COUNT
+  MG_K_TRIM_OFFSETS, MG_K_TRIM_GATHER, MG_K_SETCOPY, MG_K_COPY_TALLY, MG_K_RANK_RECORD, MG_K_COUNT
 };
 void mgProfBegin (int id, hipStream_t st);
 void mgProfEnd (int id, hipStream_t st);
@@ -241,9 +241,11 @@
 void     mgTableForget (MgTable *t, hipStream_t st);
 size_t   mgTableAddScratchBytes (const MgTable *t, U64 n);
 bool     mgTableUseBuckets (const MgTable *t, U64 n);
+struct MgValueAside { hipStream_t stream; hipEvent_t merged, done; bool launched; };
 MgStatus mgTableAdd (MgTable *t, const U64 *dKmer, U64 n, int withDepth, void *scratch, hipStream_t st,
                      const MgHistReq *counted = 0,
-                     const MgSegSrc *segSrc = 0);
+                     const MgSegSrc *segSrc = 0,
+                     MgValueAside *aside = 0);
 bool     mgTableAddTakesSegments (const MgTable *t, U64 n, const MgHistReq *counted);
 MgStatus mgTableMarkOccupied (MgTable *t, const U64 *dKmer, U64 n, hipStream_t st);
 MgStatus mgTableFind (MgTable *t, const U64 *dKmer, U64 n, U32 *dIndexOut, hipStream_t st);
diff --git a/modimizer_amd/csrc/mg_knobs.c b/modimizer_amd/csrc/mg_knobs.c
--- a/modimizer_amd/csrc/mg_knobs.c
+++ b/modimizer_amd/csrc/mg_knobs.c
@@ -30,6 +30,7 @@
   k.rankSliceShift = num ("MODGPU_RANK_SLICE_SHIFT");
   k.flagPolarity = num ("MODGPU_FLAG_POLARITY");   k.mergeSlots = num ("MODGPU_MERGE_SLOTS");
   k.mergePlace = num ("MODGPU_MERGE_PLACE");
+  k.valueAsync = num ("MODGPU_VALUE_ASYNC");
   k.bucketR = num ("MODGPU_BUCKET_R");             k.bucketT = num ("MODGPU_BUCKET_T");
   e = getenv ("MODGPU_HOT_SPLIT");
   k.hotSplit = e && *e ? atol (e) : MG_KNOB_UNSET;
diff --git a/modimizer_amd/csrc/mg_knobs.h b/modimizer_amd/csrc/mg_knobs.h
--- a/modimizer_amd/csrc/mg_knobs.h
+++ b/modimizer_amd/csrc/mg_knobs.h
@@ -24,6 +24,7 @@
   long mergePlace;
   long bucketR, bucketT;
   long hotSplit, hotChunk;
+  long valueAsync;
   long noAvx2;
   long textHost;
   long textWindowKb;
diff --git a/modimizer_amd/csrc/mg_modsetdev.hip b/modimizer_amd/csrc/mg_modsetdev.hip
--- a/modimizer_amd/csrc/mg_modsetdev.hip
+++ b/modimizer_amd/csrc/mg_modsetdev.hip
@@ -15,10 +15,47 @@
 MgDev *mgDevLookup (const Modset *ms)
 { std::lock_guard<std::mutex> g (gRegLock); auto it = gReg.find (ms); return it == gReg.end () ? 0 : it->second; }
 
+MgStatus mgValueSettle (MgDev *d, hipStream_t st, int how, int slot)
+{
+  for (int i = 0 ; i < 2 ; ++i)
+    { if (!d->valuePending[i] || (slot >= 0 && i != slot)) continue;
+      if (how == MG_SETTLE_HOST) { MG_HIP (hipEventSynchronize (d->valueDone[i])); d->valuePending[i] = false; }
+      else MG_HIP (hipStreamWaitEvent (st, d->valueDone[i], 0));
+    }
+  return MG_OK;
+}
+MgStatus mgArenaOpen (MgDev *d, int slot, size_t need)
+{
+  MgStatus s = mgValueSettle (d, 0, MG_SETTLE_HOST, slot); if (s) return s;
+  MgArena &ar = mgArenaOf (d, slot);
+  if ((s = ar.reserve (need))) return s;
+  ar.reset ();
+  return MG_OK;
+}
+void mgArenaTwin (MgDev *d, int slot)
+{
+  MgArena &ar = mgArenaOf (d, slot), &other = mgArenaOf (d, slot ^ 1);
+  if (other.bytes >= ar.used || d->valuePending[slot ^ 1] || d->slotBusy[slot ^ 1]) return;
+  (void) other.tryReserve (ar.used);
+}
+static MgStatus mgValueStream (MgDev *d)
+{
+  if (d->valueStream) return MG_OK;
+  int lo = 0, hi = 0; (void) hipDeviceGetStreamPriorityRange (&lo, &hi);
+  MG_HIP (hipStreamCreateWithPriority (&d->valueStream, hipStreamNonBlocking, hi));
+  for (int i = 0 ; i < 2 ; ++i) MG_HIP (hipEventCreateWithFlags (&d->valueDone[i], hipEventDisableTiming));
+  MG_HIP (hipEventCreateWithFlags (&d->merged, hipEventDisableTiming));
+  return MG_OK;
+}
+
 static void mgDevFree (MgDev *d)
 {
   if (!d) return;
   MgOnDevice here (d->device);
+  (void) mgValueSettle (d, 0, MG_SETTLE_HOST);
+  if (d->valueStream) { (void) hipStreamSynchronize (d->valueStream); (void) hipStreamDestroy (d->valueStream); }
+  for (int i = 0 ; i < 2 ; ++i) if (d->valueDone[i]) (void) hipEventDestroy (d->valueDone[i]);
+  if (d->merged) (void) hipEventDestroy (d->merged);
   if (d->hPin) (void) hipHostFree (d->hPin);
   if (d->built)
     { (void) hipFree (d->t.slots); (void) hipFree (d->t.value); (void) hipFree (d->t.occ); (void) hipFree (d->t.find8);
@@ -55,6 +92,7 @@
 static MgStatus mgDevBuild (Modset *ms, MgDev *d, hipStream_t st)
 {
   MgTable &t = d->t;
+  { MgStatus s0 = mgValueSettle (d, st, MG_SETTLE_HOST); if (s0) return s0; }
   if (ms->tableBits < 20 || ms->tableBits > 32)
     { mgSetError ("device modset supports table bits 20..32 (got %d)", ms->tableBits); return MG_ERR_ARG; }
   memset (&t, 0, sizeof (t));
@@ -106,6 +144,7 @@
     {
       U32 first = d->t.max + 1, last = ms->max;
       if (last >= (ms->tableSize >> 2)) { mgSetError ("modset max %u beyond table capacity", last); return MG_ERR_CAPACITY; }
+      if ((s = mgValueSettle (d, st, MG_SETTLE_STREAM))) return s;
       MG_HIP (hipMemcpyAsync (d->t.value + first, ms->value + first, (size_t) (last - first + 1) * sizeof (U64), hipMemcpyHostToDevice, st));
       MG_HIP (hipMemcpyAsync (d->t.baseDepth + first, ms->depth + first, (size_t) (last - first + 1) * sizeof (U16), hipMemcpyHostToDevice, st));
       d->t.baseZero = false;
@@ -166,8 +205,7 @@
   MgTable &t = d->t;
   if (!t.max) return MG_OK;
   if (!t.pendingDepth) return MG_OK;
-  MgStatus s = d->arena.reserve (mgAl256 ((size_t) t.max * sizeof (U16)) + 4096); if (s) return s;
-  d->arena.reset ();
+  MgStatus s = mgArenaOpen (d, 0, mgAl256 ((size_t) t.max * sizeof (U16)) + 4096); if (s) return s;
   U16 *dDelta = (U16 *) d->arena.take ((size_t) t.max * sizeof (U16));
   s = mgTableExportDepth (&t, dDelta, st);
   MG_HIP (hipStreamSynchronize (st));
@@ -180,13 +218,14 @@
   MgTable &t = d->t;
   const U32 max1 = t.max;
   const char *const sorry = "device merge failed";
+  if (mgValueSettle (d, st, MG_SETTLE_HOST)) return mgFailedWith (sorry);
   MgDevScratch scratch ("device merge");
   U8 *dI1; U32 *dIdx;
   const size_t cap1 = (size_t) max1 + n2 + 2;
   if (scratch.get (&dI1, cap1) || scratch.get (&dIdx, n2)) return -1;
   if (hipMemset (dI1, 0, cap1) || hipDeviceSynchronize ()) return mgFailedWith (sorry);
   if (mgXferH2D (dI1, ms1->info, (size_t) max1 + 1)) return mgFailedWith (sorry);
-  MgStatus as = mgAddBatch (ms1, d, dV2, n2, dIdx, 0, false, st);
+  MgStatus as = mgAddBatch (ms1, d, dV2, n2, dIdx, 0, -1, st);
   if (as == MG_ERR_CAPACITY) { fprintf (stderr, "FATAL ERROR: %s\n", mgLastError ()); exit (-1); }
   if (as) return mgFailedWith (sorry);
   t.baseZero = false; t.liveHistValid = false;
@@ -232,6 +271,7 @@
   MgDev *d; if (mgDevGet (ms, &d, st)) return -1;
   MgTable &t = d->t;
   const U32 n = t.max;
+  if (mgValueSettle (d, st, MG_SETTLE_HOST)) return -1;
   if (mgFoldCounts (d, st)) return -1;
   const char *const sorry = "device prune failed";
   MgDevScratch scratch ("device prune");
@@ -289,18 +329,28 @@
 }
 
 static MgStatus mgAddChunk (Modset *ms, MgDev *d, const U64 *dKmer, U64 n, U32 *dIndexOut, int withDepth,
-                            void *scratch, hipStream_t st, const MgHistReq *counted = 0, const MgSegSrc *segSrc = 0)
+                            void *scratch, hipStream_t st, const MgHistReq *counted = 0, const MgSegSrc *segSrc = 0, int asideSlot = -1)
 {
   MgTable &t = d->t;
   MgStatus s;
   MG_HIP (hipMemsetAsync (t.counters, 0, 16, st));
-  if ((s = mgTableAdd (&t, dKmer, n, withDepth, scratch, st, counted, segSrc))) return s;
+  MgValueAside aside = {};
+  if (asideSlot >= 0)
+    { if ((s = mgValueStream (d))) return s;
+      if ((s = mgValueSettle (d, 0, MG_SETTLE_HOST, asideSlot))) return s;
+      aside.stream = d->valueStream; aside.merged = d->merged; aside.done = d->valueDone[asideSlot];
+    }
+  else if ((s = mgValueSettle (d, st, MG_SETTLE_STREAM))) return s;
+  s = mgTableAdd (&t, dKmer, n, withDepth, scratch, st, counted, segSrc, asideSlot >= 0 ? &aside : 0);
+  if (aside.launched) { d->valuePending[asideSlot] = true; d->valueLast = asideSlot; }
+  if (s) return s;
   volatile U64 *c = d->hPin;
   MG_HIP (hipMemcpyAsync (d->hPin, t.counters, 16, hipMemcpyDeviceToHost, st));
   MG_HIP (hipStreamSynchronize (st));
   U64 newMax = (U64) t.max + c[0];
   if (c[1] || newMax >= t.size)
     {
+      if ((s = mgValueSettle (d, st, MG_SETTLE_HOST))) return s;
       if ((s = mgTableRollback (&t, st))) return s;
       mgSetError ("hashTableSize %u is too small for %llu", t.size, (unsigned long long) newMax);
       return MG_ERR_CAPACITY;
@@ -313,27 +363,29 @@
 }
 
 MgStatus mgAddBatch (Modset *ms, MgDev *d, const U64 *dKmer, U64 n, U32 *dIndexOut, int withDepth,
-                     bool arenaLive, hipStream_t st, const MgHistReq *counted, const MgSegSrc *segSrc)
+                     int liveSlot, hipStream_t st, const MgHistReq *counted, const MgSegSrc *segSrc, bool asideByDefault)
 {
   if (!n) return MG_OK;
   MgStatus s = mgDevRefuseInFlight (d); if (s) return s;
   U64 chunk = n < MG_ADD_CHUNK ? n : MG_ADD_CHUNK;
   if ((s = mgTableEnsure (&d->t, chunk, st))) return s;
   size_t need = mgTableAddScratchBytes (&d->t, chunk) + 4096;
-  if (!arenaLive)
-    { if ((s = d->arena.reserve (need))) return s;
-      d->arena.reset ();
-    }
-  else if (d->arena.bytes - d->arena.used < need)
+  const int slot = liveSlot >= 0 ? liveSlot : 0;
+  MgArena &ar = mgArenaOf (d, slot);
+  if (liveSlot < 0) { if ((s = mgArenaOpen (d, 0, need))) return s; }
+  else if (ar.bytes - ar.used < need)
     { mgSetError ("internal: arena too small for insert temporaries"); return MG_ERR_NOMEM; }
-  void *scratch = d->arena.take (mgTableAddScratchBytes (&d->t, chunk));
+  void *scratch = ar.take (mgTableAddScratchBytes (&d->t, chunk));
+  const long va = mgKnobs ()->valueAsync;
+  const bool aside = n <= chunk && mgTableUseBuckets (&d->t, chunk) && (va == MG_KNOB_UNSET ? asideByDefault : va == 1);
   for (U64 off = 0 ; off < n && !s ; off += chunk)
     { U64 m = n - off < chunk ? n - off : chunk;
       if (off) s = mgTableEnsure (&d->t, m, st);
       if (!s) s = mgAddChunk (ms, d, dKmer + off, m, dIndexOut ? dIndexOut + off : 0, withDepth, scratch, st,
                               (counted && n <= chunk) ? counted : 0,
-                              n <= chunk ? segSrc : 0);
-    }
+                              n <= chunk ? segSrc : 0, aside ? slot : -1);
+    }
+  if (aside && liveSlot < 0) { MgStatus w = mgValueSettle (d, st, MG_SETTLE_HOST, slot); if (!s) s = w; }
   return s;
 }
 
@@ -341,7 +393,7 @@
 {
   hipStream_t st = (hipStream_t) stream;
   MgDev *d; MgStatus s = mgDevGet (ms, &d, st); if (s) return s;
-  return mgAddBatch (ms, d, dKmer, n, dIndexOut, withDepth, false, st);
+  return mgAddBatch (ms, d, dKmer, n, dIndexOut, withDepth, -1, st);
 }
 
 extern "C" MgStatus modsetFindBatchDevice (Modset *ms, const U64 *dKmer, U64 n, U32 *dIndexOut, void *stream)
@@ -362,6 +414,7 @@
   hipStream_t st = 0;
   MgStatus s;
   MG_HIP (hipDeviceSynchronize ());
+  if ((s = mgValueSettle (d, st, MG_SETTLE_HOST))) return s;
   if (d->ticketsOut && (t.pendingDepth || (wantIndex && d->hostIndexMax < t.max)))
     { mgSetError ("a query batch of this modset is in flight (its scratch is what a sync would use)"); return MG_ERR_ARG; }
   if (t.max > t.syncedMax)
@@ -372,8 +425,7 @@
   ms->max = t.max;
   if ((s = mgFoldCounts (d, st, ms))) return s;
   if (wantIndex && d->hostIndexMax < t.max)
-    { if ((s = d->arena.reserve (mgAl256 (ms->tableSize * sizeof (U32)) + 4096))) return s;
-      d->arena.reset ();
+    { if ((s = mgArenaOpen (d, 0, mgAl256 (ms->tableSize * sizeof (U32)) + 4096))) return s;
       U32 *dIndex = (U32 *) d->arena.take (ms->tableSize * sizeof (U32));
       if ((s = mgTableReplayIndex (&t, mgMakeParams (ms->hasher), ms->tableBits, dIndex, st))) return s;
       MG_HIP (hipStreamSynchronize (st));
@@ -399,7 +451,7 @@
   MgDev *d = mgDevLookup (ms);
   if (!d || !d->built || d->ticketsOut) return -1;
   if (mgDevOnCallersGpu (d, true)) return -1;
-  if (hipDeviceSynchronize () != hipSuccess || mgFoldCounts (d, 0, ms)) return -1;
+  if (hipDeviceSynchronize () != hipSuccess || mgValueSettle (d, 0, MG_SETTLE_HOST) || mgFoldCounts (d, 0, ms)) return -1;
   *dValue1 = d->t.value + 1; *dDepth1 = d->t.baseDepth + 1; *max = d->t.max;
   return 0;
 }
@@ -449,6 +501,7 @@
   if (!d->built) return MG_OK;
   if ((s = mgDevRefuseInFlight (d))) return s;
   MG_HIP (hipDeviceSynchronize ());
+  if ((s = mgValueSettle (d, 0, MG_SETTLE_HOST))) return s;
   ms->max = d->t.max;
   *t = &d->t;
   return MG_OK;
diff --git a/modimizer_amd/csrc/mg_reads.hip b/modimizer_amd/csrc/mg_reads.hip
--- a/modimizer_amd/csrc/mg_reads.hip
+++ b/modimizer_amd/csrc/mg_reads.hip
@@ -5,7 +5,6 @@
 
 struct MgScanReq { const Seqhash *sh; const U32 *dPacked; U64 totalBases; const U64 *dReadOffsets; U32 nReads; bool wantPos; size_t extraPerSurvivor;
                    U32 *outPosF, *outRid; U64 outCap; bool lazy; };
-static inline MgArena &mgArenaOf (MgDev *d, int slot) { return slot ? d->arena2 : d->arena; }
 static inline U64 *mgCountPin (MgDev *d, int slot) { return d->hPin + 8 + 8 * slot; }
 
 static MgStatus mgScanStart (MgDev *d, int slot, const MgScanReq &q, U64 cap, MgScanBufs *b, hipStream_t st)
@@ -21,8 +20,7 @@
   const size_t need = mgAl256 (cap * perS) + 4 * 4096 + 512 * MG_HIST_STRIDE * 4 + mgAl256 (mgScanWorkBytes (q.totalBases, q.nReads, cap))
                       + (q.extraPerSurvivor ? mgTableAddScratchBytes (&d->t, cap < MG_ADD_CHUNK ? cap : MG_ADD_CHUNK) + 8192 : 0) + 8 * 256
                       + (lookupHist ? mgTableFindPartScratchBytes (cap) + 8192 : 0) + (lookup2 ? mgTableFindPart2ScratchBytes (cap) + 8192 : 0);
-  MgStatus s = ar.reserve (need); if (s) return s;
-  ar.reset ();
+  MgStatus s = mgArenaOpen (d, slot, need); if (s) return s;
   b->cap = cap;
   b->kmer = (U64 *) ar.take (cap * 8);
   const bool direct = q.wantPos && q.outPosF && q.outRid && q.outCap >= cap;
@@ -69,7 +67,7 @@
 static MgStatus mgScanIntoArena (MgDev *d, const Seqhash *sh, const U32 *dPacked, U64 totalBases,
                                  const U64 *dReadOffsets, U32 nReads, bool wantPos, size_t extraPerSurvivor,
                                  MgScanBufs *b, U64 *nOut, hipStream_t st,
-                                 U32 *outPosF = 0, U32 *outRid = 0, U64 outCap = 0, bool lazy = false)
+                                 U32 *outPosF = 0, U32 *outRid = 0, U64 outCap = 0, bool lazy = false, int slot = 0)
 {
   MgStatus s = mgDevRefuseInFlight (d); if (s) return s;
   MgScanReq q = { sh, dPacked, totalBases, dReadOffsets, nReads, wantPos, extraPerSurvivor, outPosF, outRid, outCap, lazy };
@@ -79,7 +77,7 @@
       if (expect > MG_ADD_CHUNK) expect = MG_ADD_CHUNK;
       if ((s = mgTableEnsure (&d->t, expect, st))) return s;
     }
-  return mgScanRounds (d, 0, q, mgSurvivorGuess (sh, totalBases), b, nOut, st);
+  return mgScanRounds (d, slot, q, mgSurvivorGuess (sh, totalBases), b, nOut, st);
 }
 
 extern "C" MgStatus mgAddReadsDevice (Modset *ms, const U32 *dPacked, U64 totalBases,
@@ -91,17 +89,28 @@
   if (!totalBases || !nReads) return MG_OK;
   MgScanBufs b; U64 n = 0;
   d->t.loadPct = 75;
-  if ((s = mgScanIntoArena (d, ms->hasher, dPacked, totalBases, dReadOffsets, nReads, false, 4, &b, &n, st, 0, 0, 0, true))) return s;
+  int slot = d->valuePending[d->valueLast] ? d->valueLast ^ 1 : 0;
+  if (d->valuePending[slot ^ 1] && mgArenaOf (d, slot).bytes < mgArenaOf (d, slot ^ 1).used)
+    {
+      if ((s = mgValueSettle (d, 0, MG_SETTLE_HOST, slot))) return s;
+      if (!mgArenaOf (d, slot).tryReserve (mgArenaOf (d, slot ^ 1).used)) slot ^= 1;
+    }
+  if ((s = mgScanIntoArena (d, ms->hasher, dPacked, totalBases, dReadOffsets, nReads, false, 4, &b, &n, st, 0, 0, 0, true, slot))) return s;
   if (nHash) *nHash = n;
   if (!n) return MG_OK;
   if (b.lazy)
     { const U64 chunk = n < MG_ADD_CHUNK ? n : MG_ADD_CHUNK;
       if ((s = mgTableEnsure (&d->t, chunk, st))) return s;
       if (n <= MG_ADD_CHUNK && mgTableAddTakesSegments (&d->t, n, &b.counted))
-        return mgAddBatch (ms, d, 0, n, 0, 1, true, st, &b.counted, &b.seg);
+        { s = mgAddBatch (ms, d, 0, n, 0, 1, slot, st, &b.counted, &b.seg, true);
+          if (!s && d->valuePending[slot]) mgArenaTwin (d, slot);
+          return s;
+        }
       if ((s = mgLaunchSegCompact (b.seg, b.kmer, b.cap, b.count, st))) return s;
     }
-  return mgAddBatch (ms, d, b.kmer, n, 0, 1, true, st, &b.counted);
+  s = mgAddBatch (ms, d, b.kmer, n, 0, 1, slot, st, &b.counted, 0, true);
+  if (!s && d->valuePending[slot]) mgArenaTwin (d, slot);
+  return s;
 }
 
 static MgStatus mgSeedsOfScanned (Modset *ms, MgDev *d, MgScanBufs &b, U64 n, U32 *dSeedIndex, U32 *dSeedPosF, U32 *dSeedRead, U64 capacity, hipStream_t st)
@@ -109,7 +118,7 @@
   if (n > capacity)
     { mgSetError ("%llu seeds exceed the caller's capacity %llu", (unsigned long long) n, (unsigned long long) capacity); return MG_ERR_CAPACITY; }
   MgStatus s;
-  if (ms) s = mgAddBatch (ms, d, b.kmer, n, dSeedIndex, 0, true, st, &b.counted);
+  if (ms) s = mgAddBatch (ms, d, b.kmer, n, dSeedIndex, 0, 0, st, &b.counted);
   else if (b.lazy && b.findScratch && mgTableFindTakesPartition (&d->t, n, &b.counted))
     s = mgTableFindPartitioned (&d->t, b.seg, n, &b.counted, dSeedIndex, b.kmer, b.findScratch, st, b.findScratch2);
   else s = b.lazy ? mgTableFindSegments (&d->t, b.seg, n, dSeedIndex, st) : mgTableFind (&d->t, b.kmer, n, dSeedIndex, st);
@@ -211,7 +220,8 @@
       for (int i = 0 ; i < 2 ; ++i) MG_HIP (hipEventCreateWithFlags (&d->scanned[i], hipEventDisableTiming));
       MG_HIP (hipEventCreateWithFlags (&d->inputReady, hipEventDisableTiming));
     }
-  const int slot = d->slotBusy[d->nextSlot] ? d->nextSlot ^ 1 : d->nextSlot;
+  int slot = d->slotBusy[d->nextSlot] ? d->nextSlot ^ 1 : d->nextSlot;
+  if (d->valuePending[slot] && !d->slotBusy[slot ^ 1] && !d->valuePending[slot ^ 1]) slot ^= 1;
   MgQueryTicket *t = new MgQueryTicket ();
   t->ms = ms; t->d = d; t->slot = slot; t->dSeedIndex = dSeedIndex; t->dSeedPosF = dSeedPosF; t->dSeedRead = dSeedRead; t->capacity = capacity;
   t->q = MgScanReq { ms->hasher, dPacked, totalBases, dReadOffsets, nReads, true, 0, dSeedPosF, dSeedRead, capacity, true };
diff --git a/modimizer_amd/csrc/mg_runtime.hip b/modimizer_amd/csrc/mg_runtime.hip
--- a/modimizer_amd/csrc/mg_runtime.hip
+++ b/modimizer_amd/csrc/mg_runtime.hip
@@ -72,7 +72,7 @@
   "mgPaintItemsKernel", "mgDepthGuardKernel", "mgDepthGatherKernel", "mgTextLenKernel", "mgTextScanKernel", "mgTextWriteKernel",
   "mgSetTextLinesKernel", "mgSetTextScanKernel", "mgSetTextParseKernel", "mgSetTextLastKernel",
   "mgOvElem..TableKernels", "mgOvEmitKernel", "overlap sorts", "mgOvHead..PairInitKernels", "mgOvPairKernel",
-  "mgTrimSkip+OffsetsKernel", "mgTrimGatherKernel", "mgSetCopyKernel", "mgCopyTallyKernel" };
+  "mgTrimSkip+OffsetsKernel", "mgTrimGatherKernel", "mgSetCopyKernel", "mgCopyTallyKernel", "mgRankRecordKernel" };
 #define MG_PROF_POOL 8192
 struct MgProfRec { int id; hipEvent_t a, b; };
 static struct {
diff --git a/modimizer_amd/csrc/mg_table.hip b/modimizer_amd/csrc/mg_table.hip
--- a/modimizer_amd/csrc/mg_table.hip
+++ b/modimizer_amd/csrc/mg_table.hip
@@ -1,3 +1,4 @@
+#include <atomic>
 #include "mg_table.h"
 
 
@@ -82,9 +83,9 @@
 }
 
 #define MG_RANK_ROWS 8
-template <bool DIRECT, bool SEG>
+template <bool DIRECT>
 __global__ __launch_bounds__ (256)
-void mgRankAssignKernel (const unsigned char *__restrict__ flags, const U64 *__restrict__ kmer, const MgSegSrc src, const MgSubSeg *__restrict__ subSeg,
+void mgRankAssignKernel (const unsigned char *__restrict__ flags, const U64 *__restrict__ kmer,
                          U64 n, U64 rowsPerUnit,
                          const U64 *__restrict__ unitBase, U32 baseMax, U32 size,
                          U64 *__restrict__ value, MgSlot *__restrict__ slots, const U32 *__restrict__ slotId,
@@ -99,8 +100,6 @@
   if (row >= rEnd) return;
   U64 run = unitBase[unit];
   const U64 below = ((U64) 1 << lane) - 1;
-  MgSegCursor cur; cur.w = 0; cur.s0 = 0; cur.s1 = 0;
-  if (SEG) { mgSegCursorFrom (subSeg, row * 64 / MG_PART_SUB, &cur); mgSegCursorSeek (src, &cur, row * 64); }
   for ( ; row < rEnd ; row += MG_RANK_ROWS)
     { bool f[MG_RANK_ROWS]; U64 km[MG_RANK_ROWS]; U32 fl[MG_RANK_ROWS];
 #pragma unroll
@@ -113,16 +112,7 @@
       for (int j = 0 ; j < MG_RANK_ROWS ; ++j)
         { const U64 o = (row + j) * 64 + lane;
           const bool in = (row + j < rEnd) && (o < n);
-          if (SEG)
-            { km[j] = 0;
-              if ((row + j) * 64 < n && row + j < rEnd)
-                { const U64 o0 = (row + j) * 64, last = o0 + 63 < n ? o0 + 63 : n - 1;
-                  mgSegCursorSeek (src, &cur, o0);
-                  const U64 *at = mgSegAddr (src, cur, o, last);
-                  if (in) km[j] = __builtin_nontemporal_load (at);
-                }
-            }
-          else km[j] = in ? __builtin_nontemporal_load (&kmer[o]) : 0;
+          km[j] = in ? __builtin_nontemporal_load (&kmer[o]) : 0;
         }
 #pragma unroll
       for (int j = 0 ; j < MG_RANK_ROWS ; ++j)
@@ -144,6 +134,92 @@
                 }
             }
           run += (U32) __popcll (bits);
+        }
+    }
+}
+
+__device__ __forceinline__ U32 mgFlagBits16 (const uint4 &q)
+{
+#define MG_NIB(w) ((((w) & 0x01010101u) * 0x00204081u >> 21) & 0xfu)
+  return MG_NIB (q.x) | MG_NIB (q.y) << 4 | MG_NIB (q.z) << 8 | MG_NIB (q.w) << 12;
+#undef MG_NIB
+}
+
+__global__ __launch_bounds__ (256)
+void mgRankRecordKernel (const unsigned char *__restrict__ flags, U64 n, U64 rowsPerUnit, const U64 *__restrict__ unitBase, MgRankGrp *__restrict__ grp)
+{
+  MG_BUILD_PRIO ();
+  const int lane = threadIdx.x & 63;
+  const U64 unit = (U64) blockIdx.x * 4 + (U32) __builtin_amdgcn_readfirstlane ((int) (threadIdx.x >> 6));
+  const U64 nRows = (n + 63) / 64;
+  U64 row = unit * rowsPerUnit, rEnd = row + rowsPerUnit;
+  if (rEnd > nRows) rEnd = nRows;
+  if (row >= rEnd) return;
+  U32 run = (U32) unitBase[unit];
+  for ( ; row < rEnd ; row += 64)
+    { const U64 r = row + lane;
+      const bool in = r < rEnd;
+      uint4 q[4] = {};
+      if (in)
+        { const uint4 *p = reinterpret_cast<const uint4 *> (flags + r * 64);
+#pragma unroll
+          for (int i = 0 ; i < 4 ; ++i) q[i] = p[i];
+        }
+      U64 bits = 0;
+#pragma unroll
+      for (int i = 0 ; i < 4 ; ++i) bits |= (U64) mgFlagBits16 (q[i]) << (16 * i);
+      if (in && (r + 1) * 64 > n) bits &= ((U64) 1 << (n - r * 64)) - 1;
+      const U32 c = (U32) __popcll (bits), inc = mgWaveInclusiveSum (c);
+      if (in) { MgRankGrp g; g.bits = bits; g.rank = run + inc - c; g.pad = 0; grp[r] = g; }
+      run += (U32) __builtin_amdgcn_readlane ((int) inc, 63);
+    }
+}
+
+template <bool SEG>
+__global__ __launch_bounds__ (256)
+void mgValueWriteKernel (const MgRankGrp *__restrict__ grp, const U64 *__restrict__ kmer, const MgSegSrc src, const MgSubSeg *__restrict__ subSeg,
+                         U64 n, U64 rowsPerWave, U32 baseMax, U32 size, U64 *__restrict__ value)
+{
+  const int lane = threadIdx.x & 63;
+  const U64 wave = (U64) blockIdx.x * 4 + (U32) __builtin_amdgcn_readfirstlane ((int) (threadIdx.x >> 6));
+  const U64 nRows = (n + 63) / 64;
+  U64 row = wave * rowsPerWave, rEnd = row + rowsPerWave;
+  if (rEnd > nRows) rEnd = nRows;
+  if (row >= rEnd) return;
+  const U64 below = ((U64) 1 << lane) - 1;
+  MgSegCursor cur; cur.w = 0; cur.s0 = 0; cur.s1 = 0;
+  if (SEG) { mgSegCursorFrom (subSeg, row * 64 / MG_PART_SUB, &cur); mgSegCursorSeek (src, &cur, row * 64); }
+  for ( ; row < rEnd ; row += MG_RANK_ROWS)
+    { U64 km[MG_RANK_ROWS]; U64 bits[MG_RANK_ROWS]; U32 rank[MG_RANK_ROWS];
+#pragma unroll
+      for (int j = 0 ; j < MG_RANK_ROWS ; ++j)
+        { const MgRankGrp g = grp[row + j < rEnd ? row + j : row];
+          bits[j] = g.bits; rank[j] = g.rank;
+        }
+#pragma unroll
+      for (int j = 0 ; j < MG_RANK_ROWS ; ++j)
+        { const U64 o = (row + j) * 64 + lane;
+          const bool in = (row + j < rEnd) && (o < n);
+          if (SEG)
+            { km[j] = 0;
+              if (row + j < rEnd)
+                { const U64 o0 = (row + j) * 64, last = o0 + 63 < n ? o0 + 63 : n - 1;
+                  mgSegCursorSeek (src, &cur, o0);
+                  const U64 *at = mgSegAddr (src, cur, o, last);
+                  if (in) km[j] = __builtin_nontemporal_load (at);
+                }
+            }
+          else km[j] = in ? __builtin_nontemporal_load (&kmer[o]) : 0;
+        }
+#pragma unroll
+      for (int j = 0 ; j < MG_RANK_ROWS ; ++j) asm volatile ("" : "+v" (km[j]));
+#pragma unroll
+      for (int j = 0 ; j < MG_RANK_ROWS ; ++j)
+        { if (row + j >= rEnd) break;
+          if ((bits[j] >> lane) & 1)
+            { const U64 idx = (U64) baseMax + 1 + rank[j] + (U32) __popcll (bits[j] & below);
+              if (idx < size) __builtin_nontemporal_store (km[j], &value[idx]);
+            }
         }
     }
 }
@@ -692,21 +768,32 @@
   p->tighten = tighten; p->tightPct = tightPct;
 }
 
-static MgStatus mgAssignIndices (MgTable *t, const unsigned char *flags, const U64 *dKmer, const MgSegSrc *segSrc, const MgSubSeg *subSeg, U64 n,
-                                 U64 *unitCount, U64 *unitBase, const U32 *slotId, MgRankGrp *grp, hipStream_t st)
+static MgStatus mgCountFlags (MgTable *t, const unsigned char *flags, U64 n, U64 *unitCount, U64 *unitBase, U32 *nBlocks, U64 *rows, hipStream_t st)
+{
+  *rows = mgRankRowsPerUnit (n, nBlocks);
+  MG_LAUNCH (MG_K_RANK_COUNT, st, mgRankCountKernel, dim3 (*nBlocks), dim3 (256), 0, st, flags, n, *rows, unitCount);
+  MG_LAUNCH (MG_K_RANK_SCAN, st, (mgGroupSumKernel<U64, U64>), dim3 (1), dim3 (MG_GROUP_THREADS), 0, st, unitCount, unitBase, *nBlocks * 4, t->counters);
+  return MG_OK;
+}
+
+#ifndef MG_VALUE_WAVES_ASIDE
+#define MG_VALUE_WAVES_ASIDE 2048u
+#endif
+#define MG_VALUE_WAVES_ALONE 8192u
+static std::atomic<U64> gValueWriters[2];
+static MgStatus mgWriteValues (MgTable *t, const MgRankGrp *grp, const U64 *dKmer, const MgSegSrc *segSrc, const MgSubSeg *subSeg, U64 n, U32 waves, hipStream_t st)
 {
   const MgSegSrc noSrc = {};
-  U32 nBlocks; const U64 rows = mgRankRowsPerUnit (n, &nBlocks);
-  MG_LAUNCH (MG_K_RANK_COUNT, st, mgRankCountKernel, dim3 (nBlocks), dim3 (256), 0, st, flags, n, rows, unitCount);
-  MG_LAUNCH (MG_K_RANK_SCAN, st, (mgGroupSumKernel<U64, U64>), dim3 (1), dim3 (MG_GROUP_THREADS), 0, st, unitCount, unitBase, nBlocks * 4, t->counters);
-#define MG_ASSIGN(DIRECT, SEG, KMER, SRC, SUB) MG_LAUNCH (MG_K_TABLE_ASSIGN, st, (mgRankAssignKernel<DIRECT, SEG>), dim3 (nBlocks), dim3 (256), 0, st, \
-                                                          flags, KMER, SRC, SUB, n, rows, unitBase, t->max, t->size, t->value, t->slots, slotId, grp)
-  if (slotId) MG_ASSIGN (true, false, dKmer, noSrc, (const MgSubSeg *) 0);
-  else if (segSrc) MG_ASSIGN (false, true, (const U64 *) 0, *segSrc, subSeg);
-  else MG_ASSIGN (false, false, dKmer, noSrc, (const MgSubSeg *) 0);
-#undef MG_ASSIGN
-  return MG_OK;
-}
+  const U64 nRows = (n + 63) / 64;
+  U64 per = (nRows + waves - 1) / waves;
+  per = (per + MG_RANK_ROWS - 1) / MG_RANK_ROWS * MG_RANK_ROWS;
+  const U32 nBlocks = (U32) (((nRows + per - 1) / per + 3) / 4);
+  if (segSrc) MG_LAUNCH (MG_K_TABLE_ASSIGN, st, (mgValueWriteKernel<true>), dim3 (nBlocks), dim3 (256), 0, st, grp, (const U64 *) 0, *segSrc, subSeg, n, per, t->max, t->size, t->value);
+  else MG_LAUNCH (MG_K_TABLE_ASSIGN, st, (mgValueWriteKernel<false>), dim3 (nBlocks), dim3 (256), 0, st, grp, dKmer, noSrc, (const MgSubSeg *) 0, n, per, t->max, t->size, t->value);
+  MG_HIP (hipGetLastError ());
+  return MG_OK;
+}
+extern "C" MgStatus mgValueWriterDiag (U64 *out2) { for (int i = 0 ; i < 2 ; ++i) out2[i] = gValueWriters[i].load (std::memory_order_relaxed); return MG_OK; }
 
 static MgStatus mgAddTighten (MgTable *t, int tightPct, const U32 *uniqCount, U64 *fullest, hipStream_t st)
 {
@@ -740,9 +827,11 @@
 }
 
 MgStatus mgTableAdd (MgTable *t, const U64 *dKmer, U64 n, int withDepth, void *scratch, hipStream_t st,
-                     const MgHistReq *counted, const MgSegSrc *segSrc)
-{
+                     const MgHistReq *counted, const MgSegSrc *segSrc, MgValueAside *aside)
+{
+  if (aside) aside->launched = false;
   if (!n) return MG_OK;
+  if ((uintptr_t) scratch & 255) { mgSetError ("internal: the insert's scratch is not 256-byte aligned"); return MG_ERR_ARG; }
   if (segSrc && !mgTableAddTakesSegments (t, n, counted)) { mgSetError ("internal: this insert needs the dense k-mers"); return MG_ERR_ARG; }
   t->liveHistValid = false;
   if (withDepth) t->pendingDepth = true;
@@ -758,10 +847,15 @@
 
   if (!mgTableUseBuckets (t, n))
     { U32 *slotId = (U32 *) wb;
+      if (aside) { mgSetError ("internal: the direct insert has no value writer to run aside"); return MG_ERR_ARG; }
       { MgStatus cs = mgTableClean (t, st); if (cs) return cs; }
       MG_LAUNCH (MG_K_TABLE_INSERT, st, mgTableInsertKernel, dim3 (mgGridWide (n)), dim3 (256), 0, st, t->slots, g, dKmer, n, slotId, withDepth, t->counters);
       MG_LAUNCH (MG_K_TABLE_FLAG, st, mgDirectFlagKernel, dim3 (mgGridWide (n)), dim3 (256), 0, st, t->slots, slotId, n, flags);
-      { MgStatus as = mgAssignIndices (t, flags, dKmer, (const MgSegSrc *) 0, (const MgSubSeg *) 0, n, blockCount, blockBase, slotId, grp, st); if (as) return as; }
+      { U32 nBlocks; U64 rows;
+        MgStatus as = mgCountFlags (t, flags, n, blockCount, blockBase, &nBlocks, &rows, st); if (as) return as;
+        MG_LAUNCH (MG_K_TABLE_ASSIGN, st, (mgRankAssignKernel<true>), dim3 (nBlocks), dim3 (256), 0, st,
+                   flags, dKmer, n, rows, blockBase, t->max, t->size, t->value, t->slots, slotId, grp);
+      }
       MG_HIP (hipGetLastError ());
       return mgTableMarkOccupied (t, dKmer, n, st);
     }
@@ -848,10 +942,22 @@
     { if ((s = mgAddTighten (t, plan.tightPct, uniqCount, &fullest, st))) return s;
       if (t->R != a.g.R) { a.g = mgGeomOf (t); lds = mgMergeLdsBytes (t->R); }
     }
-  if ((s = mgAssignIndices (t, flags, dKmer, segSrc, subSeg, n, blockCount, blockBase, (const U32 *) 0, grp, st))) return s;
+  { U32 nBlocks; U64 rows;
+    if ((s = mgCountFlags (t, flags, n, blockCount, blockBase, &nBlocks, &rows, st))) return s;
+    MG_LAUNCH (MG_K_RANK_RECORD, st, mgRankRecordKernel, dim3 (nBlocks), dim3 (256), 0, st, flags, n, rows, blockBase, grp);
+  }
+  if (!aside && (s = mgWriteValues (t, grp, dKmer, segSrc, subSeg, n, MG_VALUE_WAVES_ALONE, st))) return s;
   if ((s = mgRankLookup (a, st))) return s;
   if ((s = mgBucketMerge (a, fullest, bThreads, bGrid, perBlock, lds, st))) return s;
   MG_HIP (hipGetLastError ());
+  if (aside)
+    { MG_HIP (hipEventRecord (aside->merged, st));
+      MG_HIP (hipStreamWaitEvent (aside->stream, aside->merged, 0));
+      if ((s = mgWriteValues (t, grp, dKmer, segSrc, subSeg, n, MG_VALUE_WAVES_ASIDE, aside->stream))) return s;
+      MG_HIP (hipEventRecord (aside->done, aside->stream));
+      aside->launched = true;
+    }
+  gValueWriters[aside ? 0 : 1].fetch_add (1, std::memory_order_relaxed);
   return MG_OK;
 }
 
@@ -1057,9 +1163,8 @@
   MG_LAUNCH (MG_K_TABLE_FLAG, st, mgPruneFlagKernel, dim3 (mgGridWide (n)), dim3 (256), 0, st, t->baseDepth, n, lo, hi, keep);
   MG_LAUNCH (MG_K_RANK_COUNT, st, mgRankCountKernel, dim3 (nBlocks), dim3 (256), 0, st, keep, (U64) n, rows, unitCount);
   MG_LAUNCH (MG_K_RANK_SCAN, st, (mgGroupSumKernel<U64, U64>), dim3 (1), dim3 (MG_GROUP_THREADS), 0, st, unitCount, unitBase, nBlocks * 4, t->counters);
-  const MgSegSrc noSrc = {};
-  MG_LAUNCH (MG_K_TABLE_ASSIGN, st, (mgRankAssignKernel<false, false>), dim3 (nBlocks), dim3 (256), 0, st,
-             keep, t->value + 1, noSrc, (const MgSubSeg *) 0, (U64) n, rows, unitBase, 0u, 0xffffffffu, dNewValue, t->slots, (const U32 *) 0, grp);
+  MG_LAUNCH (MG_K_TABLE_ASSIGN, st, (mgRankAssignKernel<false>), dim3 (nBlocks), dim3 (256), 0, st,
+             keep, t->value + 1, (U64) n, rows, unitBase, 0u, 0xffffffffu, dNewValue, t->slots, (const U32 *) 0, grp);
   MG_LAUNCH (MG_K_TABLE_EXPORT, st, mgPruneMoveKernel, dim3 (mgGridWide (n)), dim3 (256), 0, st, keep, grp, n, t->baseDepth, dInfo, dNewDepth, dNewInfo);
   MG_HIP (hipGetLastError ());
   return MG_OK;
```

Measured after the change: 1281 Gbp/s (median of 6 runs). 3.5% higher.
